# Acelogic/LTX-2-MLX

Measured on AMD Instinct MI355X. Metric: denoise_steps_per_sec, higher is better.
Workload: dtype bf16; 1 GPU; LTX-2 19B distilled DiT (48 layers, D=4096, 32x128 heads), 768x512x65 (N=3456 video tokens, S=1024 text tokens), 8-step distilled sigmas, bf16, random-init weights; parallelism=prompt-parallel x1 (independent prompt/seed per GPU, one RCCL weight broadcast)

## Files before the change

include/ltx2hip.h:

```cpp
#ifndef LTX2HIP_H
#define LTX2HIP_H

#include <stdint.h>

#ifdef __cplusplus
extern "C" {
#endif

#define LTX2_OK 0
#define LTX2_E_INVALID (-1)
#define LTX2_E_HIP (-2)
#define LTX2_E_STATE (-3)

#define LTX2_DTYPE_BF16 0
#define LTX2_DTYPE_F32 1
#define LTX2_DTYPE_FP8_E4M3FN 2

#define LTX2_ABI_VERSION 3

const char* ltx2_last_error(void);
void ltx2_clear_error(void);
int ltx2_abi_version(void);


#define LTX2_EPI_BF16 0
#define LTX2_EPI_GELU_BF16 1
#define LTX2_EPI_SILU_BF16 2
#define LTX2_EPI_F32 3
#define LTX2_EPI_RESID_GATE_F32 4
#define LTX2_EPI_ADD_BF16 5

int ltx2_gemm_bf16(const void* A, int64_t lda, const void* W, const float* bias, void* out, int64_t ldo, int M,
                   int N, int K, int epilogue, const float* gate, int64_t gate_stride, const float* gate_table,
                   const void* res, int64_t ldres, void* stream);

int ltx2_gemm_qkv_vt(const void* A, int64_t lda, const void* W, const float* bias, void* out, int64_t ldo, int M, int N, int K,
                     void* vt, int vt_col0, int Npad, int head_dim, int* fused, void* stream);

int ltx2_gemm_w8a16(const void* A, int64_t lda, const void* W8, const float* wscale, const float* bias, void* out, int64_t ldo, int M,
                    int N, int K, int epilogue, const float* gate, int64_t gate_stride, const float* gate_table, void* stream);

int ltx2_gemm_bf16_rowss(const void* A, int64_t lda, const void* W, const float* bias, void* out, int64_t ldo, int M, int N, int K, float* rowss,
                         int* written, void* stream);
int ltx2_flash_attn_rowscale(const void* Q, int64_t ldq, const void* K, int64_t ldk, const void* VT, int Npad, void* out, int64_t ldo, int Nq, int Nkv,
                             int H, int head_dim, float scale, const float* q_ss, int q_ss_ld, int q_norm_dim, float q_eps, void* stream);

int ltx2_gemm_bf16_fold(const void* A, int64_t lda, const void* W, const float* bias, void* out, int64_t ldo, int M, int N, int K, int epilogue,
                        const float* gate_table, void* shadow, int64_t ld_shadow, const float* shadow_scale, float* shadow_ss, int64_t ld_ss,
                        const float* rf_parts, int64_t rf_ld, int rf_nparts, int rf_dim, float rf_eps, int* supported, void* stream);

int ltx2_flash_attn_keymask(const void* Q, int64_t ldq, const void* K, int64_t ldk, const void* VT, int Npad, void* out, int64_t ldo,
                            int Nq, int Nkv, int H, int head_dim, float scale, const float* mask, void* words, void* stream);

#define LTX2_ROUTE_SKINNY 0
#define LTX2_ROUTE_V4_224 1
#define LTX2_ROUTE_V4_256 2
#define LTX2_ROUTE_V4_W8_224 3
#define LTX2_ROUTE_V4_W8_256 4
#define LTX2_ROUTE_V4_F8_224 5
#define LTX2_ROUTE_V4_F8_256 6
#define LTX2_ROUTE_PP 7
#define LTX2_ROUTE_SMALL 8
#define LTX2_ROUTE_NARROW 9
int ltx2_gemm_route(int M, int N, int K, int epilogue, int weights, int has_vt);

int ltx2_quantize_rows_fp8(const void* x_bf16, int64_t ldx, int rows, int K, void* codes, int64_t ldo, float* scale, void* stream);
int ltx2_gemm_fp8(const void* A8, int64_t lda, const float* ascale, const void* W8, const float* wscale, const float* bias, void* out,
                  int64_t ldo, int M, int N, int K, int epilogue, const float* gate, int64_t gate_stride, const float* gate_table,
                  void* stream);

int ltx2_gemm_fp8_qkv_vt(const void* A8, int64_t lda, const float* ascale, const void* W8, const float* wscale, const float* bias, void* out,
                         int64_t ldo, int M, int N, int K, void* vt, int vt_col0, int Npad, int head_dim, int* fused, void* stream);

int ltx2_gemv_f32(const float* a, int64_t lda, const void* W, const float* bias, float* out, int64_t ldo, int M,
                  int N, int K, int act_in, int act_out, void* stream);

int ltx2_conv3d_fused(const void* x, const void* w, const float* bias, void* out, int T, int H, int W, int Cin,
                      int Cout, int causal, int mode, const void* res, int ft, int fh, int fw, int residual,
                      int pad_zero, int kt, void* stream);

int ltx2_groupnorm_silu(const void* x, const void* res, void* y, int64_t P, int C, int groups, float eps,
                        const float* gamma, const float* beta, float* scratch, int act, void* stream);

int ltx2_s2d_downsample(const void* y, const void* x, void* out, int T, int H, int W, int Cc, int Cin, int st, int sh,
                        int sw, void* stream);

int ltx2_latent_normalize_nchw(const void* x, const float* mean, const float* std, float* out, int C, int64_t P,
                               void* stream);

int ltx2_adaln_rmsnorm(const float* x, int64_t ldx, void* out, int64_t ldo, int rows, int D, float eps,
                       int layer_norm, const float* scale_tab, const float* shift_tab, const float* scale_emb,
                       const float* shift_emb, int64_t emb_stride, void* stream);
int ltx2_adaln_rmsnorm2(const float* x, int64_t ldx, void* out0, void* out1, int64_t ldo, int rows, int D, float eps, const float* scale0,
                        const float* shift0, const float* scale1, const float* shift1, void* stream);

int ltx2_adaln_rmsnorm_fp8(const float* x, int64_t ldx, void* out_bf16, int64_t ldo, void* codes, int64_t ldq, float* scale, int rows, int D,
                           float eps, int layer_norm, const float* scale_tab, const float* shift_tab, const float* scale_emb,
                           const float* shift_emb, int64_t emb_stride, void* stream);

int ltx2_qknorm_rope(void* buf, int64_t ld, int rows, int D, int head_dim, int q_off, const float* q_weight,
                     int k_off, const float* k_weight, float eps, const float* cos, const float* sin, void* stream);

int ltx2_vt_transpose(const void* V, int64_t ld, void* VT, int Nkv, int Npad, int H, int head_dim, void* stream);

int ltx2_flash_attn(const void* Q, int64_t ldq, const void* K, int64_t ldk, const void* VT, int Npad, void* out,
                    int64_t ldo, int Nq, int Nkv, int H, int head_dim, float scale, void* stream);


int ltx2_attn_head_gate(void* att, int64_t ld, const void* x, int64_t ldx, const void* gate_w, const float* gate_b,
                        float* logits, int rows, int Dq, int H, int head_dim, void* stream);

int ltx2_flash_attn_gated(const void* Q, int64_t ldq, const void* K, int64_t ldk, const void* VT, int Npad, void* out, int64_t ldo, int Nq, int Nkv,
                          int H, int head_dim, float scale, const float* gate_logits, int gate_ld, void* stream);

int ltx2_flash_attn_gated_parts(const void* Q, int64_t ldq, const void* K, int64_t ldk, const void* VT, int Npad, void* out, int64_t ldo, int Nq, int Nkv,
                                int H, int head_dim, float scale, const void* x, int64_t ldx, const void* gate_w, const float* gate_b, int Dq, float* parts,
                                void* stream);

int ltx2_rope_tables(const float* positions, const float* freq_grid, const float* max_pos, int N, int n_dims, int n_freq,
                     int half_dim, float* cos_out, float* sin_out, void* stream);

int ltx2_timestep_sinusoid(const float* t, int64_t t_stride, float mult, int T, int dim, float* out_f32,
                           void* out_bf16, void* stream);

int ltx2_dequant_fp8_e4m3fn(const void* in, float scale, void* out_bf16, int64_t n, void* stream);
int ltx2_cast_f32_bf16(const float* in, void* out, int64_t n, void* stream);

int ltx2_x0_from_velocity(const float* latent, const float* velocity, const float* ts_ptr, int64_t ts_stride,
                          float ts_scalar, float* x0, int rows, int C, void* stream);

int ltx2_euler_step(const float* x, const float* x0, const float* mask, const float* clean, float sigma,
                    float sigma_next, float* out, int rows, int C, void* stream);

int ltx2_vae_prepare_latent(const float* latent, const float* std, const float* mean, const float* noise,
                            float noise_scale, void* out_bf16, int C, int64_t P, void* stream);
int ltx2_pixnorm_mod_silu(const void* x, void* y, int64_t P, int C, float eps, const float* table, const float* te,
                          int shift_row, int scale_row, void* stream);
int ltx2_vae_unpatchify(const void* x, float* video, int T, int H, int W, void* stream);
int ltx2_video_to_uint8(const float* video, uint8_t* frames, int T, int H, int W, void* stream);
int ltx2_video_chunk_to_uint8(const float* cur, const float* prev, const float* ramp, uint8_t* frames, int Tc, int prev_T, int ov, int H,
                              int W, int t_dst0, int T_out, void* stream);
int ltx2_tile_blend_accumulate(const float* tile, int dt, int dh, int dw, int nt, int nh, int nw, const float* mt, const float* mh,
                               const float* mw, float* out, float* wsum, int OT, int OH, int OW, int t0, int h0, int w0, void* stream);
int ltx2_tile_blend_finish(float* out, const float* wsum, int64_t plane, void* stream);

#define LTX2_MODEL_VIDEO_ONLY 0
#define LTX2_MODEL_AUDIO_VIDEO 1

typedef struct ltx2_dit ltx2_dit;

typedef struct ltx2_dit_config {
    int num_layers;
    int num_heads;
    int head_dim;
    int in_channels;
    int out_channels;
    int caption_channels;
    float norm_eps;
    float timestep_scale;
    int model_type;
    int audio_heads;
    int audio_head_dim;
    int audio_in_channels;
    int audio_out_channels;
    int cross_attention_adaln;
    int apply_gated_attention;
    float av_ca_timestep_scale;
} ltx2_dit_config;

int ltx2_dit_create(const ltx2_dit_config* cfg, ltx2_dit** out);
void ltx2_dit_destroy(ltx2_dit* ctx);

int ltx2_dit_set_weight(ltx2_dit* ctx, const char* name, const void* ptr, int dtype, int64_t numel);

int64_t ltx2_dit_workspace_bytes(const ltx2_dit* ctx, int N, int S, int per_token);
int ltx2_dit_bind_workspace(ltx2_dit* ctx, void* ptr, int64_t bytes, int N, int S, int per_token);
int64_t ltx2_dit_workspace_bytes_av(const ltx2_dit* ctx, int N, int S, int Na, int Sa, int per_token);
int ltx2_dit_bind_workspace_av(ltx2_dit* ctx, void* ptr, int64_t bytes, int N, int S, int Na, int Sa, int per_token);

int ltx2_dit_prepare(ltx2_dit* ctx, const float* context, int S, const float* rope_cos, const float* rope_sin,
                     void* stream);
int ltx2_dit_prepare_av(ltx2_dit* ctx, const float* v_context, int S, const float* v_cos, const float* v_sin,
                        const float* v_cross_cos, const float* v_cross_sin, const float* a_context, int Sa,
                        const float* a_cos, const float* a_sin, const float* a_cross_cos, const float* a_cross_sin,
                        void* stream);

int ltx2_dit_forward(ltx2_dit* ctx, const float* latent, const float* timesteps, int n_timesteps, const float* sigma,
                     float* velocity, void* stream);
int ltx2_dit_forward_av(ltx2_dit* ctx, const float* v_latent, const float* v_timesteps, int n_v_timesteps,
                        const float* v_sigma, const float* a_latent, const float* a_timesteps, int n_a_timesteps,
                        const float* a_sigma, float* v_velocity, float* a_velocity, void* stream);

int ltx2_dit_denoise_step(ltx2_dit* ctx, float* latent, const float* timesteps, int n_timesteps, const float* sigma_dev,
                          const float* mask, const float* clean, float sigma, float sigma_next, float* x0_out, void* stream);
int ltx2_dit_denoise_step_av(ltx2_dit* ctx, float* v_latent, float* a_latent, const float* v_timesteps,
                             int n_v_timesteps, const float* a_timesteps, int n_a_timesteps, const float* sigma_dev,
                             const float* v_mask, const float* v_clean, const float* a_mask, const float* a_clean,
                             float sigma, float sigma_next, float* v_x0_out, float* a_x0_out, void* stream);

int ltx2_dit_graph_capture(ltx2_dit* ctx, float* latent, const float* host_sigmas, int n_steps, void* stream);
int ltx2_dit_graph_capture_cond(ltx2_dit* ctx, float* latent, const float* host_sigmas, int n_steps, const float* mask, int64_t n_mask, const float* clean,
                                int64_t n_clean, void* stream);
int ltx2_dit_graph_capture_cond_av(ltx2_dit* ctx, float* v_latent, float* a_latent, const float* host_sigmas, int n_steps, const float* v_mask, int64_t n_v_mask,
                                   const float* v_clean, int64_t n_v_clean, const float* a_mask, int64_t n_a_mask, const float* a_clean, int64_t n_a_clean, void* stream);
int ltx2_dit_graph_capture_av(ltx2_dit* ctx, float* v_latent, float* a_latent, const float* host_sigmas, int n_steps,
                              void* stream);
int ltx2_dit_graph_launch(ltx2_dit* ctx, void* stream);

int ltx2_dit_set_context_mask(ltx2_dit* ctx, int modality, const float* mask, int S, void* stream);

int ltx2_dit_set_option(ltx2_dit* ctx, const char* name, int value);


int ltx2_dit_profile_begin(ltx2_dit* ctx, int epilogue);
int ltx2_dit_profile_end(ltx2_dit* ctx, double* total_ms, int64_t* launches, double* flops);

typedef struct ltx2_vae ltx2_vae;

#define LTX2_VAE_MAX_BLOCKS 16
#define LTX2_VAE_RES 0
#define LTX2_VAE_UPSAMPLE 1

typedef struct ltx2_vae_config {
    int n_blocks;
    int kind[LTX2_VAE_MAX_BLOCKS];
    int num_layers[LTX2_VAE_MAX_BLOCKS];
    int stride[LTX2_VAE_MAX_BLOCKS][3];
    int multiplier[LTX2_VAE_MAX_BLOCKS];
    int residual[LTX2_VAE_MAX_BLOCKS];
    int base_channels;
    int latent_channels;
    int timestep_conditioning;
    float decode_noise_scale;
} ltx2_vae_config;

int ltx2_vae_create(const ltx2_vae_config* cfg, ltx2_vae** out);
void ltx2_vae_destroy(ltx2_vae* ctx);
int ltx2_vae_set_weight(ltx2_vae* ctx, const char* name, const void* ptr, int dtype, int64_t numel);
int ltx2_vae_set_timestep_multiplier(ltx2_vae* ctx, float multiplier);
int64_t ltx2_vae_workspace_bytes(const ltx2_vae* ctx, int T, int H, int W);
int ltx2_vae_bind_workspace(ltx2_vae* ctx, void* ptr, int64_t bytes);
int ltx2_vae_decode(ltx2_vae* ctx, const float* latent, int T, int H, int W, float timestep, const float* noise,
                    int causal, float* video, void* stream);
int ltx2_vae_out_frames(const ltx2_vae* ctx, int T);

int ltx2_gemma_attn(const void* q, int64_t ldq, const void* k, int64_t ldk, const void* v, int64_t ldv, void* out, int64_t ldo, int Tq,
                    int Tkv, int heads, int kv_heads, int causal, int window, float scale, void* stream);
int ltx2_gemma_qknorm_rope(void* qkv, int64_t ld, int rows, int q_heads, int kv_heads, const float* q_w, const float* k_w, float eps,
                           const float* cos, const float* sin, void* stream);
int ltx2_gemma_resid_norm(const float* x_in, int64_t ldx, const void* y, int64_t ldy, const float* w_post, const float* w_next, float* x_out,
                          int64_t ld_xout, void* h_out, int64_t ldh, float* hf_out, int64_t ldhf, int rows, int D, float eps, void* stream);
#define LTX2_GEMMA_ACT_SILU 0
#define LTX2_GEMMA_ACT_GELU_TANH 1
int ltx2_gemma_gated_act(const void* gu, int64_t ldgu, void* out, int64_t ldo, int rows, int inter, int act, void* stream);
int ltx2_gemma_embed(const int32_t* ids, int rows, const void* table, int vocab, int D, float scale, float* x, int64_t ldx, void* stream);
int ltx2_gemma_features_rms(const float* hs, int64_t layer_stride, int64_t row_stride, const int32_t* valid, void* out, int64_t ldo, int T, int L,
                            int D, float eps, void* stream);

#define LTX2_AUDIO_PRO_NONE 0
#define LTX2_AUDIO_PRO_LEAKY_RELU 1
#define LTX2_AUDIO_PRO_MAGNITUDE 2
#define LTX2_AUDIO_ACT_NONE 0
#define LTX2_AUDIO_ACT_TANH 1
#define LTX2_AUDIO_ACT_CLIP 2
#define LTX2_AUDIO_ACT_LOG 3
int ltx2_audio_conv(const float* x, int64_t ldx, int h_in, int w_in, int c_in, const float* w, int64_t ldw, const float* bias, float* y,
                    int64_t ldy, int h_out, int w_out, int c_out, int kh, int kw, int stride, int dilation, int pad_h, int pad_w, int upsample,
                    int prologue, float slope, const float* res, int64_t ldres, float alpha, float beta, int act, void* stream);
int ltx2_audio_conv_transpose1d(const float* x, int64_t ldx, int t_in, int c_in, const float* w_phase, const float* bias, float* y, int64_t ldy,
                                int t_out, int c_out, int k, int rate, int padding, int prologue, float slope, void* stream);
int ltx2_audio_pixnorm_silu(const float* x, int64_t ldx, float* y, int64_t ldy, int64_t rows, int c, float eps, void* stream);
int ltx2_audio_snake_aa(const float* x, int64_t ldx, int t, int c, const float* alpha, const float* beta, const float* up_filter, int up_k,
                        const float* down_filter, int down_k, float* y, int64_t ldy, void* stream);
int ltx2_audio_upsample(const float* x, int64_t ldx, int t_in, int c, const float* filter, int k, int ratio, int pad, int pad_left, float* y,
                        int64_t ldy, int t_out, void* stream);

#ifdef __cplusplus
}
#endif
#endif
```

ltx-2-mlx_amd/csrc/attention.h:

```cpp
#pragma once
#include "common.h"

struct AttnParams {
    const bf16* Q;
    const bf16* K;
    const bf16* VT;
    bf16* O;
    long ldq, ldk, ldo, vt_head_stride;
    int Nq, Nkv, Npad, H;
    int head_dim;
    float scale_log2e;
    const float* q_ss;
    int q_ss_ld, q_norm_dim;
    float q_eps;
    const unsigned long long* kmask;
    const float* gate;
    int gate_ld;
    int gate_parts;
    const float* gate_bias;
};

int attn_launch(const AttnParams& p, hipStream_t stream);
int vt_transpose_launch(const bf16* V, long ld, bf16* VT, int Nkv, int Npad, int H, hipStream_t stream, int head_dim = 128);
```

ltx-2-mlx_amd/csrc/attention.hip:

```cpp
#include "attention.h"
#include <type_traits>

namespace {

constexpr int KVB = 64;
template <int HD>
struct Geo {
    static constexpr int K_TILE = KVB * HD * 2;
    static constexpr int V_TILE = HD * KVB * 2;
    static constexpr int STAGE = K_TILE + V_TILE;
    static constexpr int LDS_BYTES = 2 * STAGE;
    static constexpr int NJ = HD / 32;
};

#ifndef AT_DK
#define AT_DK 6
#endif
#ifndef AT_DV
#define AT_DV 6
#endif
#ifndef AT_XCD
#define AT_XCD 1
#endif
#ifndef AT_DMA
#define AT_DMA 0
#endif
#ifndef AT_PQK
#define AT_PQK 2
#endif
#ifndef AT_PPV
#define AT_PPV 1
#endif
#ifndef AT_PGAP
#define AT_PGAP 0
#endif
#ifndef AT_PRIO
#define AT_PRIO 1
#endif

__device__ __forceinline__ float max3(float a, float b, float c) {
    float d;
    asm("v_max3_f32 %0, %1, %2, %3" : "=v"(d) : "v"(a), "v"(b), "v"(c));
    return d;
}

#define AT_KEY_MASKED (-1.0e30f)

__device__ __forceinline__ void quad_fold_max(float& a, float& b) {
    asm volatile("s_nop 1\n\tv_permlane32_swap_b32 %0, %1\n\ts_nop 1" : "+v"(a), "+v"(b));
    float c = fmaxf(a, b), d = c;
    asm volatile("s_nop 1\n\tv_permlane16_swap_b32 %0, %1\n\ts_nop 1" : "+v"(c), "+v"(d));
    float e = fmaxf(c, d);
    a = e;
    b = e;
    asm volatile("s_nop 1\n\tv_permlane32_swap_b32 %0, %1\n\ts_nop 1" : "+v"(a), "+v"(b));
}
__device__ __forceinline__ void quad_fold_sum(float& a, float& b) {
    asm volatile("s_nop 1\n\tv_permlane32_swap_b32 %0, %1\n\ts_nop 1" : "+v"(a), "+v"(b));
    float c = a + b, d = c;
    asm volatile("s_nop 1\n\tv_permlane16_swap_b32 %0, %1\n\ts_nop 1" : "+v"(c), "+v"(d));
    float e = c + d;
    a = e;
    b = e;
    asm volatile("s_nop 1\n\tv_permlane32_swap_b32 %0, %1\n\ts_nop 1" : "+v"(a), "+v"(b));
}
__device__ __forceinline__ void mfma16_result_guard(f32x4 (&s)[4][2], float& t0, float& t1) {
    asm volatile("s_nop 7\n\ts_nop 7\n\ts_nop 3" : "+v"(s[0][0]), "+v"(s[0][1]), "+v"(s[1][0]), "+v"(s[1][1]), "+v"(s[2][0]), "+v"(s[2][1]), "+v"(s[3][0]), "+v"(s[3][1]),
                 "+v"(t0), "+v"(t1));
}

#ifndef AT_P_BIG
#ifdef LTX2_F16
#define AT_P_BIG 32768.0f
#else
#define AT_P_BIG 1073741824.0f
#endif
#endif

#ifdef AT_COUNT_FALLBACK
__device__ unsigned long long ltx2_at_counts[2];
#endif

template <int HD, bool QS = false, bool KM = false, int NW = 4>
__global__ __launch_bounds__(NW * 64, NW == 4 ? 2 : 1) void attn_fwd_kernel(const AttnParams p) {
    using G = Geo<HD>;
    constexpr int K_TILE = G::K_TILE, STAGE = G::STAGE, NJ = G::NJ * 4 / NW, QB = NW * 32;
    static_assert(NW == 4 || (NW == 8 && HD == 128), "waves per workgroup");
    constexpr int NKS = HD / 32, NDB = HD / 16;
    constexpr int NK = 4 * NKS, NV = 2 * NDB;
    constexpr int DK = AT_DK < NK ? AT_DK : NK, DV = AT_DV < NV ? AT_DV : NV;
    extern __shared__ __attribute__((aligned(16))) char smem[];
    const unsigned lds0 = (unsigned)(uintptr_t)(lds_ptr_t)smem;
    const int tid = threadIdx.x, lane = tid & 63;
    const int wv = __builtin_amdgcn_readfirstlane(tid >> 6);
    const int l15 = lane & 15, g = lane >> 4;
    const int nt = (p.Nkv + KVB - 1) / KVB, nfull = p.Nkv / KVB;

    unsigned k_vo[NJ], v_vo[NJ];
#pragma unroll
    for (int j = 0; j < NJ; ++j) {
        const int kr = HD == 128 ? (wv * NJ + j) * 4 + (lane >> 4) : (wv * NJ + j) * 8 + (lane >> 3);
        const int kchunk = HD == 128 ? ((lane & 15) ^ (kr & 15)) : ((lane & 7) ^ ((kr >> 1) & 7));
        k_vo[j] = ((unsigned)kr * (unsigned)p.ldk + kchunk * 8) * 2;
        const int vr = (wv * NJ + j) * 8 + (lane >> 3);
        const int vchunk = (lane & 7) ^ ((vr >> 1) & 7);
        v_vo[j] = ((unsigned)vr * (unsigned)p.Npad + vchunk * 8) * 2;
    }
    const unsigned k_tile_bytes = (unsigned)KVB * (unsigned)p.ldk * 2;
    const unsigned k_bytes = ((unsigned)(p.Nkv - 1) * (unsigned)p.ldk + HD) * 2, v_bytes = (unsigned)HD * (unsigned)p.Npad * 2;
    const int k_xor = HD == 128 ? l15 : ((l15 >> 1) & 7);
    const int v_xor = (l15 >> 1) & 7;
    unsigned k_lane[NKS], v_lane[2];
#pragma unroll
    for (int ks = 0; ks < NKS; ++ks) k_lane[ks] = lds0 + l15 * (2 * HD) + (((4 * ks + g) ^ k_xor) << 4);
#pragma unroll
    for (int kk = 0; kk < 2; ++kk) v_lane[kk] = lds0 + K_TILE + l15 * 128 + (((4 * kk + g) ^ v_xor) << 4);

    int head = blockIdx.y, qt = blockIdx.x;
#if AT_XCD
    if ((gridDim.y & 7) == 0) {
        const int b = blockIdx.y * gridDim.x + blockIdx.x, xcd = b & 7, idx = b >> 3;
        head = xcd + 8 * (idx / (int)gridDim.x);
        qt = idx % (int)gridDim.x;
    }
#endif
    const int tb = nt;
    const int q0 = qt * QB + wv * 32;

    const __amdgpu_buffer_rsrc_t rk = __builtin_amdgcn_make_buffer_rsrc((void*)(p.K + head * HD), 0, (int)k_bytes, 0x00020000);
    const __amdgpu_buffer_rsrc_t rv = __builtin_amdgcn_make_buffer_rsrc((void*)(p.VT + (long)head * p.vt_head_stride), 0, (int)v_bytes, 0x00020000);
    auto stage_piece = [&](int t, int buf, int i) {
        char* dst = smem + buf * STAGE + wv * (NJ * 1024);
#if defined(__HIP_DEVICE_COMPILE__)
        if (i < NJ)
            __builtin_amdgcn_raw_ptr_buffer_load_lds(rk, (lds_ptr_t)(dst + i * 1024), 16, k_vo[i], t * k_tile_bytes, 0, 0);
        else
            __builtin_amdgcn_raw_ptr_buffer_load_lds(rv, (lds_ptr_t)(dst + K_TILE + (i - NJ) * 1024), 16, v_vo[i - NJ], t * (KVB * 2), 0, 0);
#else
        (void)dst; (void)t; (void)i;
#endif
    };
#pragma unroll
    for (int i = 0; i < 2 * NJ; ++i) stage_piece(0, 0, i);

    float c[2] = {p.scale_log2e, p.scale_log2e};
    if constexpr (QS) {
        const int quarter = p.q_ss_ld >> 2;
        float ss[2] = {0.f, 0.f};
#pragma unroll
        for (int qb = 0; qb < 2; ++qb) {
            const float* sp = p.q_ss + (long)min(q0 + 16 * qb + l15, p.Nq - 1) * p.q_ss_ld + g * quarter;
#pragma unroll 4
            for (int jj = 0; jj < quarter; jj += 4) {
                const f32x4 t = *(const f32x4*)(sp + jj);
                ss[qb] += (t[0] + t[1]) + (t[2] + t[3]);
            }
        }
        quad_fold_sum(ss[0], ss[1]);
        c[0] *= rsqrtf(ss[0] / (float)p.q_norm_dim + p.q_eps);
        c[1] *= rsqrtf(ss[1] / (float)p.q_norm_dim + p.q_eps);
    }
    bf16x8 qf[2][NKS];
#pragma unroll
    for (int qb = 0; qb < 2; ++qb) {
        const int qrow = min(q0 + 16 * qb + l15, p.Nq - 1);
        const bf16* qp = p.Q + (long)qrow * p.ldq + head * HD + 8 * g;
#pragma unroll
        for (int ks = 0; ks < NKS; ++ks) {
            const bf16x8 raw = *(const bf16x8*)(qp + 32 * ks);
#pragma unroll
            for (int e = 0; e < 8; ++e) qf[qb][ks][e] = f2bf(bf2f(raw[e]) * c[qb]);
        }
    }

    f32x4 o[NDB][2];
#pragma unroll
    for (int d = 0; d < NDB; ++d)
#pragma unroll
        for (int qb = 0; qb < 2; ++qb) o[d][qb] = f32x4{0.f, 0.f, 0.f, 0.f};
    float M[2] = {0.f, 0.f}, l_run[2] = {0.f, 0.f};
    auto tile = [&](const int t, auto fast, auto masked, auto par, const bool first) __attribute__((always_inline)) {
        constexpr bool FAST = decltype(fast)::value, MASKED = decltype(masked)::value;
        constexpr int PAR = decltype(par)::value;
        static_assert(!(FAST && (MASKED || KM)), "the stale-maximum path takes whole, unmasked tiles");
        asm volatile("s_waitcnt vmcnt(0)" ::: "memory");
        __syncthreads();
        const int tn = min(t + 1, tb - 1);
        constexpr int nbuf = 1 - PAR;
#if AT_PRIO
        __builtin_amdgcn_s_setprio(AT_PQK);
#endif
        f32x4 s[4][2];
#pragma unroll
        for (int kb = 0; kb < 4; ++kb)
#pragma unroll
            for (int qb = 0; qb < 2; ++qb) {
                const float init = KM ? 0.f : -M[qb];
                s[kb][qb] = f32x4{init, init, init, init};
            }
        bf16x8 pf[2][2];
        float ps[2] = {0.f, 0.f};
        auto exp_pair = [&](auto KB, auto Q4) __attribute__((always_inline)) {
            constexpr int kb = decltype(KB)::value, q4 = decltype(Q4)::value, qb = q4 / 2, r = 2 * (q4 % 2), kk = kb / 2, e = 4 * (kb % 2) + r;
            asm volatile("" : "+v"(s[kb][qb]));
            float p0 = __builtin_amdgcn_exp2f(s[kb][qb][r]), p1 = __builtin_amdgcn_exp2f(s[kb][qb][r + 1]);
            asm volatile("" : "+v"(p0), "+v"(p1));
            ps[qb] += p0 + p1;
            pf[qb][kk][e] = f2bf(p0);
            pf[qb][kk][e + 1] = f2bf(p1);
        };
        u32x4 kf[NK];
        auto read_k = [&](auto N) {
            constexpr int n = decltype(N)::value, kb = n / NKS, ks = n % NKS;
            kf[n] = lds_read16<PAR * STAGE + kb * 16 * 2 * HD>(k_lane[ks]);
        };
        static_for<0, DK>(read_k);
        static_for<0, NK>([&](auto N) __attribute__((always_inline)) {
            constexpr int n = decltype(N)::value, kb = n / NKS, ks = n % NKS;
            if constexpr (n + DK < NK) read_k(std::integral_constant<int, n + DK>{});
            lds_wait<(n + DK < NK ? DK : NK - 1 - n)>(kf[n]);
            s[kb][0] = LTX2_MFMA_16x16x32(as_bf16x8(kf[n]), qf[0][ks], s[kb][0], 0, 0, 0);
            if constexpr (FAST && kb > 0) static_for<(4 * ks) / NKS, (4 * ks + 2) / NKS>([&](auto Q4) { exp_pair(std::integral_constant<int, kb - 1>{}, Q4); });
            s[kb][1] = LTX2_MFMA_16x16x32(as_bf16x8(kf[n]), qf[1][ks], s[kb][1], 0, 0, 0);
            if constexpr (FAST && kb > 0) static_for<(4 * ks + 2) / NKS, (4 * (ks + 1)) / NKS>([&](auto Q4) { exp_pair(std::integral_constant<int, kb - 1>{}, Q4); });
#if AT_DMA == 0
            if constexpr ((n & 1) && n / 2 < 2 * NJ) stage_piece(tn, nbuf, n / 2);
#elif AT_DMA == 2
            if constexpr ((n & 1) && n / 2 < NJ) stage_piece(tn, nbuf, n / 2);
#endif
        });
#if AT_DMA == 0
        static_for<NK / 2, 2 * NJ>([&](auto I) { stage_piece(tn, nbuf, decltype(I)::value); });
#elif AT_DMA == 1
        static_for<0, 2 * NJ>([&](auto I) { stage_piece(tn, nbuf, decltype(I)::value); });
#else
        static_for<(NK / 2 < NJ ? NK / 2 : NJ), 2 * NJ>([&](auto I) { stage_piece(tn, nbuf, decltype(I)::value); });
#endif
        u32x4 vf[NV];
        auto read_v = [&](auto N) {
            constexpr int n = decltype(N)::value, kk = n / NDB, db = n % NDB;
            vf[n] = lds_read16<PAR * STAGE + db * 16 * 128>(v_lane[kk]);
        };
        static_for<0, DV>(read_v);
#if AT_PRIO
        __builtin_amdgcn_s_setprio(AT_PGAP);
#endif
        auto pv = [&](auto N0, auto N1) __attribute__((always_inline)) {
            constexpr int n0 = decltype(N0)::value, n1 = decltype(N1)::value;
#if AT_PRIO
            __builtin_amdgcn_s_setprio(AT_PPV);
#endif
            static_for<n0, n1>([&](auto N) __attribute__((always_inline)) {
                constexpr int n = decltype(N)::value, kk = n / NDB, db = n % NDB;
                if constexpr (n + DV < NV) read_v(std::integral_constant<int, n + DV>{});
                lds_wait<(n + DV < NV ? DV : NV - 1 - n)>(vf[n]);
                o[db][0] = LTX2_MFMA_16x16x32(as_bf16x8(vf[n]), pf[0][kk], o[db][0], 0, 0, 0);
                o[db][1] = LTX2_MFMA_16x16x32(as_bf16x8(vf[n]), pf[1][kk], o[db][1], 0, 0, 0);
            });
#if AT_PRIO
            __builtin_amdgcn_s_setprio(AT_PGAP);
#endif
        };
        using I0 = std::integral_constant<int, 0>;
        using IN = std::integral_constant<int, NV>;
        bool classic = !FAST;
        if constexpr (FAST) {
            static_for<0, 4>([&](auto Q4) { exp_pair(std::integral_constant<int, 3>{}, Q4); });
            classic = __any(!(ps[0] <= AT_P_BIG && ps[1] <= AT_P_BIG));
#ifdef AT_COUNT_FALLBACK
            if (lane == 0) {
                atomicAdd(&ltx2_at_counts[0], 1ull);
                if (classic) atomicAdd(&ltx2_at_counts[1], 1ull);
            }
#endif
        }
        if (classic) {
            if constexpr (MASKED) {
                const int kv0 = t * KVB;
                unsigned long long km = ~0ull;
                if constexpr (KM) km = p.kmask[t];
#pragma unroll
                for (int kb = 0; kb < 4; ++kb)
#pragma unroll
                    for (int r = 0; r < 4; ++r) {
                        const int kl = 16 * kb + 4 * g + r;
                        const bool oob = kv0 + kl >= p.Nkv, off = KM && !((km >> kl) & 1ull);
#pragma unroll
                        for (int qb = 0; qb < 2; ++qb) {
                            if (oob) s[kb][qb][r] = -INFINITY;
                            else if (off) s[kb][qb][r] = AT_KEY_MASKED;
                        }
                    }
            }
            float tmax[2] = {-INFINITY, -INFINITY};
            mfma16_result_guard(s, tmax[0], tmax[1]);
#pragma unroll
            for (int qb = 0; qb < 2; ++qb)
#pragma unroll
                for (int r = 0; r < 4; ++r) {
                    tmax[qb] = max3(tmax[qb], s[0][qb][r], s[1][qb][r]);
                    tmax[qb] = max3(tmax[qb], s[2][qb][r], s[3][qb][r]);
                }
            quad_fold_max(tmax[0], tmax[1]);
            float sub[2];
#pragma unroll
            for (int qb = 0; qb < 2; ++qb) {
                if constexpr (KM) {
                    const float m_new = first ? tmax[qb] : fmaxf(M[qb], tmax[qb]);
                    if (!first) {
                        const float alpha = __builtin_amdgcn_exp2f(M[qb] - m_new);
                        l_run[qb] *= alpha;
#pragma unroll
                        for (int d = 0; d < NDB; ++d) o[d][qb] *= alpha;
                    }
                    M[qb] = m_new;
                    sub[qb] = m_new;
                } else {
                    const float up = first ? tmax[qb] : fmaxf(tmax[qb], 0.f);
                    if (!first) {
                        const float alpha = __builtin_amdgcn_exp2f(-up);
                        l_run[qb] *= alpha;
#pragma unroll
                        for (int d = 0; d < NDB; ++d) o[d][qb] *= alpha;
                    }
                    M[qb] += up;
                    sub[qb] = up;
                }
            }
            ps[0] = 0.f;
            ps[1] = 0.f;
#pragma unroll
            for (int kb = 0; kb < 4; ++kb)
#pragma unroll
                for (int qb = 0; qb < 2; ++qb)
#pragma unroll
                    for (int r = 0; r < 4; r += 2) {
                        const float p0 = __builtin_amdgcn_exp2f(s[kb][qb][r] - sub[qb]), p1 = __builtin_amdgcn_exp2f(s[kb][qb][r + 1] - sub[qb]);
                        ps[qb] += p0 + p1;
                        pf[qb][kb / 2][4 * (kb % 2) + r] = f2bf(p0);
                        pf[qb][kb / 2][4 * (kb % 2) + r + 1] = f2bf(p1);
                    }
        }
        l_run[0] += ps[0];
        l_run[1] += ps[1];
        pv(I0{}, IN{});
    };

    using T_ = std::true_type;
    using F_ = std::false_type;
    using P0 = std::integral_constant<int, 0>;
    using P1 = std::integral_constant<int, 1>;
    if constexpr (KM) {
        for (int t = 0; t < tb; ++t) {
            if (t & 1) tile(t, F_{}, T_{}, P1{}, false);
            else tile(t, F_{}, T_{}, P0{}, t == 0);
        }
    } else {
        const int t_fast_end = min(tb, nfull);
        int t = 0;
        if (nfull > 0) {
            tile(0, F_{}, F_{}, P0{}, true);
            t = 1;
            for (; t + 1 < t_fast_end; t += 2) {
                tile(t, T_{}, F_{}, P1{}, false);
                tile(t + 1, T_{}, F_{}, P0{}, false);
            }
            if (t < t_fast_end) {
                tile(t, T_{}, F_{}, P1{}, false);
                ++t;
            }
        }
        if (nfull < tb) {
            if (nfull & 1) tile(nfull, F_{}, T_{}, P1{}, false);
            else tile(nfull, F_{}, T_{}, P0{}, nfull == 0);
        }
    }
    asm volatile("s_waitcnt vmcnt(0)" ::: "memory");

    float lt[2] = {l_run[0], l_run[1]};
    quad_fold_sum(lt[0], lt[1]);
#pragma unroll
    for (int qb = 0; qb < 2; ++qb) {
        const int qrow = q0 + 16 * qb + l15;
        float inv = 1.0f / lt[qb];
        if (p.gate && qrow < p.Nq) {
            float gl = p.gate[(long)qrow * p.gate_ld + head];
            if (p.gate_parts > 1) {
                for (int pt = 1; pt < p.gate_parts; ++pt) gl += p.gate[((long)pt * p.Nq + qrow) * p.gate_ld + head];
                gl += p.gate_bias[head];
            }
            inv *= 2.f / (1.f + __expf(-gl));
        }
        bf16* op = p.O + (long)min(qrow, p.Nq - 1) * p.ldo + head * HD + 16 * (g & 1) + 8 * (g >> 1);
#pragma unroll
        for (int i = 0; i < NDB / 2; ++i) {
            bf16x4 a, b;
#pragma unroll
            for (int e = 0; e < 4; ++e) {
                a[e] = f2bf(o[2 * i][qb][e] * inv);
                b[e] = f2bf(o[2 * i + 1][qb][e] * inv);
            }
            u32x2 ua = __builtin_bit_cast(u32x2, a), ub = __builtin_bit_cast(u32x2, b);
            asm volatile("s_nop 1\n\tv_permlane16_swap_b32 %0, %2\n\tv_permlane16_swap_b32 %1, %3\n\ts_nop 1" : "+v"(ua[0]), "+v"(ua[1]), "+v"(ub[0]), "+v"(ub[1]));
            const u32x4 w = {ua[0], ua[1], ub[0], ub[1]};
            if (qrow < p.Nq) *(u32x4*)(op + 32 * i) = w;
        }
    }
}

template <int HD>
__global__ __launch_bounds__(256) void vt_transpose_kernel(const bf16* __restrict__ V, long ld, bf16* __restrict__ VT,
                                                           int Nkv, int Npad, long head_stride) {
    __shared__ bf16 tile[64][HD + 2];
    const int head = blockIdx.y, kv0 = blockIdx.x * 64, tid = threadIdx.x;
    {
        constexpr int W = HD / 4;
        const int r = tid >> 2, c0 = (tid & 3) * W;
        const int kv = kv0 + r;
        if (kv < Nkv) {
            const bf16* src = V + (long)kv * ld + head * HD + c0;
#pragma unroll
            for (int i = 0; i < W / 8; ++i) {
                const bf16x8 v = *(const bf16x8*)(src + i * 8);
#pragma unroll
                for (int e = 0; e < 8; ++e) tile[r][c0 + i * 8 + e] = v[e];
            }
        } else {
#pragma unroll
            for (int i = 0; i < W; ++i) tile[r][c0 + i] = f2bf(0.f);
        }
    }
    __syncthreads();
    if (tid < 2 * HD) {
        const int d = tid >> 1, p0 = (tid & 1) * 32;
        bf16* dst = VT + (long)head * head_stride + (long)d * Npad + kv0 + p0;
#pragma unroll
        for (int i = 0; i < 4; ++i) {
            bf16x8 v;
#pragma unroll
            for (int e = 0; e < 8; ++e) {
                const int pos = i * 8 + e;
                const int kvl = 16 * ((pos >> 2) & 1) + 4 * (pos >> 3) + (pos & 3);
                v[e] = tile[p0 + kvl][d];
            }
            *(bf16x8*)(dst + i * 8) = v;
        }
    }
}

}

int attn_launch(const AttnParams& p, hipStream_t stream) {
    LTX2_CHECK_ARG(p.Nq > 0 && p.Nkv > 0 && p.H > 0, "attention: empty problem");
    LTX2_CHECK_ARG(p.head_dim == 0 || p.head_dim == 128 || p.head_dim == 64, "attention: head_dim=%d, only 128 and 64 are implemented", p.head_dim);
    LTX2_CHECK_ARG(p.Npad % 64 == 0 && p.Npad >= p.Nkv, "attention: Npad=%d must be a multiple of 64 >= Nkv", p.Npad);
    LTX2_CHECK_ARG(p.ldq % 8 == 0 && p.ldk % 8 == 0 && p.ldo % 8 == 0, "attention: row strides must keep 16-byte alignment");
    LTX2_CHECK_ARG(p.ldk > 0 && ((long)p.Nkv + 2 * KVB) * p.ldk * 2 < (1L << 31), "attention: Nkv * ldk exceeds the 31-bit K byte offset");
    LTX2_CHECK_ARG((long)p.Npad * (p.head_dim == 64 ? 64 : 128) * 2 < (1L << 31), "attention: Npad * head_dim exceeds the 31-bit V^T byte offset");
    if (p.q_ss)
        LTX2_CHECK_ARG(p.head_dim != 64 && p.q_ss_ld > 0 && p.q_ss_ld % 16 == 0 && p.q_norm_dim > 0, "attention: the per-row scale form needs head_dim 128 and q_ss_ld %% 16 == 0");
#ifndef AT_NW
#define AT_NW 4
#endif
    const int nw = (p.head_dim != 64 && !p.kmask) ? AT_NW : 4;
    dim3 grid((p.Nq + nw * 32 - 1) / (nw * 32), p.H);
#define AT_LAUNCH_NW(HDV, QSV, KMV, NWV)                                                                                                        \
    do {                                                                                                                                        \
        static PerDeviceOnce once_;                                                                                                             \
        if (once_.first())                                                                                                                      \
            (void)hipFuncSetAttribute((const void*)attn_fwd_kernel<HDV, QSV, KMV, NWV>, hipFuncAttributeMaxDynamicSharedMemorySize, Geo<HDV>::LDS_BYTES); \
        hipLaunchKernelGGL((attn_fwd_kernel<HDV, QSV, KMV, NWV>), grid, dim3(NWV * 64), Geo<HDV>::LDS_BYTES, stream, p);                         \
    } while (0)
#define AT_LAUNCH(HDV, QSV, KMV) AT_LAUNCH_NW(HDV, QSV, KMV, 4)
    if (p.head_dim == 64) {
        if (p.kmask) AT_LAUNCH(64, false, true);
        else AT_LAUNCH(64, false, false);
    } else if (p.kmask) {
        if (p.q_ss) AT_LAUNCH(128, true, true);
        else AT_LAUNCH(128, false, true);
    } else if (p.q_ss) {
        if (nw == 8) AT_LAUNCH_NW(128, true, false, 8);
        else AT_LAUNCH(128, true, false);
    } else if (nw == 8) AT_LAUNCH_NW(128, false, false, 8);
    else AT_LAUNCH(128, false, false);
#undef AT_LAUNCH
#undef AT_LAUNCH_NW
    LTX2_CHECK_LAUNCH("attn_fwd_kernel");
    return LTX2_OK;
}

#ifdef AT_COUNT_FALLBACK
extern "C" int ltx2_attn_fallback_counts(unsigned long long* out2, int reset) {
    if (hipMemcpyFromSymbol(out2, HIP_SYMBOL(ltx2_at_counts), 16) != hipSuccess) return LTX2_E_HIP;
    if (reset) {
        const unsigned long long z[2] = {0, 0};
        if (hipMemcpyToSymbol(HIP_SYMBOL(ltx2_at_counts), z, 16) != hipSuccess) return LTX2_E_HIP;
    }
    return LTX2_OK;
}
#endif

int vt_transpose_launch(const bf16* V, long ld, bf16* VT, int Nkv, int Npad, int H, hipStream_t stream, int head_dim) {
    LTX2_CHECK_ARG(Npad % 64 == 0 && Npad >= Nkv && ld % 8 == 0, "vt_transpose: bad strides");
    LTX2_CHECK_ARG(head_dim == 128 || head_dim == 64, "vt_transpose: head_dim=%d, only 128 and 64 are implemented", head_dim);
    dim3 grid(Npad / 64, H);
    if (head_dim == 64)
        hipLaunchKernelGGL(vt_transpose_kernel<64>, grid, dim3(256), 0, stream, V, ld, VT, Nkv, Npad, 64L * Npad);
    else
        hipLaunchKernelGGL(vt_transpose_kernel<128>, grid, dim3(256), 0, stream, V, ld, VT, Nkv, Npad, 128L * Npad);
    LTX2_CHECK_LAUNCH("vt_transpose_kernel");
    return LTX2_OK;
}
```

ltx-2-mlx_amd/csrc/capi.hip:

```cpp
#include <stdarg.h>
#include <stdio.h>

#include "../../include/ltx2hip.h"
#include "attention.h"
#include "gemm.h"
#include "gemma.h"
#include "rowops.h"

static thread_local char g_err[512] = "";

void ltx2_set_error(const char* fmt, ...) {
    va_list ap;
    va_start(ap, fmt);
    vsnprintf(g_err, sizeof(g_err), fmt, ap);
    va_end(ap);
}

extern "C" {

const char* ltx2_last_error(void) { return g_err; }
void ltx2_clear_error(void) { g_err[0] = 0; }
int ltx2_abi_version(void) { return LTX2_ABI_VERSION; }

int ltx2_gemm_bf16(const void* A, int64_t lda, const void* W, const float* bias, void* out, int64_t ldo, int M,
                   int N, int K, int epilogue, const float* gate, int64_t gate_stride, const float* gate_table,
                   const void* res, int64_t ldres, void* stream) {
    LTX2_CHECK_ARG(epilogue >= 0 && epilogue <= LTX2_EPI_ADD_BF16, "gemm: epilogue %d out of range", epilogue);
    LTX2_CHECK_ARG(epilogue != LTX2_EPI_ADD_BF16 || res, "gemm: epilogue ADD_BF16 needs res");
    GemmParams p{};
    p.A = (const bf16*)A;
    p.lda = lda;
    p.W = (const bf16*)W;
    p.bias = bias;
    p.out = out;
    p.ldo = ldo;
    p.M = M;
    p.N = N;
    p.K = K;
    p.gate = gate;
    p.gate_stride = gate_stride;
    p.gate_table = gate_table;
    p.res = (const bf16*)res;
    p.ldres = ldres;
    return gemm_launch(p, epilogue, false, (hipStream_t)stream);
}

int ltx2_adaln_rmsnorm2(const float* x, int64_t ldx, void* out0, void* out1, int64_t ldo, int rows, int D, float eps, const float* scale0,
                        const float* shift0, const float* scale1, const float* shift1, void* stream) {
    LTX2_CHECK_ARG(x && out0 && out1, "adaln_rmsnorm2: null operand");
    const float* sct[2] = {scale0, scale1};
    const float* sht[2] = {shift0, shift1};
    const float* none[2] = {nullptr, nullptr};
    return norm_mod2_launch(x, ldx, (bf16*)out0, (bf16*)out1, ldo, rows, D, eps, sct, sht, none, none, (hipStream_t)stream);
}

int ltx2_gemm_bf16_rowss(const void* A, int64_t lda, const void* W, const float* bias, void* out, int64_t ldo, int M, int N, int K, float* rowss,
                         int* written, void* stream) {
    LTX2_CHECK_ARG(A && W && out && rowss && written, "gemm_bf16_rowss: null argument");
    GemmParams p{};
    p.A = (const bf16*)A;
    p.lda = lda;
    p.W = (const bf16*)W;
    p.bias = bias;
    p.out = out;
    p.ldo = ldo;
    p.M = M;
    p.N = N;
    p.K = K;
    *written = gemm_rowss_supported(p, EPI_BF16) ? 1 : 0;
    if (*written) p.rowss = rowss;
    return gemm_launch(p, EPI_BF16, false, (hipStream_t)stream);
}

int ltx2_gemm_bf16_fold(const void* A, int64_t lda, const void* W, const float* bias, void* out, int64_t ldo, int M, int N, int K, int epilogue,
                        const float* gate_table, void* shadow, int64_t ld_shadow, const float* shadow_scale, float* shadow_ss, int64_t ld_ss,
                        const float* rf_parts, int64_t rf_ld, int rf_nparts, int rf_dim, float rf_eps, int* supported, void* stream) {
    LTX2_CHECK_ARG(A && W && out && supported, "gemm_bf16_fold: null argument");
    LTX2_CHECK_ARG(epilogue == LTX2_EPI_BF16 || epilogue == LTX2_EPI_GELU_BF16 || epilogue == LTX2_EPI_RESID_GATE_F32, "gemm_bf16_fold: epilogue %d (BF16, GELU_BF16 or RESID_GATE_F32)", epilogue);
    GemmParams p{};
    p.A = (const bf16*)A;
    p.lda = lda;
    p.W = (const bf16*)W;
    p.bias = bias;
    p.out = out;
    p.ldo = ldo;
    p.M = M;
    p.N = N;
    p.K = K;
    p.gate_table = gate_table;
    p.shadow = (bf16*)shadow;
    p.ld_shadow = ld_shadow;
    p.shadow_scale = shadow_scale;
    p.shadow_ss = shadow_ss;
    p.ld_ss = ld_ss;
    p.rf_parts = rf_parts;
    p.rf_ld = rf_ld;
    p.rf_nparts = rf_nparts;
    p.rf_dim = rf_dim;
    p.rf_eps = rf_eps;
    *supported = ((p.shadow || p.rf_parts) && gemm_fold_supported(p, epilogue)) ? 1 : 0;
    if (!*supported) return LTX2_OK;
    return gemm_launch(p, epilogue, false, (hipStream_t)stream);
}

int ltx2_flash_attn_rowscale(const void* Q, int64_t ldq, const void* K, int64_t ldk, const void* VT, int Npad, void* out, int64_t ldo, int Nq, int Nkv,
                             int H, int head_dim, float scale, const float* q_ss, int q_ss_ld, int q_norm_dim, float q_eps, void* stream) {
    LTX2_CHECK_ARG(Q && K && VT && out && q_ss, "flash_attn_rowscale: null operand");
    LTX2_CHECK_ARG(head_dim == 128, "flash_attn_rowscale: head_dim=%d, only 128 is implemented", head_dim);
    AttnParams a{};
    a.Q = (const bf16*)Q;
    a.ldq = ldq;
    a.K = (const bf16*)K;
    a.ldk = ldk;
    a.VT = (const bf16*)VT;
    a.vt_head_stride = (long)head_dim * Npad;
    a.head_dim = head_dim;
    a.O = (bf16*)out;
    a.ldo = ldo;
    a.Nq = Nq;
    a.Nkv = Nkv;
    a.Npad = Npad;
    a.H = H;
    a.scale_log2e = scale * 1.4426950408889634f;
    a.q_ss = q_ss;
    a.q_ss_ld = q_ss_ld;
    a.q_norm_dim = q_norm_dim;
    a.q_eps = q_eps;
    return attn_launch(a, (hipStream_t)stream);
}

int ltx2_flash_attn_keymask(const void* Q, int64_t ldq, const void* K, int64_t ldk, const void* VT, int Npad, void* out, int64_t ldo, int Nq, int Nkv,
                            int H, int head_dim, float scale, const float* mask, void* words, void* stream) {
    LTX2_CHECK_ARG(Q && K && VT && out && mask && words, "flash_attn_keymask: null operand");
    if (const int rc = keymask_words_launch(mask, Nkv, (unsigned long long*)words, Npad / 64, (hipStream_t)stream)) return rc;
    AttnParams a{};
    a.Q = (const bf16*)Q;
    a.ldq = ldq;
    a.K = (const bf16*)K;
    a.ldk = ldk;
    a.VT = (const bf16*)VT;
    a.vt_head_stride = (long)head_dim * Npad;
    a.head_dim = head_dim;
    a.O = (bf16*)out;
    a.ldo = ldo;
    a.Nq = Nq;
    a.Nkv = Nkv;
    a.Npad = Npad;
    a.H = H;
    a.scale_log2e = scale * 1.4426950408889634f;
    a.kmask = (const unsigned long long*)words;
    return attn_launch(a, (hipStream_t)stream);
}

int ltx2_gemm_route(int M, int N, int K, int epilogue, int weights, int has_vt) {
    static const long dummy[2] = {0, 0};
    GemmParams p{};
    p.M = M;
    p.N = N;
    p.K = K;
    p.lda = K;
    p.ldo = N;
    p.out = (void*)dummy;
    if (weights == 2) {
        p.A8 = (const unsigned char*)dummy;
        p.ascale = (const float*)dummy;
    } else {
        p.A = (const bf16*)dummy;
    }
    if (weights >= 1) {
        p.W8 = (const unsigned char*)dummy;
        p.wscale = (const float*)dummy;
    } else {
        p.W = (const bf16*)dummy;
    }
    const int r = gemm_route(p, epilogue, false);
    if (!has_vt || r < 0) return r;
    p.vt = (bf16*)dummy;
    p.vt_col0 = 2 * (N / 3);
    p.vt_hd = (N / 3) % 128 == 0 ? 128 : 64;
    p.vt_npad = (M + 63) / 64 * 64;
    return r | (gemm_vt_fused(p, epilogue) ? 0x100 : 0);
}

int ltx2_quantize_rows_fp8(const void* x, int64_t ldx, int rows, int K, void* codes, int64_t ldo, float* scale, void* stream) {
    LTX2_CHECK_ARG(x && codes && scale, "quantize_rows_fp8: null argument");
    return quant_rows_fp8_launch((const bf16*)x, ldx, rows, K, (unsigned char*)codes, ldo, scale, (hipStream_t)stream);
}

int ltx2_gemm_fp8(const void* A8, int64_t lda, const float* ascale, const void* W8, const float* wscale, const float* bias, void* out,
                  int64_t ldo, int M, int N, int K, int epilogue, const float* gate, int64_t gate_stride, const float* gate_table,
                  void* stream) {
    LTX2_CHECK_ARG(A8 && ascale && W8 && wscale && out, "gemm_fp8: null operand");
    GemmParams p{};
    p.A8 = (const unsigned char*)A8;
    p.ascale = ascale;
    p.lda = lda;
    p.W8 = (const unsigned char*)W8;
    p.wscale = wscale;
    p.bias = bias;
    p.out = out;
    p.ldo = ldo;
    p.M = M;
    p.N = N;
    p.K = K;
    p.gate = gate;
    p.gate_stride = gate_stride;
    p.gate_table = gate_table;
    return gemm_launch(p, epilogue, false, (hipStream_t)stream);
}

int ltx2_gemm_qkv_vt(const void* A, int64_t lda, const void* W, const float* bias, void* out, int64_t ldo, int M, int N, int K,
                     void* vt, int vt_col0, int Npad, int head_dim, int* fused, void* stream) {
    LTX2_CHECK_ARG(A && W && out && vt, "gemm_qkv_vt: null operand");
    LTX2_CHECK_ARG(head_dim == 64 || head_dim == 128, "gemm_qkv_vt: head_dim=%d, only 128 and 64 are implemented", head_dim);
    LTX2_CHECK_ARG(vt_col0 > 0 && vt_col0 < N && (N - vt_col0) % head_dim == 0 && Npad % 64 == 0 && Npad >= M, "gemm_qkv_vt: bad V column range / Npad");
    GemmParams p{};
    p.A = (const bf16*)A;
    p.lda = lda;
    p.W = (const bf16*)W;
    p.bias = bias;
    p.out = out;
    p.ldo = ldo;
    p.M = M;
    p.N = N;
    p.K = K;
    p.vt = (bf16*)vt;
    p.vt_col0 = vt_col0;
    p.vt_npad = Npad;
    p.vt_hd = head_dim;
    p.vt_head_stride = (long)head_dim * Npad;
    const bool f = gemm_vt_fused(p, EPI_BF16);
    if (fused) *fused = f ? 1 : 0;
    if (!f) p.vt = nullptr;
    int rc = gemm_launch(p, EPI_BF16, false, (hipStream_t)stream);
    if (rc != LTX2_OK || f) return rc;
    return vt_transpose_launch((const bf16*)out + vt_col0, ldo, (bf16*)vt, M, Npad, (N - vt_col0) / head_dim, (hipStream_t)stream, head_dim);
}

int ltx2_gemm_fp8_qkv_vt(const void* A8, int64_t lda, const float* ascale, const void* W8, const float* wscale, const float* bias, void* out,
                         int64_t ldo, int M, int N, int K, void* vt, int vt_col0, int Npad, int head_dim, int* fused, void* stream) {
    LTX2_CHECK_ARG(A8 && ascale && W8 && wscale && out && vt, "gemm_fp8_qkv_vt: null operand");
    LTX2_CHECK_ARG(head_dim == 64 || head_dim == 128, "gemm_fp8_qkv_vt: head_dim=%d, only 128 and 64 are implemented", head_dim);
    LTX2_CHECK_ARG(vt_col0 > 0 && vt_col0 < N && (N - vt_col0) % head_dim == 0 && Npad % 64 == 0 && Npad >= M, "gemm_fp8_qkv_vt: bad V column range / Npad");
    GemmParams p{};
    p.A8 = (const unsigned char*)A8;
    p.ascale = ascale;
    p.lda = lda;
    p.W8 = (const unsigned char*)W8;
    p.wscale = wscale;
    p.bias = bias;
    p.out = out;
    p.ldo = ldo;
    p.M = M;
    p.N = N;
    p.K = K;
    p.vt = (bf16*)vt;
    p.vt_col0 = vt_col0;
    p.vt_npad = Npad;
    p.vt_hd = head_dim;
    p.vt_head_stride = (long)head_dim * Npad;
    const bool f = gemm_vt_fused(p, EPI_BF16);
    if (fused) *fused = f ? 1 : 0;
    if (!f) p.vt = nullptr;
    int rc = gemm_launch(p, EPI_BF16, false, (hipStream_t)stream);
    if (rc != LTX2_OK || f) return rc;
    return vt_transpose_launch((const bf16*)out + vt_col0, ldo, (bf16*)vt, M, Npad, (N - vt_col0) / head_dim, (hipStream_t)stream, head_dim);
}

int ltx2_gemm_w8a16(const void* A, int64_t lda, const void* W8, const float* wscale, const float* bias, void* out, int64_t ldo, int M,
                    int N, int K, int epilogue, const float* gate, int64_t gate_stride, const float* gate_table, void* stream) {
    LTX2_CHECK_ARG(A && W8 && wscale && out, "gemm_w8a16: null operand");
    GemmParams p{};
    p.A = (const bf16*)A;
    p.lda = lda;
    p.W8 = (const unsigned char*)W8;
    p.wscale = wscale;
    p.bias = bias;
    p.out = out;
    p.ldo = ldo;
    p.M = M;
    p.N = N;
    p.K = K;
    p.gate = gate;
    p.gate_stride = gate_stride;
    p.gate_table = gate_table;
    return gemm_launch(p, epilogue, false, (hipStream_t)stream);
}

int ltx2_gemv_f32(const float* a, int64_t lda, const void* W, const float* bias, float* out, int64_t ldo, int M,
                  int N, int K, int act_in, int act_out, void* stream) {
    LTX2_CHECK_ARG(a && W && out, "gemv: null operand");
    return gemv_launch(a, lda, (const bf16*)W, bias, out, ldo, M, N, K, act_in, act_out, (hipStream_t)stream);
}

int ltx2_adaln_rmsnorm(const float* x, int64_t ldx, void* out, int64_t ldo, int rows, int D, float eps,
                       int layer_norm, const float* scale_tab, const float* shift_tab, const float* scale_emb,
                       const float* shift_emb, int64_t emb_stride, void* stream) {
    LTX2_CHECK_ARG(x && out, "adaln_rmsnorm: null operand");
    return norm_mod_launch(x, ldx, (bf16*)out, ldo, rows, D, eps, layer_norm, scale_tab, shift_tab, scale_emb, shift_emb,
                           emb_stride, (hipStream_t)stream);
}

int ltx2_adaln_rmsnorm_fp8(const float* x, int64_t ldx, void* out_bf16, int64_t ldo, void* codes, int64_t ldq, float* scale, int rows, int D,
                           float eps, int layer_norm, const float* scale_tab, const float* shift_tab, const float* scale_emb,
                           const float* shift_emb, int64_t emb_stride, void* stream) {
    LTX2_CHECK_ARG(x && codes && scale, "adaln_rmsnorm_fp8: null operand");
    return norm_mod_launch(x, ldx, (bf16*)out_bf16, ldo, rows, D, eps, layer_norm, scale_tab, shift_tab, scale_emb, shift_emb, emb_stride,
                           (hipStream_t)stream, (unsigned char*)codes, ldq, scale);
}

int ltx2_qknorm_rope(void* buf, int64_t ld, int rows, int D, int head_dim, int q_off, const float* q_weight,
                     int k_off, const float* k_weight, float eps, const float* cos, const float* sin, void* stream) {
    LTX2_CHECK_ARG(buf && q_weight, "qknorm_rope: null operand");
    const int offs[2] = {q_off, k_off};
    const float* wts[2] = {q_weight, k_weight};
    return qknorm_rope_launch((bf16*)buf, ld, rows, D, head_dim, k_weight ? 2 : 1, offs, wts, eps, cos, sin,
                              (hipStream_t)stream);
}

int ltx2_vt_transpose(const void* V, int64_t ld, void* VT, int Nkv, int Npad, int H, int head_dim, void* stream) {
    LTX2_CHECK_ARG(V && VT, "vt_transpose: null operand");
    return vt_transpose_launch((const bf16*)V, ld, (bf16*)VT, Nkv, Npad, H, (hipStream_t)stream, head_dim);
}

int ltx2_attn_head_gate(void* att, int64_t ld, const void* x, int64_t ldx, const void* gate_w, const float* gate_b,
                        float* logits, int rows, int Dq, int H, int head_dim, void* stream) {
    LTX2_CHECK_ARG(att && x && gate_w && gate_b && logits, "attn_head_gate: null operand");
    int rc = gate_logits_launch((const bf16*)x, ldx, (const bf16*)gate_w, gate_b, logits, H, rows, Dq, H, (hipStream_t)stream);
    if (rc != LTX2_OK) return rc;
    return head_gate_launch((bf16*)att, ld, logits, H, rows, H, head_dim, (hipStream_t)stream);
}

int ltx2_flash_attn_gated(const void* Q, int64_t ldq, const void* K, int64_t ldk, const void* VT, int Npad, void* out, int64_t ldo, int Nq, int Nkv,
                          int H, int head_dim, float scale, const float* gate_logits, int gate_ld, void* stream) {
    LTX2_CHECK_ARG(Q && K && VT && out && gate_logits && gate_ld >= H, "flash_attn_gated: null operand / gate_ld < H");
    LTX2_CHECK_ARG(head_dim == 128 || head_dim == 64, "flash_attn_gated: head_dim=%d, only 128 and 64 are implemented", head_dim);
    AttnParams a{};
    a.Q = (const bf16*)Q;
    a.ldq = ldq;
    a.K = (const bf16*)K;
    a.ldk = ldk;
    a.VT = (const bf16*)VT;
    a.vt_head_stride = (long)head_dim * Npad;
    a.head_dim = head_dim;
    a.O = (bf16*)out;
    a.ldo = ldo;
    a.Nq = Nq;
    a.Nkv = Nkv;
    a.Npad = Npad;
    a.H = H;
    a.scale_log2e = scale * 1.4426950408889634f;
    a.gate = gate_logits;
    a.gate_ld = gate_ld;
    return attn_launch(a, (hipStream_t)stream);
}

int ltx2_flash_attn_gated_parts(const void* Q, int64_t ldq, const void* K, int64_t ldk, const void* VT, int Npad, void* out, int64_t ldo, int Nq, int Nkv,
                                int H, int head_dim, float scale, const void* x, int64_t ldx, const void* gate_w, const float* gate_b, int Dq, float* parts,
                                void* stream) {
    LTX2_CHECK_ARG(Q && K && VT && out && x && gate_w && gate_b && parts, "flash_attn_gated_parts: null operand");
    LTX2_CHECK_ARG(head_dim == 128 || head_dim == 64, "flash_attn_gated_parts: head_dim=%d, only 128 and 64 are implemented", head_dim);
    if (const int rc = gate_logits_parts_launch((const bf16*)x, ldx, (const bf16*)gate_w, parts, Nq, Dq, H, (hipStream_t)stream)) return rc;
    AttnParams a{};
    a.Q = (const bf16*)Q;
    a.ldq = ldq;
    a.K = (const bf16*)K;
    a.ldk = ldk;
    a.VT = (const bf16*)VT;
    a.vt_head_stride = (long)head_dim * Npad;
    a.head_dim = head_dim;
    a.O = (bf16*)out;
    a.ldo = ldo;
    a.Nq = Nq;
    a.Nkv = Nkv;
    a.Npad = Npad;
    a.H = H;
    a.scale_log2e = scale * 1.4426950408889634f;
    a.gate = parts;
    a.gate_ld = H;
    a.gate_parts = GATE_LOGIT_PARTS;
    a.gate_bias = gate_b;
    return attn_launch(a, (hipStream_t)stream);
}

int ltx2_flash_attn(const void* Q, int64_t ldq, const void* K, int64_t ldk, const void* VT, int Npad, void* out,
                    int64_t ldo, int Nq, int Nkv, int H, int head_dim, float scale, void* stream) {
    LTX2_CHECK_ARG(Q && K && VT && out, "flash_attn: null operand");
    LTX2_CHECK_ARG(head_dim == 128 || head_dim == 64, "flash_attn: head_dim=%d, only 128 and 64 are implemented", head_dim);
    AttnParams a{};
    a.Q = (const bf16*)Q;
    a.ldq = ldq;
    a.K = (const bf16*)K;
    a.ldk = ldk;
    a.VT = (const bf16*)VT;
    a.vt_head_stride = (long)head_dim * Npad;
    a.head_dim = head_dim;
    a.O = (bf16*)out;
    a.ldo = ldo;
    a.Nq = Nq;
    a.Nkv = Nkv;
    a.Npad = Npad;
    a.H = H;
    a.scale_log2e = scale * 1.4426950408889634f;
    return attn_launch(a, (hipStream_t)stream);
}

int ltx2_timestep_sinusoid(const float* t, int64_t t_stride, float mult, int T, int dim, float* out_f32,
                           void* out_bf16, void* stream) {
    LTX2_CHECK_ARG(t && (out_f32 || out_bf16), "timestep_sinusoid: null operand");
    return timestep_sinusoid_launch(t, t_stride, 0.f, mult, T, dim, out_f32, (bf16*)out_bf16, (hipStream_t)stream);
}

int ltx2_dequant_fp8_e4m3fn(const void* in, float scale, void* out_bf16, int64_t n, void* stream) {
    return dequant_fp8_launch((const unsigned char*)in, scale, (bf16*)out_bf16, n, (hipStream_t)stream);
}

int ltx2_groupnorm_silu(const void* x, const void* res, void* y, int64_t P, int C, int groups, float eps,
                        const float* gamma, const float* beta, float* scratch, int act, void* stream) {
    return groupnorm_silu_launch((const bf16*)x, (const bf16*)res, (bf16*)y, P, C, groups, eps, gamma, beta, scratch, act, (hipStream_t)stream);
}

int ltx2_s2d_downsample(const void* y, const void* x, void* out, int T, int H, int W, int Cc, int Cin, int st, int sh,
                        int sw, void* stream) {
    return s2d_downsample_launch((const bf16*)y, (const bf16*)x, (bf16*)out, T, H, W, Cc, Cin, st, sh, sw, (hipStream_t)stream);
}

int ltx2_latent_normalize_nchw(const void* x, const float* mean, const float* std, float* out, int C, int64_t P, void* stream) {
    return latent_normalize_nchw_launch((const bf16*)x, mean, std, out, C, P, (hipStream_t)stream);
}

int ltx2_rope_tables(const float* positions, const float* freq_grid, const float* max_pos, int N, int n_dims, int n_freq,
                     int half_dim, float* cos_out, float* sin_out, void* stream) {
    return rope_tables_launch(positions, freq_grid, max_pos, N, n_dims, n_freq, half_dim, cos_out, sin_out, (hipStream_t)stream);
}

int ltx2_cast_f32_bf16(const float* in, void* out, int64_t n, void* stream) {
    LTX2_CHECK_ARG(in && out, "cast: null operand");
    return cast_f32_bf16_launch(in, (bf16*)out, n, (hipStream_t)stream);
}

int ltx2_x0_from_velocity(const float* latent, const float* velocity, const float* ts_ptr, int64_t ts_stride,
                          float ts_scalar, float* x0, int rows, int C, void* stream) {
    LTX2_CHECK_ARG(latent && velocity && x0, "x0_from_velocity: null operand");
    return x0_from_velocity_launch(latent, velocity, ts_ptr, ts_stride, ts_scalar, x0, rows, C, (hipStream_t)stream);
}

int ltx2_euler_step(const float* x, const float* x0, const float* mask, const float* clean, float sigma,
                    float sigma_next, float* out, int rows, int C, void* stream) {
    LTX2_CHECK_ARG(x && x0 && out, "euler_step: null operand");
    return euler_step_launch(x, x0, mask, clean, sigma, sigma_next, out, rows, C, (hipStream_t)stream);
}

int ltx2_vae_prepare_latent(const float* latent, const float* std, const float* mean, const float* noise,
                            float noise_scale, void* out_bf16, int C, int64_t P, void* stream) {
    LTX2_CHECK_ARG(latent && std && mean && out_bf16, "vae_prepare_latent: null operand");
    return vae_prepare_latent_launch(latent, std, mean, noise, noise_scale, (bf16*)out_bf16, C, P, (hipStream_t)stream);
}

int ltx2_pixnorm_mod_silu(const void* x, void* y, int64_t P, int C, float eps, const float* table, const float* te,
                          int shift_row, int scale_row, void* stream) {
    LTX2_CHECK_ARG(x && y && table, "pixnorm_mod_silu: null operand");
    return pixnorm_mod_silu_launch((const bf16*)x, (bf16*)y, P, C, eps, table, te, shift_row, scale_row,
                                   (hipStream_t)stream);
}

int ltx2_vae_unpatchify(const void* x, float* video, int T, int H, int W, void* stream) {
    LTX2_CHECK_ARG(x && video, "vae_unpatchify: null operand");
    return vae_unpatchify_launch((const bf16*)x, video, T, H, W, (hipStream_t)stream);
}

int ltx2_video_chunk_to_uint8(const float* cur, const float* prev, const float* ramp, uint8_t* frames, int Tc, int prev_T, int ov, int H,
                              int W, int t_dst0, int T_out, void* stream) {
    LTX2_CHECK_ARG(cur && frames, "video_chunk_to_uint8: null operand");
    return video_chunk_to_uint8_launch(cur, prev, ramp, frames, Tc, prev_T, ov, H, W, t_dst0, T_out, (hipStream_t)stream);
}

int ltx2_tile_blend_accumulate(const float* tile, int dt, int dh, int dw, int nt, int nh, int nw, const float* mt, const float* mh,
                               const float* mw, float* out, float* wsum, int OT, int OH, int OW, int t0, int h0, int w0, void* stream) {
    LTX2_CHECK_ARG(tile && mt && mh && mw && out && wsum, "tile_blend_accumulate: null operand");
    return tile_blend_accumulate_launch(tile, dt, dh, dw, nt, nh, nw, mt, mh, mw, out, wsum, OT, OH, OW, t0, h0, w0, (hipStream_t)stream);
}

int ltx2_tile_blend_finish(float* out, const float* wsum, int64_t plane, void* stream) {
    LTX2_CHECK_ARG(out && wsum && plane > 0, "tile_blend_finish: bad argument");
    return tile_blend_finish_launch(out, wsum, (long)plane, (hipStream_t)stream);
}

int ltx2_video_to_uint8(const float* video, uint8_t* frames, int T, int H, int W, void* stream) {
    LTX2_CHECK_ARG(video && frames, "video_to_uint8: null operand");
    return video_to_uint8_launch(video, frames, T, H, W, (hipStream_t)stream);
}

int ltx2_gemma_attn(const void* q, int64_t ldq, const void* k, int64_t ldk, const void* v, int64_t ldv, void* out, int64_t ldo, int Tq,
                    int Tkv, int heads, int kv_heads, int causal, int window, float scale, void* stream) {
    return gemma_attn_launch((const bf16*)q, (long)ldq, (const bf16*)k, (long)ldk, (const bf16*)v, (long)ldv, (bf16*)out, (long)ldo, Tq, Tkv,
                             heads, kv_heads, causal, window, scale, (hipStream_t)stream);
}

int ltx2_gemma_qknorm_rope(void* qkv, int64_t ld, int rows, int q_heads, int kv_heads, const float* q_w, const float* k_w, float eps,
                           const float* cos, const float* sin, void* stream) {
    return gemma_qknorm_rope_launch((bf16*)qkv, (long)ld, rows, q_heads, kv_heads, q_w, k_w, eps, cos, sin, (hipStream_t)stream);
}

int ltx2_gemma_resid_norm(const float* x_in, int64_t ldx, const void* y, int64_t ldy, const float* w_post, const float* w_next, float* x_out,
                          int64_t ld_xout, void* h_out, int64_t ldh, float* hf_out, int64_t ldhf, int rows, int D, float eps, void* stream) {
    return gemma_resid_norm_launch(x_in, (long)ldx, (const bf16*)y, (long)ldy, w_post, w_next, x_out, (long)ld_xout, (bf16*)h_out, (long)ldh,
                                   hf_out, (long)ldhf, rows, D, eps, (hipStream_t)stream);
}

int ltx2_gemma_gated_act(const void* gu, int64_t ldgu, void* out, int64_t ldo, int rows, int inter, int act, void* stream) {
    return gemma_gated_act_launch((const bf16*)gu, (long)ldgu, (bf16*)out, (long)ldo, rows, inter, act, (hipStream_t)stream);
}

int ltx2_gemma_embed(const int32_t* ids, int rows, const void* table, int vocab, int D, float scale, float* x, int64_t ldx, void* stream) {
    return gemma_embed_launch((const int*)ids, rows, (const bf16*)table, vocab, D, scale, x, (long)ldx, (hipStream_t)stream);
}

int ltx2_gemma_features_rms(const float* hs, int64_t layer_stride, int64_t row_stride, const int32_t* valid, void* out, int64_t ldo, int T, int L,
                            int D, float eps, void* stream) {
    return gemma_features_rms_launch(hs, (long)layer_stride, (long)row_stride, (const int*)valid, (bf16*)out, (long)ldo, T, L, D, eps,
                                     (hipStream_t)stream);
}

}
```

ltx-2-mlx_amd/csrc/dit_engine.hip:

```cpp
#include <math.h>
#include <string.h>

#include <string>
#include <unordered_map>
#include <vector>

#include "../../include/ltx2hip.h"
#include "attention.h"
#include "gemm.h"
#include "rowops.h"

#define TRY(expr)                       \
    do {                                \
        int rc_ = (expr);               \
        if (rc_ != LTX2_OK) return rc_; \
    } while (0)

namespace {
struct Wt {
    const void* p;
    int dtype;
    long n;
};

struct AdaW {
    const bf16 *t1_w = nullptr, *t2_w = nullptr, *lin_w = nullptr;
    const float *t1_b = nullptr, *t2_b = nullptr, *lin_b = nullptr;
    int rows = 0;
};

struct AttnW {
    const bf16 *qkv_w = nullptr, *q_w = nullptr, *kv_w = nullptr, *o_w = nullptr, *g_w = nullptr;
    const float *qkv_b = nullptr, *q_b = nullptr, *kv_b = nullptr, *o_b = nullptr, *g_b = nullptr, *qn = nullptr,
                *kn = nullptr;
};

struct BlockW {
    AttnW self, text;
    const bf16 *ff1_w = nullptr, *ff2_w = nullptr;
    const float *ff1_b = nullptr, *ff2_b = nullptr, *sst = nullptr, *prompt_sst = nullptr;
};

struct LayerW {
    BlockW m[2];
    AttnW a2v, v2a;
    const float* ca[2] = {nullptr, nullptr};
};

struct ModW {
    const bf16 *patch_w = nullptr, *cap1_w = nullptr, *cap2_w = nullptr, *proj_w = nullptr;
    const float *patch_b = nullptr, *cap1_b = nullptr, *cap2_b = nullptr, *proj_b = nullptr, *sst_out = nullptr;
    AdaW ada, prompt, cross_ss, cross_gate;
};

struct Mod {
    int D = 0, H = 0, hd = 0, Cin = 0, Cout = 0;
    int N = 0, Npad = 0, S = 0, Spad = 0;
    float *x = nullptr, *sin_f = nullptr, *e1_f = nullptr, *e_f = nullptr, *emb = nullptr, *vel = nullptr, *x0 = nullptr,
          *cosb = nullptr, *sinb = nullptr, *ccos = nullptr, *csin = nullptr, *aux_e = nullptr, *prompt_emb = nullptr, *sst_all = nullptr, *comb = nullptr, *ca_all = nullptr, *ca_comb = nullptr,
          *cross_ss = nullptr, *cross_gate = nullptr, *glog = nullptr;
    int glog_parts = 1;
    const float* glog_bias = nullptr;
    bf16 *lat = nullptr, *h = nullptr, *h2 = nullptr, *qkv = nullptr, *vt = nullptr, *att = nullptr, *ff = nullptr,
         *sin_b = nullptr, *e1_b = nullptr, *es_b = nullptr, *ctx_in = nullptr, *c1 = nullptr, *ctxp = nullptr,
         *ctxm = nullptr, *kv2 = nullptr, *vt2 = nullptr;
    const bf16* ctx = nullptr;
    unsigned long long* kmask = nullptr;
    bool use_comb = false;
    bool has_kmask = false;
    float* ts_tok = nullptr;
    float* qss = nullptr;
    float* knq = nullptr;
    bool qfold = false;
    float* rss = nullptr;
    long rss_ld = 0;
    int fold_max = 0;
    unsigned char* a8 = nullptr;
    float* a8s = nullptr;
};

inline long align_up(long v, long a = 256) { return (v + a - 1) / a * a; }
}

struct ltx2_dit {
    ltx2_dit_config cfg{};
    bool av = false, v2 = false, gated = false;
    std::unordered_map<std::string, Wt> weights;
    std::vector<LayerW> layers;
    ModW mw[2];
    Mod m[2];
    bool resolved = false;
    char* ws = nullptr;
    long ws_bytes = 0;
    int per_token = 0;
    float* sigmas_dev = nullptr;
    std::unordered_map<const void*, const float*> fp8_scale;
    bool adaln_combine = true;
    bool text_kv_ahead = true;
    hipEvent_t text_kv_ev = nullptr;
    int fold_norms = 1;
    bool fp8_compute = false;
    bool prepared = false;
    hipGraph_t graph = nullptr;
    hipGraphExec_t exec = nullptr;
    hipStream_t side = nullptr;
    std::vector<hipEvent_t> sync_ev;
    size_t sync_next = 0;
    int prof_epi = -2;
    std::vector<hipEvent_t> prof_ev;
    size_t prof_used = 0;
    double prof_flops = 0;
};

namespace {

long carve(ltx2_dit* c, char* base, int N, int S, int Na, int Sa, int per_token) {
    const long L = c->cfg.num_layers;
    long off = 0;
    auto take = [&](long bytes) {
        char* p = base ? base + off : nullptr;
        off += align_up(bytes);
        return p;
    };
    c->sigmas_dev = (float*)take(4L * 64);
    for (int k = 0; k < (c->av ? 2 : 1); ++k) {
        Mod& m = c->m[k];
        const long n = k ? Na : N, s = k ? Sa : S;
        const long D = m.D, npad = align_up(n, 64), spad = align_up(s, 64);
        const long Cctx = c->cfg.caption_channels > 0 ? c->cfg.caption_channels : D;
        const long T = per_token ? n : 1, rows = c->v2 ? 9 : 6;
        m.x = (float*)take(4L * n * D);
        m.lat = (bf16*)take(2L * n * m.Cin);
        m.h = (bf16*)take(2L * n * D);
        m.h2 = (bf16*)take(c->av ? 2L * n * D : 0);
        m.qkv = (bf16*)take(2L * n * 3 * D);
        m.vt = (bf16*)take(2L * D * npad);
        m.att = (bf16*)take(2L * n * D);
        m.ff = (bf16*)take(2L * n * 4 * D);
        m.glog = (float*)take(c->gated ? 4L * n * m.H * GATE_LOGIT_PARTS : 0);
        m.kmask = (unsigned long long*)take(8L * (spad / 64));
        m.qss = (float*)take(4L * n * (D / 64));
        m.knq = (float*)take(4L * L * D);
        const bool fold_bufs = k == 0 && !c->av;
        m.rss_ld = align_up(n, 256) + 256;
        m.rss = (float*)take(fold_bufs ? 4L * (D / 256 + 1) * m.rss_ld : 0);
        m.a8 = (unsigned char*)take((c->fp8_compute && k == 0) ? n * 4 * D : 0);
        m.a8s = (float*)take((c->fp8_compute && k == 0) ? 4L * n : 0);
        m.sin_f = (float*)take(4L * 256);
        m.e1_f = (float*)take(4L * D);
        m.aux_e = (float*)take(4L * D);
        m.e_f = (float*)take(4L * T * D);
        m.emb = (float*)take(4L * T * rows * D);
        m.prompt_emb = (float*)take(c->v2 ? 4L * 2 * D : 0);
        m.sst_all = (float*)take(4L * L * rows * D);
        m.comb = (float*)take(4L * L * rows * D);
        m.cross_ss = (float*)take(c->av ? 4L * 4 * D : 0);
        m.cross_gate = (float*)take(c->av ? 4L * D : 0);
        m.ca_all = (float*)take(c->av ? 4L * L * 5 * D : 0);
        m.ca_comb = (float*)take(c->av ? 4L * L * 5 * D : 0);
        m.ts_tok = (float*)take(per_token ? 4L * n : 0);
        m.sin_b = (bf16*)take(per_token ? 2L * n * 256 : 0);
        m.e1_b = (bf16*)take(per_token ? 2L * n * D : 0);
        m.es_b = (bf16*)take(per_token ? 2L * n * D : 0);
        m.vel = (float*)take(4L * n * m.Cout);
        m.x0 = (float*)take(4L * n * m.Cout);
        m.cosb = (float*)take(4L * n * (D / 2));
        m.sinb = (float*)take(4L * n * (D / 2));
        const long Dc = c->m[c->av ? 1 : 0].D;
        m.ccos = (float*)take(c->av ? 4L * n * (Dc / 2) : 0);
        m.csin = (float*)take(c->av ? 4L * n * (Dc / 2) : 0);
        m.ctx_in = (bf16*)take(2L * s * Cctx);
        m.c1 = (bf16*)take(c->cfg.caption_channels > 0 ? 2L * s * D : 0);
        m.ctxp = (bf16*)take(c->cfg.caption_channels > 0 ? 2L * s * D : 0);
        m.ctxm = (bf16*)take(c->v2 ? 2L * s * D : 0);
        const long kv_layers = c->v2 ? 1 : L;
        m.kv2 = (bf16*)take(2L * kv_layers * s * 2 * D);
        m.vt2 = (bf16*)take(2L * kv_layers * D * spad);
    }
    return off;
}

const void* find(ltx2_dit* c, const std::string& name, int dtype, long numel) {
    auto it = c->weights.find(name);
    if (it == c->weights.end()) {
        ltx2_set_error("dit: missing weight '%s'", name.c_str());
        return nullptr;
    }
    if (dtype == LTX2_DTYPE_BF16 && it->second.dtype == LTX2_DTYPE_FP8_E4M3FN && it->second.n == numel) {
        auto sc = c->weights.find(name + "_scale");
        if (sc == c->weights.end() || sc->second.dtype != LTX2_DTYPE_F32) {
            ltx2_set_error("dit: fp8-resident weight '%s' has no fp32 '%s_scale' vector", name.c_str(), name.c_str());
            return nullptr;
        }
        c->fp8_scale[it->second.p] = (const float*)sc->second.p;
        return it->second.p;
    }
    if (it->second.dtype != dtype || it->second.n != numel) {
        ltx2_set_error("dit: weight '%s' has dtype %d / numel %ld, expected dtype %d / numel %ld", name.c_str(),
                       it->second.dtype, it->second.n, dtype, numel);
        return nullptr;
    }
    return it->second.p;
}

#define GETW(dst, name, rows, cols)                                                                          \
    do {                                                                                                     \
        dst = (const bf16*)find(c, std::string(name) + ".weight", LTX2_DTYPE_BF16, (long)(rows) * (cols));   \
        if (!dst) return LTX2_E_STATE;                                                                       \
    } while (0)
#define GETB(dst, name, n)                                                                    \
    do {                                                                                      \
        dst = (const float*)find(c, std::string(name) + ".bias", LTX2_DTYPE_F32, (long)(n));  \
        if (!dst) return LTX2_E_STATE;                                                        \
    } while (0)
#define GETF(dst, name, n)                                                          \
    do {                                                                            \
        dst = (const float*)find(c, std::string(name), LTX2_DTYPE_F32, (long)(n));  \
        if (!dst) return LTX2_E_STATE;                                              \
    } while (0)

int resolve_ada(ltx2_dit* c, AdaW& a, const std::string& name, long D, int rows) {
    GETW(a.t1_w, name + ".emb.timestep_embedder.linear_1", D, 256);
    GETB(a.t1_b, name + ".emb.timestep_embedder.linear_1", D);
    GETW(a.t2_w, name + ".emb.timestep_embedder.linear_2", D, D);
    GETB(a.t2_b, name + ".emb.timestep_embedder.linear_2", D);
    GETW(a.lin_w, name + ".linear", rows * D, D);
    GETB(a.lin_b, name + ".linear", rows * D);
    a.rows = rows;
    return LTX2_OK;
}

int resolve_attn(ltx2_dit* c, AttnW& a, const std::string& name, long Dq, long Dc, long Di, int heads, bool self) {
    if (self) {
        GETW(a.qkv_w, name + ".to_qkv", 3 * Di, Dq);
        GETB(a.qkv_b, name + ".to_qkv", 3 * Di);
    } else {
        GETW(a.q_w, name + ".to_q", Di, Dq);
        GETB(a.q_b, name + ".to_q", Di);
        GETW(a.kv_w, name + ".to_kv", 2 * Di, Dc);
        GETB(a.kv_b, name + ".to_kv", 2 * Di);
    }
    GETW(a.o_w, name + ".to_out.0", Dq, Di);
    GETB(a.o_b, name + ".to_out.0", Dq);
    GETF(a.qn, name + ".q_norm.weight", Di);
    GETF(a.kn, name + ".k_norm.weight", Di);
    if (c->gated) {
        GETW(a.g_w, name + ".to_gate_logits", heads, Dq);
        GETB(a.g_b, name + ".to_gate_logits", heads);
    }
    return LTX2_OK;
}

int resolve(ltx2_dit* c) {
    if (c->resolved) return LTX2_OK;
    c->fp8_scale.clear();
    const int nm = c->av ? 2 : 1;
    const int rows = c->v2 ? 9 : 6;
    for (int k = 0; k < nm; ++k) {
        const std::string pre = k ? "audio_" : "";
        const long D = c->m[k].D;
        ModW& w = c->mw[k];
        GETW(w.patch_w, pre + "patchify_proj", D, c->m[k].Cin);
        GETB(w.patch_b, pre + "patchify_proj", D);
        TRY(resolve_ada(c, w.ada, pre + "adaln_single", D, rows));
        if (c->v2) TRY(resolve_ada(c, w.prompt, pre + "prompt_adaln_single", D, 2));
        if (c->cfg.caption_channels > 0) {
            GETW(w.cap1_w, pre + "caption_projection.linear_1", D, c->cfg.caption_channels);
            GETB(w.cap1_b, pre + "caption_projection.linear_1", D);
            GETW(w.cap2_w, pre + "caption_projection.linear_2", D, D);
            GETB(w.cap2_b, pre + "caption_projection.linear_2", D);
        }
        GETF(w.sst_out, pre + "scale_shift_table", 2 * D);
        GETW(w.proj_w, pre + "proj_out", c->m[k].Cout, D);
        GETB(w.proj_b, pre + "proj_out", c->m[k].Cout);
    }
    if (c->av) {
        TRY(resolve_ada(c, c->mw[0].cross_ss, "av_ca_video_scale_shift_adaln_single", c->m[0].D, 4));
        TRY(resolve_ada(c, c->mw[0].cross_gate, "av_ca_a2v_gate_adaln_single", c->m[0].D, 1));
        TRY(resolve_ada(c, c->mw[1].cross_ss, "av_ca_audio_scale_shift_adaln_single", c->m[1].D, 4));
        TRY(resolve_ada(c, c->mw[1].cross_gate, "av_ca_v2a_gate_adaln_single", c->m[1].D, 1));
    }
    c->layers.assign(c->cfg.num_layers, LayerW());
    for (int i = 0; i < c->cfg.num_layers; ++i) {
        LayerW& w = c->layers[i];
        const std::string p = "transformer_blocks." + std::to_string(i) + ".";
        for (int k = 0; k < nm; ++k) {
            const std::string pre = k ? "audio_" : "";
            const long D = c->m[k].D;
            BlockW& b = w.m[k];
            TRY(resolve_attn(c, b.self, p + pre + "attn1", D, D, D, c->m[k].H, true));
            TRY(resolve_attn(c, b.text, p + pre + "attn2", D, D, D, c->m[k].H, false));
            GETW(b.ff1_w, p + pre + "ff.net.0.proj", 4 * D, D);
            GETB(b.ff1_b, p + pre + "ff.net.0.proj", 4 * D);
            GETW(b.ff2_w, p + pre + "ff.net.2", D, 4 * D);
            GETB(b.ff2_b, p + pre + "ff.net.2", D);
            GETF(b.sst, p + pre + "scale_shift_table", rows * D);
            if (c->v2) GETF(b.prompt_sst, p + pre + "prompt_scale_shift_table", 2 * D);
        }
        if (c->av) {
            const long Dv = c->m[0].D, Da = c->m[1].D;
            TRY(resolve_attn(c, w.a2v, p + "audio_to_video_attn", Dv, Da, Da, c->m[1].H, false));
            TRY(resolve_attn(c, w.v2a, p + "video_to_audio_attn", Da, Dv, Da, c->m[1].H, false));
            GETF(w.ca[0], p + "scale_shift_table_a2v_ca_video", 5 * Dv);
            GETF(w.ca[1], p + "scale_shift_table_a2v_ca_audio", 5 * Da);
        }
    }
    c->resolved = true;
    return LTX2_OK;
}
#undef GETW
#undef GETB
#undef GETF

thread_local ltx2_dit* g_prof_ctx = nullptr;

struct VtOut {
    bf16* vt;
    int col0, npad, hd;
};

bool f8_route(ltx2_dit* c, const bf16* W, int M, int N, int K, int epi) {
    if (!c->fp8_compute || !c->m[0].a8 || M < 1024 || M > c->m[0].N || K > 4 * c->m[0].D) return false;
    auto f8 = c->fp8_scale.find((const void*)W);
    if (f8 == c->fp8_scale.end()) return false;
    GemmParams q{};
    q.A8 = c->m[0].a8;
    q.ascale = c->m[0].a8s;
    q.lda = K;
    q.W8 = (const unsigned char*)W;
    q.wscale = f8->second;
    q.out = c->m[0].x;
    q.ldo = 8;
    q.M = M;
    q.N = N;
    q.K = K;
    return gemm_v4_f8_supported(q, epi);
}

bool text_qfold_ok(ltx2_dit* c, int k) {
    const Mod& m = c->m[k];
    if (m.D % 1024 != 0 || m.hd != 128) return false;
    const bf16* W = c->layers[0].m[k].text.q_w;
    GemmParams q{};
    q.M = m.N;
    q.N = m.D;
    q.K = m.D;
    q.lda = m.D;
    q.ldo = m.D;
    q.out = m.x;
    if (k == 0 && f8_route(c, W, m.N, m.D, m.D, EPI_BF16)) {
        q.A8 = m.a8;
        q.ascale = m.a8s;
    } else {
        q.A = m.h;
    }
    auto f8 = c->fp8_scale.find((const void*)W);
    if (f8 != c->fp8_scale.end()) {
        q.W8 = (const unsigned char*)W;
        q.wscale = f8->second;
    } else {
        q.W = W;
    }
    return gemm_rowss_supported(q, EPI_BF16);
}

int fold_supported(ltx2_dit* c, int k) {
#ifdef LTX2_F16
    (void)c; (void)k;
    return 0;
#else
    if (c->av || c->v2 || c->gated || c->fp8_compute || !c->fp8_scale.empty() || k != 0) return 0;
    const Mod& m = c->m[k];
    if (!m.rss || m.D % 256 != 0 || m.D / 256 > GEMM_RF_MAX_PARTS) return 0;
    const BlockW& w = c->layers[0].m[k];
    GemmParams q{};
    q.A = m.h;
    q.lda = m.D;
    q.M = m.N;
    q.K = m.D;
    q.out = m.x;
    q.W = w.self.o_w;
    q.N = m.D;
    q.ldo = m.D;
    q.shadow = m.h;
    q.ld_shadow = m.D;
    q.shadow_ss = m.rss;
    q.ld_ss = m.rss_ld;
    if (!gemm_fold_supported(q, EPI_RESID_GATE_F32)) return 0;
    GemmParams r{};
    r.A = m.h;
    r.lda = m.D;
    r.M = m.N;
    r.K = m.D;
    r.N = m.D;
    r.ldo = m.D;
    r.out = m.qkv;
    r.W = w.text.q_w;
    r.rf_parts = m.rss;
    r.rf_ld = m.rss_ld;
    r.rf_nparts = m.D / 256;
    r.rf_dim = m.D;
    if (!gemm_fold_supported(r, EPI_BF16)) return 0;
    return 1;
#endif
}

__global__ void vec_mul_kernel(const float* __restrict__ a, const float* __restrict__ b, float* __restrict__ out, int n) {
    const int i = blockIdx.x * blockDim.x + threadIdx.x;
    if (i < n) out[i] = a[i] * b[i];
}

struct Fold {
    bf16* shadow = nullptr;
    const float* shadow_scale = nullptr;
    float* shadow_ss = nullptr;
    long ld_shadow = 0;
    const float* rf_parts = nullptr;
    long ld_ss = 0;
    int rf_nparts = 0, rf_dim = 0;
    float rf_eps = 0.f;
};

int dense(ltx2_dit* c, const bf16* A, long lda, const bf16* W, const float* bias, void* out, long ldo, int M, int N, int K, int epi,
          hipStream_t st, const float* gate = nullptr, long gate_stride = 0, const float* gate_table = nullptr,
          const VtOut* vt = nullptr, bool* vt_done = nullptr, bool preq = false, float* rowss = nullptr, const Fold* fold = nullptr) {
    GemmParams p{};
    if (fold) {
        p.shadow = fold->shadow;
        p.shadow_scale = fold->shadow_scale;
        p.shadow_ss = fold->shadow_ss;
        p.ld_shadow = fold->ld_shadow;
        p.ld_ss = fold->ld_ss;
        p.rf_parts = fold->rf_parts;
        p.rf_ld = fold->ld_ss;
        p.rf_nparts = fold->rf_nparts;
        p.rf_dim = fold->rf_dim;
        p.rf_eps = fold->rf_eps;
    }
    p.A = A;
    p.lda = lda;
    p.W = W;
    if (!c->fp8_scale.empty()) {
        auto f8 = c->fp8_scale.find((const void*)W);
        if (f8 != c->fp8_scale.end()) {
            p.W = nullptr;
            p.W8 = (const unsigned char*)W;
            p.wscale = f8->second;
        }
    }
    p.bias = bias;
    p.out = out;
    p.ldo = ldo;
    p.M = M;
    p.N = N;
    p.K = K;
    p.gate = gate;
    p.gate_stride = gate_stride;
    p.gate_table = gate_table;
    p.rowss = rowss;
    if (p.W8 && f8_route(c, W, M, N, K, epi)) {
        if (!preq) TRY(quant_rows_fp8_launch(A, lda, M, K, c->m[0].a8, K, c->m[0].a8s, st));
        p.A8 = c->m[0].a8;
        p.ascale = c->m[0].a8s;
        p.lda = K;
        p.A = nullptr;
    } else if (preq) {
        ltx2_set_error("dit: a pre-quantised activation reached a GEMM that does not take the fp8 path");
        return LTX2_E_STATE;
    }
    if (vt) {
        p.vt = vt->vt;
        p.vt_col0 = vt->col0;
        p.vt_npad = vt->npad;
        p.vt_hd = vt->hd;
        p.vt_head_stride = (long)vt->hd * vt->npad;
        *vt_done = gemm_vt_fused(p, epi);
        if (!*vt_done) p.vt = nullptr;
    }
    ltx2_dit* pc = g_prof_ctx;
    const bool prof = pc && (pc->prof_epi == -1 || pc->prof_epi == epi);
    if (prof) {
        while (pc->prof_ev.size() < pc->prof_used + 2) {
            hipEvent_t e;
            if (hipEventCreate(&e) != hipSuccess) return LTX2_E_HIP;
            pc->prof_ev.push_back(e);
        }
        (void)hipEventRecord(pc->prof_ev[pc->prof_used], st);
    }
    const int rc = gemm_launch(p, epi, false, st);
    if (prof) {
        (void)hipEventRecord(pc->prof_ev[pc->prof_used + 1], st);
        pc->prof_used += 2;
        pc->prof_flops += 2.0 * M * N * K;
    }
    return rc;
}

__global__ void mask_sigma_kernel(const float* __restrict__ mask, const float* __restrict__ sigma, float* __restrict__ ts, int n) {
    const int i = blockIdx.x * blockDim.x + threadIdx.x;
    if (i < n) ts[i] = mask[i] * sigma[0];
}

__global__ void silu_cast_kernel(const float* __restrict__ in, bf16* __restrict__ out, long n) {
    for (long i = (long)blockIdx.x * blockDim.x + threadIdx.x; i < n; i += (long)gridDim.x * blockDim.x)
        out[i] = f2bf(silu_f(in[i]));
}

int adaln_chain(ltx2_dit* c, Mod& m, const AdaW& a, const float* ts, long t_stride, int T, float mult, float* emb, float* e_out,
                hipStream_t st) {
    const int D = m.D;
    if (T == 1) {
        float* e = e_out ? e_out : m.aux_e;
        TRY(timestep_sinusoid_launch(ts, 0, 0.f, mult, 1, 256, m.sin_f, nullptr, st));
        TRY(gemv_launch(m.sin_f, 256, a.t1_w, a.t1_b, m.e1_f, D, 1, D, 256, 0, 1, st));
        TRY(gemv_launch(m.e1_f, D, a.t2_w, a.t2_b, e, D, 1, D, D, 0, 0, st));
        TRY(gemv_launch(e, D, a.lin_w, a.lin_b, emb, (long)a.rows * D, 1, a.rows * D, D, 1, 0, st));
    } else {
        TRY(timestep_sinusoid_launch(ts, t_stride, 0.f, mult, T, 256, nullptr, m.sin_b, st));
        TRY(dense(c, m.sin_b, 256, a.t1_w, a.t1_b, m.e1_b, D, T, D, 256, EPI_SILU_BF16, st));
        TRY(dense(c, m.e1_b, D, a.t2_w, a.t2_b, e_out, D, T, D, D, EPI_F32, st));
        hipLaunchKernelGGL(silu_cast_kernel, dim3(2048), dim3(256), 0, st, e_out, m.es_b, (long)T * D);
        LTX2_CHECK_LAUNCH("silu_cast_kernel");
        TRY(dense(c, m.es_b, D, a.lin_w, a.lin_b, emb, (long)a.rows * D, T, a.rows * D, D, EPI_F32, st));
    }
    return LTX2_OK;
}

struct GateRef {
    const float* p = nullptr;
    int parts = 1;
    const float* bias = nullptr;
};
int attend(const bf16* q, long ldq, const bf16* k, long ldk, const bf16* vt, int npad, bf16* out, long ldo, int nq,
           int nkv, int H, int hd, hipStream_t st, const float* q_ss = nullptr, float q_eps = 0.f,
           const unsigned long long* kmask = nullptr, GateRef gate = GateRef{}) {
    AttnParams a{};
    a.kmask = kmask;
    a.gate = gate.p;
    a.gate_ld = H;
    a.gate_parts = gate.parts;
    a.gate_bias = gate.bias;
    if (q_ss) {
        a.q_ss = q_ss;
        a.q_ss_ld = H * hd / 64;
        a.q_norm_dim = H * hd;
        a.q_eps = q_eps;
    }
    a.Q = q;
    a.ldq = ldq;
    a.K = k;
    a.ldk = ldk;
    a.VT = vt;
    a.vt_head_stride = (long)hd * npad;
    a.O = out;
    a.ldo = ldo;
    a.Nq = nq;
    a.Nkv = nkv;
    a.Npad = npad;
    a.H = H;
    a.head_dim = hd;
    a.scale_log2e = 1.4426950408889634f / sqrtf((float)hd);
    return attn_launch(a, st);
}

hipEvent_t next_event(ltx2_dit* c) {
    if (c->sync_next == c->sync_ev.size()) {
        hipEvent_t e = nullptr;
        if (hipEventCreateWithFlags(&e, hipEventDisableTiming) != hipSuccess) return nullptr;
        c->sync_ev.push_back(e);
    }
    return c->sync_ev[c->sync_next++];
}

int stream_after(ltx2_dit* c, hipStream_t from, hipStream_t to) {
    if (from == to) return LTX2_OK;
    hipEvent_t e = next_event(c);
    if (!e || hipEventRecord(e, from) != hipSuccess || hipStreamWaitEvent(to, e, 0) != hipSuccess) {
        ltx2_set_error("dit: stream fork/join failed: %s", hipGetErrorString(hipGetLastError()));
        return LTX2_E_HIP;
    }
    return LTX2_OK;
}

hipEvent_t event_record(ltx2_dit* c, hipStream_t from) {
    hipEvent_t e = next_event(c);
    if (!e || hipEventRecord(e, from) != hipSuccess) {
        ltx2_set_error("dit: event record failed: %s", hipGetErrorString(hipGetLastError()));
        return nullptr;
    }
    return e;
}

int event_wait(hipEvent_t e, hipStream_t to) {
    if (!e || hipStreamWaitEvent(to, e, 0) != hipSuccess) {
        ltx2_set_error("dit: stream wait failed: %s", hipGetErrorString(hipGetLastError()));
        return LTX2_E_HIP;
    }
    return LTX2_OK;
}

inline bool gate_in_parts(int rows, int Dq) { return rows >= 1024 && Dq % (GATE_LOGIT_PARTS * 32) == 0 && Dq <= 8192; }
int gate_logits(ltx2_dit* c, Mod& m, const AttnW& w, const bf16* xin, int Dq, int rows, int H, hipStream_t st) {
    if (!c->gated) return LTX2_OK;
    m.glog_parts = gate_in_parts(rows, Dq) ? GATE_LOGIT_PARTS : 1;
    m.glog_bias = w.g_b;
    if (m.glog_parts > 1) return gate_logits_parts_launch(xin, Dq, w.g_w, m.glog, rows, Dq, H, st);
    return gate_logits_launch(xin, Dq, w.g_w, w.g_b, m.glog, H, rows, Dq, H, st);
}

GateRef glog(ltx2_dit* c, const Mod& m) { return c->gated ? GateRef{m.glog, m.glog_parts, m.glog_bias} : GateRef{}; }

int project_kv(ltx2_dit* c, const bf16* ctx, int rows, int Dc, const AttnW& w, int Di, int H, int hd, float eps, const float* cosb,
               const float* sinb, bf16* kv, bf16* vt, int npad, hipStream_t st, const float* k_weight = nullptr) {
    const VtOut vo{vt, Di, npad, hd};
    bool vt_done = false;
    TRY(dense(c, ctx, Dc, w.kv_w, w.kv_b, kv, 2 * Di, rows, 2 * Di, Dc, EPI_BF16, st, nullptr, 0, nullptr, &vo, &vt_done));
    const int offs[1] = {0};
    const float* wts[1] = {k_weight ? k_weight : w.kn};
    TRY(qknorm_rope_launch(kv, 2 * Di, rows, Di, hd, 1, offs, wts, eps, cosb, sinb, st));
    if (vt_done) return LTX2_OK;
    return vt_transpose_launch(kv + Di, 2 * Di, vt, rows, npad, H, st, hd);
}

int text_kv(ltx2_dit* c, int k, int l, hipStream_t st) {
    Mod& m = c->m[k];
    const BlockW& w = c->layers[l].m[k];
    const int D = m.D;
    TRY(ctx_mod_launch(m.ctx, m.ctxm, m.S, D, w.prompt_sst + D, w.prompt_sst, m.prompt_emb + D, m.prompt_emb, st));
    return project_kv(c, m.ctxm, m.S, D, w.text, D, m.H, m.hd, c->cfg.norm_eps, nullptr, nullptr, m.kv2, m.vt2, m.Spad, st, m.qfold ? m.knq + (long)l * D : nullptr);
}

inline void fold_produce(Fold& f, Mod& m, const float* scale) {
    f.shadow = m.h;
    f.ld_shadow = m.D;
    f.shadow_ss = m.rss;
    f.ld_ss = m.rss_ld;
    f.shadow_scale = scale;
}
inline void fold_consume(Fold& f, const Mod& m, float eps) {
    f.rf_parts = m.rss;
    f.ld_ss = m.rss_ld;
    f.rf_nparts = m.D / 256;
    f.rf_dim = m.D;
    f.rf_eps = eps;
}

int block_attention(ltx2_dit* c, int k, int l, long es, hipStream_t st, int fold = 0) {
    Mod& m = c->m[k];
    const BlockW& w = c->layers[l].m[k];
    const int N = m.N, D = m.D, H = m.H, hd = m.hd;
    const float eps = c->cfg.norm_eps;
    const float* const tab = m.use_comb ? m.comb + (long)l * (c->v2 ? 9 : 6) * D : w.sst;
    const float* const emb0 = m.use_comb ? nullptr : m.emb;
    auto E = [&](int r) { return emb0 ? emb0 + (long)r * D : nullptr; };
    const bool q1 = k == 0 && f8_route(c, w.self.qkv_w, N, 3 * D, D, EPI_BF16);
    const int fl = k == 0 ? fold : 0;
    TRY(norm_mod_launch(m.x, D, (q1 && !c->gated) ? nullptr : m.h, D, N, D, eps, 0, tab + D, tab, E(1), E(0), es, st, q1 ? m.a8 : nullptr, D,
                        q1 ? m.a8s : nullptr));
    TRY(gate_logits(c, m, w.self, m.h, D, N, H, st));
    const VtOut vo{m.vt, 2 * D, m.Npad, hd};
    bool vt_done = false;
    TRY(dense(c, m.h, D, w.self.qkv_w, w.self.qkv_b, m.qkv, 3 * D, N, 3 * D, D, EPI_BF16, st, nullptr, 0, nullptr, &vo, &vt_done, q1));
    {
        const int offs[2] = {0, D};
        const float* wts[2] = {w.self.qn, w.self.kn};
        TRY(qknorm_rope_launch(m.qkv, 3 * D, N, D, hd, 2, offs, wts, eps, m.cosb, m.sinb, st));
    }
    if (!vt_done) TRY(vt_transpose_launch(m.qkv + 2 * D, 3 * D, m.vt, N, m.Npad, H, st, hd));
    TRY(attend(m.qkv, 3 * D, m.qkv + D, 3 * D, m.vt, m.Npad, m.att, D, N, N, H, hd, st, nullptr, 0.f, nullptr, glog(c, m)));
    Fold fo{};
    if (fl >= 1) fold_produce(fo, m, nullptr);
    TRY(dense(c, m.att, D, w.self.o_w, w.self.o_b, m.x, D, N, D, D, EPI_RESID_GATE_F32, st, E(2), es, tab + 2 * D, nullptr, nullptr, false, nullptr, fl >= 1 ? &fo : nullptr));

    const bf16* kk;
    const bf16* vt;
    const bool q2 = k == 0 && f8_route(c, w.text.q_w, N, D, D, EPI_BF16);
    bf16* h2 = (q2 && !c->gated) ? nullptr : m.h;
    unsigned char* a8q = q2 ? m.a8 : nullptr;
    float* a8sq = q2 ? m.a8s : nullptr;
    if (c->v2) {
        TRY(norm_mod_launch(m.x, D, h2, D, N, D, eps, 0, tab + 7 * D, tab + 6 * D, E(7), E(6), es, st, a8q, D, a8sq));
        if (k == 0 && c->text_kv_ev) {
            TRY(event_wait(c->text_kv_ev, st));
            c->text_kv_ev = nullptr;
        } else {
            TRY(text_kv(c, k, l, st));
        }
        kk = m.kv2;
        vt = m.vt2;
    } else {
        if (fl < 1) TRY(norm_mod_launch(m.x, D, h2, D, N, D, eps, 0, nullptr, nullptr, nullptr, nullptr, 0, st, a8q, D, a8sq));
        kk = m.kv2 + (long)l * m.S * 2 * D;
        vt = m.vt2 + (long)l * D * m.Spad;
    }
    TRY(gate_logits(c, m, w.text, m.h, D, N, H, st));
    Fold fc{};
    fold_consume(fc, m, eps);
    TRY(dense(c, m.h, D, w.text.q_w, w.text.q_b, m.qkv, D, N, D, D, EPI_BF16, st, nullptr, 0, nullptr, nullptr, nullptr, q2, m.qfold ? m.qss : nullptr, fl >= 1 ? &fc : nullptr));
    if (!m.qfold) {
        const int offs[1] = {0};
        const float* wts[1] = {w.text.qn};
        TRY(qknorm_rope_launch(m.qkv, D, N, D, hd, 1, offs, wts, eps, nullptr, nullptr, st));
    }
    TRY(attend(m.qkv, D, kk, 2 * D, vt, m.Spad, m.att, D, N, m.S, H, hd, st, m.qfold ? m.qss : nullptr, eps,
               m.has_kmask ? m.kmask : nullptr, glog(c, m)));
    if (c->v2)
        TRY(dense(c, m.att, D, w.text.o_w, w.text.o_b, m.x, D, N, D, D, EPI_RESID_GATE_F32, st, E(8), es, tab + 8 * D));
    else
        TRY(dense(c, m.att, D, w.text.o_w, w.text.o_b, m.x, D, N, D, D, EPI_RESID_GATE_F32, st));
    return LTX2_OK;
}

int block_ffn(ltx2_dit* c, int k, int l, long es, hipStream_t st) {
    Mod& m = c->m[k];
    const BlockW& w = c->layers[l].m[k];
    const int N = m.N, D = m.D;
    const float* const tab = m.use_comb ? m.comb + (long)l * (c->v2 ? 9 : 6) * D : w.sst;
    const float* const emb0 = m.use_comb ? nullptr : m.emb;
    auto E = [&](int r) { return emb0 ? emb0 + (long)r * D : nullptr; };
    const bool q3 = k == 0 && f8_route(c, w.ff1_w, N, 4 * D, D, EPI_GELU_BF16);
    TRY(norm_mod_launch(m.x, D, q3 ? nullptr : m.h, D, N, D, c->cfg.norm_eps, 0, tab + 4 * D, tab + 3 * D, E(4), E(3), es, st,
                        q3 ? m.a8 : nullptr, D, q3 ? m.a8s : nullptr));
    TRY(dense(c, m.h, D, w.ff1_w, w.ff1_b, m.ff, 4 * D, N, 4 * D, D, EPI_GELU_BF16, st, nullptr, 0, nullptr, nullptr, nullptr, q3));
    TRY(dense(c, m.ff, 4 * D, w.ff2_w, w.ff2_b, m.x, D, N, D, 4 * D, EPI_RESID_GATE_F32, st, E(5), es, tab + 5 * D));
    return LTX2_OK;
}

int block_cross_modal(ltx2_dit* c, int l, hipStream_t st, hipStream_t sa) {
    Mod &v = c->m[0], &a = c->m[1];
    const LayerW& w = c->layers[l];
    const int Dv = v.D, Da = a.D, H = a.H, hd = a.hd;
    const float eps = c->cfg.norm_eps;
    const bool comb = c->adaln_combine;
    const float *tv = comb ? v.ca_comb + (long)l * 5 * Dv : w.ca[0], *ta = comb ? a.ca_comb + (long)l * 5 * Da : w.ca[1];
    const int offs[1] = {0};
    bf16* v_q = v.qkv;
    bf16* v_kv = v.qkv + (long)v.N * Da;
    bf16* a_kv = a.qkv;
    bf16* a_q = a.qkv + (long)a.N * 2 * Da;
    {
        const float* sct[2] = {tv, tv + 2 * Dv};
        const float* sht[2] = {tv + Dv, tv + 3 * Dv};
        const float* sce[2] = {comb ? nullptr : v.cross_ss, comb ? nullptr : v.cross_ss + 2 * Dv};
        const float* she[2] = {comb ? nullptr : v.cross_ss + Dv, comb ? nullptr : v.cross_ss + 3 * Dv};
        TRY(norm_mod2_launch(v.x, Dv, v.h, v.h2, Dv, v.N, Dv, eps, sct, sht, sce, she, st));
    }
    bool vt_done = false;
    const VtOut vo{v.vt, Da, v.Npad, hd};
    hipEvent_t video_norm = event_record(c, st);
    if (!video_norm) return LTX2_E_HIP;
    TRY(gate_logits(c, v, w.a2v, v.h, Dv, v.N, H, st));
    TRY(dense(c, v.h, Dv, w.a2v.q_w, w.a2v.q_b, v_q, Da, v.N, Da, Dv, EPI_BF16, st));
    {
        const float* wts[1] = {w.a2v.qn};
        TRY(qknorm_rope_launch(v_q, Da, v.N, Da, hd, 1, offs, wts, eps, v.ccos, v.csin, st));
    }
    {
        const float* sct[2] = {ta, ta + 2 * Da};
        const float* sht[2] = {ta + Da, ta + 3 * Da};
        const float* sce[2] = {comb ? nullptr : a.cross_ss, comb ? nullptr : a.cross_ss + 2 * Da};
        const float* she[2] = {comb ? nullptr : a.cross_ss + Da, comb ? nullptr : a.cross_ss + 3 * Da};
        TRY(norm_mod2_launch(a.x, Da, a.h, a.h2, Da, a.N, Da, eps, sct, sht, sce, she, sa));
    }
    TRY(project_kv(c, a.h, a.N, Da, w.a2v, Da, H, hd, eps, a.ccos, a.csin, a_kv, a.vt, a.Npad, sa));
    hipEvent_t audio_kv = event_record(c, sa);
    if (!audio_kv) return LTX2_E_HIP;
    TRY(gate_logits(c, a, w.v2a, a.h2, Da, a.N, H, sa));
    TRY(dense(c, a.h2, Da, w.v2a.q_w, w.v2a.q_b, a_q, Da, a.N, Da, Da, EPI_BF16, sa));
    {
        const float* wts[1] = {w.v2a.qn};
        TRY(qknorm_rope_launch(a_q, Da, a.N, Da, hd, 1, offs, wts, eps, a.ccos, a.csin, sa));
    }
    TRY(event_wait(audio_kv, st));
    TRY(attend(v_q, Da, a_kv, 2 * Da, a.vt, a.Npad, v.att, Da, v.N, a.N, H, hd, st, nullptr, 0.f, nullptr, glog(c, v)));
    TRY(dense(c, v.att, Da, w.a2v.o_w, w.a2v.o_b, v.x, Dv, v.N, Dv, Da, EPI_RESID_GATE_F32, st, comb ? nullptr : v.cross_gate, 0, tv + 4 * Dv));
    TRY(event_wait(video_norm, sa));
    TRY(dense(c, v.h2, Dv, w.v2a.kv_w, w.v2a.kv_b, v_kv, 2 * Da, v.N, 2 * Da, Dv, EPI_BF16, sa, nullptr, 0, nullptr, &vo, &vt_done));
    {
        const float* wts[1] = {w.v2a.kn};
        TRY(qknorm_rope_launch(v_kv, 2 * Da, v.N, Da, hd, 1, offs, wts, eps, v.ccos, v.csin, sa));
    }
    if (!vt_done) TRY(vt_transpose_launch(v_kv + Da, 2 * Da, v.vt, v.N, v.Npad, H, sa, hd));
    TRY(attend(a_q, Da, v_kv, 2 * Da, v.vt, v.Npad, a.att, Da, a.N, v.N, H, hd, sa, nullptr, 0.f, nullptr, glog(c, a)));
    TRY(dense(c, a.att, Da, w.v2a.o_w, w.v2a.o_b, a.x, Da, a.N, Da, Da, EPI_RESID_GATE_F32, sa, comb ? nullptr : a.cross_gate, 0, ta + 4 * Da));
    return LTX2_OK;
}

struct ModIn {
    const float* latent;
    const float* ts;
    int n_ts;
    const float* sigma;
    float* velocity;
};

int forward(ltx2_dit* c, const ModIn* in, hipStream_t st, bool rewind_events = true) {
    const int nm = c->av ? 2 : 1;
    if (rewind_events) c->sync_next = 0;
    long es[2] = {0, 0}, ee[2] = {0, 0};
    for (int k = 0; k < nm; ++k) {
        Mod& m = c->m[k];
        const ModW& w = c->mw[k];
        LTX2_CHECK_ARG(in[k].n_ts == 1 || in[k].n_ts == m.N, "dit_forward: n_timesteps=%d must be 1 or N=%d", in[k].n_ts, m.N);
        LTX2_CHECK_ARG(in[k].n_ts == 1 || c->per_token, "dit_forward: workspace was not sized for per-token timesteps");
        TRY(cast_f32_bf16_launch(in[k].latent, m.lat, (long)m.N * m.Cin, st));
        TRY(dense(c, m.lat, m.Cin, w.patch_w, w.patch_b, m.x, m.D, m.N, m.D, m.Cin, EPI_F32, st));
        TRY(adaln_chain(c, m, w.ada, in[k].ts, 1, in[k].n_ts, c->cfg.timestep_scale, m.emb, m.e_f, st));
        if (in[k].n_ts > 1) {
            es[k] = (long)w.ada.rows * m.D;
            ee[k] = m.D;
        } else if (c->adaln_combine) {
            TRY(adaln_combine_launch(m.sst_all, m.emb, m.comb, c->cfg.num_layers, (long)w.ada.rows * m.D, st));
        }
        m.use_comb = in[k].n_ts == 1 && c->adaln_combine;
        if (c->v2)
            TRY(adaln_chain(c, m, w.prompt, in[k].sigma, 0, 1, c->cfg.timestep_scale, m.prompt_emb, nullptr, st));
        if (c->av) {
            const float* cs = in[1 - k].sigma;
            TRY(adaln_chain(c, m, w.cross_ss, cs, 0, 1, c->cfg.timestep_scale, m.cross_ss, nullptr, st));
            TRY(adaln_chain(c, m, w.cross_gate, cs, 0, 1, c->cfg.av_ca_timestep_scale, m.cross_gate, nullptr, st));
            if (c->adaln_combine) {
                LTX2_CHECK_ARG(m.cross_gate == m.cross_ss + 4L * m.D, "dit_forward: cross-modal embedding rows are not contiguous");
                TRY(adaln_combine_launch(m.ca_all, m.cross_ss, m.ca_comb, c->cfg.num_layers, 5L * m.D, st));
            }
        }
    }
    const int fold = (!c->av && c->m[0].use_comb && c->fold_norms >= 1 && c->m[0].fold_max >= 1) ? 1 : 0;
    hipStream_t sa = (c->av && c->side) ? c->side : st;
    c->text_kv_ev = nullptr;
    for (int l = 0; l < c->cfg.num_layers; ++l) {
        if (c->av) {
            TRY(stream_after(c, st, sa));
            if (c->v2 && c->text_kv_ahead && sa != st && !c->fp8_compute) {
                TRY(text_kv(c, 0, l, sa));
                c->text_kv_ev = event_record(c, sa);
                if (!c->text_kv_ev) return LTX2_E_HIP;
            }
            TRY(block_attention(c, 1, l, es[1], sa));
        }
        TRY(block_attention(c, 0, l, es[0], st, fold));
        if (c->av) {
            TRY(block_cross_modal(c, l, st, sa));
            TRY(block_ffn(c, 1, l, es[1], sa));
        }
        TRY(block_ffn(c, 0, l, es[0], st));
        if (c->av) TRY(stream_after(c, sa, st));
    }
    for (int k = 0; k < nm; ++k) {
        Mod& m = c->m[k];
        const ModW& w = c->mw[k];
        TRY(norm_mod_launch(m.x, m.D, m.h, m.D, m.N, m.D, c->cfg.norm_eps, 1, w.sst_out + m.D, w.sst_out, m.e_f, m.e_f, ee[k], st));
        TRY(dense(c, m.h, m.D, w.proj_w, w.proj_b, in[k].velocity, m.Cout, m.N, m.Cout, m.D, EPI_F32, st));
    }
    return LTX2_OK;
}

struct StepIo {
    float* latent;
    const float* mask;
    const float* clean;
    float* x0_out;
};

int denoise_step(ltx2_dit* c, ModIn* in, const StepIo* io, float sigma, float sigma_next, hipStream_t st,
                 bool rewind_events = true) {
    const int nm = c->av ? 2 : 1;
    for (int k = 0; k < nm; ++k) {
        in[k].latent = io[k].latent;
        in[k].velocity = c->m[k].vel;
    }
    TRY(forward(c, in, st, rewind_events));
    for (int k = 0; k < nm; ++k) {
        Mod& m = c->m[k];
        float* x0 = io[k].x0_out ? io[k].x0_out : m.x0;
        TRY(x0_from_velocity_launch(io[k].latent, m.vel, in[k].ts, in[k].n_ts == 1 ? 0 : 1, 0.f, x0, m.N, m.Cout, st));
        TRY(euler_step_launch(io[k].latent, x0, io[k].mask, io[k].clean, sigma, sigma_next, io[k].latent, m.N, m.Cout, st));
    }
    return LTX2_OK;
}

int prepare_modality(ltx2_dit* c, int k, const float* context, int S, const float* cosb, const float* sinb,
                     const float* ccos, const float* csin, hipStream_t st) {
    Mod& m = c->m[k];
    const ModW& w = c->mw[k];
    LTX2_CHECK_ARG(context && cosb && sinb, "dit_prepare: null argument");
    LTX2_CHECK_ARG(S == m.S, "dit_prepare: S=%d differs from the bound workspace S=%d", S, m.S);
    const int D = m.D;
    const int Cctx = c->cfg.caption_channels > 0 ? c->cfg.caption_channels : D;
    bool ok = hipMemcpyAsync(m.cosb, cosb, 4L * m.N * (D / 2), hipMemcpyDeviceToDevice, st) == hipSuccess &&
              hipMemcpyAsync(m.sinb, sinb, 4L * m.N * (D / 2), hipMemcpyDeviceToDevice, st) == hipSuccess;
    if (c->av) {
        LTX2_CHECK_ARG(ccos && csin, "dit_prepare: cross-modal RoPE tables are required for AudioVideo models");
        const long Dc = c->m[1].D;
        ok = ok && hipMemcpyAsync(m.ccos, ccos, 4L * m.N * (Dc / 2), hipMemcpyDeviceToDevice, st) == hipSuccess &&
             hipMemcpyAsync(m.csin, csin, 4L * m.N * (Dc / 2), hipMemcpyDeviceToDevice, st) == hipSuccess;
    }
    if (!ok) {
        ltx2_set_error("dit_prepare: RoPE table copy failed");
        return LTX2_E_HIP;
    }
    TRY(cast_f32_bf16_launch(context, m.ctx_in, (long)S * Cctx, st));
    m.ctx = m.ctx_in;
    if (c->cfg.caption_channels > 0) {
        TRY(dense(c, m.ctx_in, Cctx, w.cap1_w, w.cap1_b, m.c1, D, S, D, Cctx, EPI_GELU_BF16, st));
        TRY(dense(c, m.c1, D, w.cap2_w, w.cap2_b, m.ctxp, D, S, D, D, EPI_BF16, st));
        m.ctx = m.ctxp;
    }
    {
        const long n = (long)(c->v2 ? 9 : 6) * D;
        for (int l = 0; l < c->cfg.num_layers; ++l)
            if (hipMemcpyAsync(m.sst_all + l * n, c->layers[l].m[k].sst, 4L * n, hipMemcpyDeviceToDevice, st) != hipSuccess) {
                ltx2_set_error("dit_prepare: scale_shift_table copy failed");
                return LTX2_E_HIP;
            }
    }
    if (c->av)
        for (int l = 0; l < c->cfg.num_layers; ++l)
            if (hipMemcpyAsync(m.ca_all + (long)l * 5 * D, c->layers[l].ca[k], 4L * 5 * D, hipMemcpyDeviceToDevice, st) != hipSuccess) {
                ltx2_set_error("dit_prepare: cross-modal scale_shift_table copy failed");
                return LTX2_E_HIP;
            }
    m.fold_max = fold_supported(c, k);
    m.qfold = text_qfold_ok(c, k);
    if (m.qfold)
        for (int l = 0; l < c->cfg.num_layers; ++l) {
            const AttnW& tw = c->layers[l].m[k].text;
            hipLaunchKernelGGL(vec_mul_kernel, dim3((D + 255) / 256), dim3(256), 0, st, tw.kn, tw.qn, m.knq + (long)l * D, D);
        }
    if (!c->v2)
        for (int l = 0; l < c->cfg.num_layers; ++l)
            TRY(project_kv(c, m.ctx, S, D, c->layers[l].m[k].text, D, m.H, m.hd, c->cfg.norm_eps, nullptr, nullptr,
                           m.kv2 + (long)l * S * 2 * D, m.vt2 + (long)l * D * m.Spad, m.Spad, st, m.qfold ? m.knq + (long)l * D : nullptr));
    return LTX2_OK;
}

int begin_capture(ltx2_dit* c, const float* host_sigmas, int n_steps, hipStream_t st) {
    LTX2_CHECK_ARG(st != nullptr, "dit_graph_capture: needs a non-default stream");
    for (int i = 0; i < n_steps; ++i) LTX2_CHECK_ARG(host_sigmas[i] != 0.f, "Sigma can't be 0.0");
    if (hipMemcpyAsync(c->sigmas_dev, host_sigmas, 4L * (n_steps + 1), hipMemcpyHostToDevice, st) != hipSuccess ||
        hipStreamSynchronize(st) != hipSuccess) {
        ltx2_set_error("dit_graph_capture: sigma upload failed");
        return LTX2_E_HIP;
    }
    if (c->exec) {
        (void)hipGraphExecDestroy(c->exec);
        c->exec = nullptr;
    }
    if (c->graph) {
        (void)hipGraphDestroy(c->graph);
        c->graph = nullptr;
    }
    if (hipStreamBeginCapture(st, hipStreamCaptureModeThreadLocal) != hipSuccess) {
        ltx2_set_error("dit_graph_capture: hipStreamBeginCapture failed");
        return LTX2_E_HIP;
    }
    return LTX2_OK;
}

int end_capture(ltx2_dit* c, int rc, hipStream_t st) {
    hipGraph_t g = nullptr;
    const hipError_t e = hipStreamEndCapture(st, &g);
    if (rc != LTX2_OK) {
        if (g) (void)hipGraphDestroy(g);
        return rc;
    }
    if (e != hipSuccess || !g) {
        ltx2_set_error("dit_graph_capture: hipStreamEndCapture failed: %s", hipGetErrorString(e));
        return LTX2_E_HIP;
    }
    c->graph = g;
    if (hipGraphInstantiate(&c->exec, g, nullptr, nullptr, 0) != hipSuccess) {
        ltx2_set_error("dit_graph_capture: hipGraphInstantiate failed");
        return LTX2_E_HIP;
    }
    return LTX2_OK;
}

int check_ready(ltx2_dit* c, const char* who, bool want_av) {
    LTX2_CHECK_ARG(c, "%s: null context", who);
    LTX2_CHECK_ARG(c->av == want_av, "%s: model is %s", who, c->av ? "AudioVideo (use the *_av entry points)" : "VideoOnly");
    if (!c->prepared) {
        ltx2_set_error("%s: ltx2_dit_prepare has not been called", who);
        return LTX2_E_STATE;
    }
    return LTX2_OK;
}

int bind(ltx2_dit* c, void* ptr, int64_t bytes, int N, int S, int Na, int Sa, int per_token) {
    LTX2_CHECK_ARG(((uintptr_t)ptr & 255) == 0, "dit_bind_workspace: pointer must be 256-byte aligned");
    const long need = carve(c, (char*)ptr, N, S, Na, Sa, per_token);
    if (bytes < need) {
        ltx2_set_error("dit_bind_workspace: %ld bytes given, %ld needed", (long)bytes, need);
        return LTX2_E_STATE;
    }
    c->ws = (char*)ptr;
    c->ws_bytes = bytes;
    const int n[2] = {N, Na}, s[2] = {S, Sa};
    for (int k = 0; k < 2; ++k) {
        c->m[k].N = n[k];
        c->m[k].S = s[k];
        c->m[k].Npad = (int)align_up(n[k], 64);
        c->m[k].Spad = (int)align_up(s[k], 64);
    }
    c->per_token = per_token;
    c->prepared = false;
    c->m[0].has_kmask = c->m[1].has_kmask = false;
    return LTX2_OK;
}

}

extern "C" {

int ltx2_dit_create(const ltx2_dit_config* cfg, ltx2_dit** out) {
    LTX2_CHECK_ARG(cfg && out, "dit_create: null argument");
    LTX2_CHECK_ARG(cfg->head_dim == 128 || cfg->head_dim == 64, "dit_create: head_dim=%d, only 128 and 64 are implemented", cfg->head_dim);
    LTX2_CHECK_ARG(cfg->num_layers > 0 && cfg->num_heads > 0, "dit_create: bad layer/head count");
    LTX2_CHECK_ARG(cfg->in_channels % 64 == 0, "dit_create: in_channels must be a multiple of 64");
    LTX2_CHECK_ARG(cfg->caption_channels % 64 == 0, "dit_create: caption_channels must be a multiple of 64");
    LTX2_CHECK_ARG(cfg->model_type == LTX2_MODEL_VIDEO_ONLY || cfg->model_type == LTX2_MODEL_AUDIO_VIDEO, "dit_create: bad model_type %d", cfg->model_type);
    ltx2_dit* c = new ltx2_dit();
    c->cfg = *cfg;
    c->av = cfg->model_type == LTX2_MODEL_AUDIO_VIDEO;
    c->v2 = cfg->cross_attention_adaln != 0;
    c->gated = cfg->apply_gated_attention != 0;
    Mod& v = c->m[0];
    v.H = cfg->num_heads;
    v.hd = cfg->head_dim;
    v.D = v.H * v.hd;
    v.Cin = cfg->in_channels;
    v.Cout = cfg->out_channels;
    if (c->av) {
        if (!(cfg->audio_head_dim == 64 && cfg->audio_heads == cfg->num_heads && cfg->audio_in_channels % 64 == 0)) {
            delete c;
            ltx2_set_error("dit_create: AudioVideo needs audio_head_dim = 64, audio_heads = num_heads (shared cross-modal RoPE heads) and audio_in_channels %% 64 == 0");
            return LTX2_E_INVALID;
        }
        Mod& a = c->m[1];
        a.H = cfg->audio_heads;
        a.hd = cfg->audio_head_dim;
        a.D = a.H * a.hd;
        a.Cin = cfg->audio_in_channels;
        a.Cout = cfg->audio_out_channels;
    }
    if (c->av) {
        const bool ok = hipStreamCreateWithFlags(&c->side, hipStreamNonBlocking) == hipSuccess;
        if (!ok) {
            ltx2_set_error("dit_create: side stream / event creation failed");
            return LTX2_E_HIP;
        }
    }
    *out = c;
    return LTX2_OK;
}

void ltx2_dit_destroy(ltx2_dit* c) {
    if (!c) return;
    for (hipEvent_t e : c->sync_ev) (void)hipEventDestroy(e);
    if (c->side) (void)hipStreamDestroy(c->side);
    if (c->exec) (void)hipGraphExecDestroy(c->exec);
    if (c->graph) (void)hipGraphDestroy(c->graph);
    for (hipEvent_t e : c->prof_ev) (void)hipEventDestroy(e);
    delete c;
}

int ltx2_dit_set_weight(ltx2_dit* c, const char* name, const void* ptr, int dtype, int64_t numel) {
    LTX2_CHECK_ARG(c && name && ptr, "dit_set_weight: null argument");
    LTX2_CHECK_ARG(dtype == LTX2_DTYPE_BF16 || dtype == LTX2_DTYPE_F32 || dtype == LTX2_DTYPE_FP8_E4M3FN, "dit_set_weight: bad dtype %d", dtype);
    c->weights[name] = Wt{ptr, dtype, (long)numel};
    c->resolved = false;
    c->prepared = false;
    return LTX2_OK;
}

int64_t ltx2_dit_workspace_bytes_av(const ltx2_dit* c, int N, int S, int Na, int Sa, int per_token) {
    if (!c || N <= 0 || S <= 0 || (c->av && (Na <= 0 || Sa <= 0))) return -1;
    ltx2_dit tmp;
    tmp.cfg = c->cfg;
    tmp.av = c->av;
    tmp.v2 = c->v2;
    tmp.gated = c->gated;
    tmp.fp8_compute = c->fp8_compute;
    tmp.m[0] = c->m[0];
    tmp.m[1] = c->m[1];
    return carve(&tmp, nullptr, N, S, Na, Sa, per_token);
}

int64_t ltx2_dit_workspace_bytes(const ltx2_dit* c, int N, int S, int per_token) {
    if (!c || c->av) return -1;
    return ltx2_dit_workspace_bytes_av(c, N, S, 0, 0, per_token);
}

int ltx2_dit_bind_workspace(ltx2_dit* c, void* ptr, int64_t bytes, int N, int S, int per_token) {
    LTX2_CHECK_ARG(c && ptr && N > 0 && S > 0, "dit_bind_workspace: bad argument");
    LTX2_CHECK_ARG(!c->av, "dit_bind_workspace: AudioVideo model, use ltx2_dit_bind_workspace_av");
    return bind(c, ptr, bytes, N, S, 0, 0, per_token);
}

int ltx2_dit_bind_workspace_av(ltx2_dit* c, void* ptr, int64_t bytes, int N, int S, int Na, int Sa, int per_token) {
    LTX2_CHECK_ARG(c && ptr && N > 0 && S > 0 && Na > 0 && Sa > 0, "dit_bind_workspace_av: bad argument");
    LTX2_CHECK_ARG(c->av, "dit_bind_workspace_av: VideoOnly model, use ltx2_dit_bind_workspace");
    return bind(c, ptr, bytes, N, S, Na, Sa, per_token);
}

int ltx2_dit_prepare(ltx2_dit* c, const float* context, int S, const float* rope_cos, const float* rope_sin,
                     void* stream) {
    LTX2_CHECK_ARG(c, "dit_prepare: null context");
    LTX2_CHECK_ARG(!c->av, "dit_prepare: AudioVideo model, use ltx2_dit_prepare_av");
    if (!c->ws) {
        ltx2_set_error("dit_prepare: no workspace bound");
        return LTX2_E_STATE;
    }
    TRY(resolve(c));
    TRY(prepare_modality(c, 0, context, S, rope_cos, rope_sin, nullptr, nullptr, (hipStream_t)stream));
    c->prepared = true;
    return LTX2_OK;
}

int ltx2_dit_prepare_av(ltx2_dit* c, const float* v_context, int S, const float* v_cos, const float* v_sin,
                        const float* v_cross_cos, const float* v_cross_sin, const float* a_context, int Sa,
                        const float* a_cos, const float* a_sin, const float* a_cross_cos, const float* a_cross_sin,
                        void* stream) {
    LTX2_CHECK_ARG(c, "dit_prepare_av: null context");
    LTX2_CHECK_ARG(c->av, "dit_prepare_av: VideoOnly model, use ltx2_dit_prepare");
    if (!c->ws) {
        ltx2_set_error("dit_prepare_av: no workspace bound");
        return LTX2_E_STATE;
    }
    TRY(resolve(c));
    TRY(prepare_modality(c, 0, v_context, S, v_cos, v_sin, v_cross_cos, v_cross_sin, (hipStream_t)stream));
    TRY(prepare_modality(c, 1, a_context, Sa, a_cos, a_sin, a_cross_cos, a_cross_sin, (hipStream_t)stream));
    c->prepared = true;
    return LTX2_OK;
}

int ltx2_dit_forward(ltx2_dit* c, const float* latent, const float* timesteps, int n_timesteps, const float* sigma,
                     float* velocity, void* stream) {
    LTX2_CHECK_ARG(latent && timesteps && velocity, "dit_forward: null argument");
    TRY(check_ready(c, "dit_forward", false));
    ModIn in[1] = {{latent, timesteps, n_timesteps, sigma ? sigma : timesteps, velocity}};
    return forward(c, in, (hipStream_t)stream);
}

int ltx2_dit_forward_av(ltx2_dit* c, const float* v_latent, const float* v_timesteps, int n_v_timesteps,
                        const float* v_sigma, const float* a_latent, const float* a_timesteps, int n_a_timesteps,
                        const float* a_sigma, float* v_velocity, float* a_velocity, void* stream) {
    LTX2_CHECK_ARG(v_latent && v_timesteps && v_sigma && a_latent && a_timesteps && a_sigma && v_velocity && a_velocity,
                   "dit_forward_av: null argument");
    TRY(check_ready(c, "dit_forward_av", true));
    ModIn in[2] = {{v_latent, v_timesteps, n_v_timesteps, v_sigma, v_velocity},
                   {a_latent, a_timesteps, n_a_timesteps, a_sigma, a_velocity}};
    return forward(c, in, (hipStream_t)stream);
}

int ltx2_dit_denoise_step(ltx2_dit* c, float* latent, const float* timesteps, int n_timesteps, const float* sigma_dev,
                          const float* mask, const float* clean, float sigma, float sigma_next, float* x0_out, void* stream) {
    LTX2_CHECK_ARG(latent && timesteps, "dit_denoise_step: null argument");
    TRY(check_ready(c, "dit_denoise_step", false));
    ModIn in[1] = {{latent, timesteps, n_timesteps, sigma_dev ? sigma_dev : timesteps, nullptr}};
    const StepIo io[1] = {{latent, mask, clean, x0_out}};
    return denoise_step(c, in, io, sigma, sigma_next, (hipStream_t)stream);
}

int ltx2_dit_denoise_step_av(ltx2_dit* c, float* v_latent, float* a_latent, const float* v_timesteps, int n_v_timesteps,
                             const float* a_timesteps, int n_a_timesteps, const float* sigma_dev, const float* v_mask,
                             const float* v_clean, const float* a_mask, const float* a_clean, float sigma,
                             float sigma_next, float* v_x0_out, float* a_x0_out, void* stream) {
    LTX2_CHECK_ARG(v_latent && a_latent && v_timesteps && a_timesteps && sigma_dev, "dit_denoise_step_av: null argument");
    TRY(check_ready(c, "dit_denoise_step_av", true));
    ModIn in[2] = {{v_latent, v_timesteps, n_v_timesteps, sigma_dev, nullptr},
                   {a_latent, a_timesteps, n_a_timesteps, sigma_dev, nullptr}};
    const StepIo io[2] = {{v_latent, v_mask, v_clean, v_x0_out}, {a_latent, a_mask, a_clean, a_x0_out}};
    return denoise_step(c, in, io, sigma, sigma_next, (hipStream_t)stream);
}

int ltx2_dit_graph_capture(ltx2_dit* c, float* latent, const float* host_sigmas, int n_steps, void* stream) {
    LTX2_CHECK_ARG(latent && host_sigmas && n_steps > 0 && n_steps < 64, "dit_graph_capture: bad argument");
    TRY(check_ready(c, "dit_graph_capture", false));
    hipStream_t st = (hipStream_t)stream;
    TRY(begin_capture(c, host_sigmas, n_steps, st));
    int rc = LTX2_OK;
    for (int i = 0; i < n_steps && rc == LTX2_OK; ++i) {
        ModIn in[1] = {{latent, c->sigmas_dev + i, 1, c->sigmas_dev + i, nullptr}};
        const StepIo io[1] = {{latent, nullptr, nullptr, nullptr}};
        rc = denoise_step(c, in, io, host_sigmas[i], host_sigmas[i + 1], st, i == 0);
    }
    return end_capture(c, rc, st);
}

namespace {
int cond_modality(ltx2_dit* c, int k, const float* mask, long n_mask, const float* clean, long n_clean, const float* sigma_i, ModIn& in, StepIo& io, hipStream_t st) {
    Mod& m = c->m[k];
    if (!mask) return LTX2_OK;
    LTX2_CHECK_ARG(clean, "dit_graph_capture_cond: a denoise mask needs the clean latent");
    LTX2_CHECK_ARG(n_mask == m.N && n_clean == (long)m.N * m.Cout, "dit_graph_capture_cond: modality %d has %d tokens x %d channels, got a mask of %ld and a clean latent of %ld elements", k, m.N, m.Cout, n_mask, n_clean);
    if (!c->per_token || !m.ts_tok) {
        ltx2_set_error("dit_graph_capture_cond: the workspace was not bound for per-token timesteps");
        return LTX2_E_STATE;
    }
    hipLaunchKernelGGL(mask_sigma_kernel, dim3((m.N + 255) / 256), dim3(256), 0, st, mask, sigma_i, m.ts_tok, m.N);
    LTX2_CHECK_LAUNCH("mask_sigma_kernel");
    in.ts = m.ts_tok;
    in.n_ts = m.N;
    io.mask = mask;
    io.clean = clean;
    return LTX2_OK;
}
}

int ltx2_dit_graph_capture_cond(ltx2_dit* c, float* latent, const float* host_sigmas, int n_steps, const float* mask, int64_t n_mask, const float* clean,
                                int64_t n_clean, void* stream) {
    LTX2_CHECK_ARG(latent && host_sigmas && n_steps > 0 && n_steps < 64, "dit_graph_capture_cond: bad argument");
    TRY(check_ready(c, "dit_graph_capture_cond", false));
    hipStream_t st = (hipStream_t)stream;
    TRY(begin_capture(c, host_sigmas, n_steps, st));
    int rc = LTX2_OK;
    for (int i = 0; i < n_steps && rc == LTX2_OK; ++i) {
        ModIn in[1] = {{latent, c->sigmas_dev + i, 1, c->sigmas_dev + i, nullptr}};
        StepIo io[1] = {{latent, nullptr, nullptr, nullptr}};
        rc = cond_modality(c, 0, mask, n_mask, clean, n_clean, c->sigmas_dev + i, in[0], io[0], st);
        if (rc == LTX2_OK) rc = denoise_step(c, in, io, host_sigmas[i], host_sigmas[i + 1], st, i == 0);
    }
    return end_capture(c, rc, st);
}

int ltx2_dit_graph_capture_cond_av(ltx2_dit* c, float* v_latent, float* a_latent, const float* host_sigmas, int n_steps, const float* v_mask, int64_t n_v_mask,
                                   const float* v_clean, int64_t n_v_clean, const float* a_mask, int64_t n_a_mask, const float* a_clean, int64_t n_a_clean, void* stream) {
    LTX2_CHECK_ARG(v_latent && a_latent && host_sigmas && n_steps > 0 && n_steps < 64, "dit_graph_capture_cond_av: bad argument");
    TRY(check_ready(c, "dit_graph_capture_cond_av", true));
    hipStream_t st = (hipStream_t)stream;
    TRY(begin_capture(c, host_sigmas, n_steps, st));
    int rc = LTX2_OK;
    for (int i = 0; i < n_steps && rc == LTX2_OK; ++i) {
        const float* s = c->sigmas_dev + i;
        ModIn in[2] = {{v_latent, s, 1, s, nullptr}, {a_latent, s, 1, s, nullptr}};
        StepIo io[2] = {{v_latent, nullptr, nullptr, nullptr}, {a_latent, nullptr, nullptr, nullptr}};
        rc = cond_modality(c, 0, v_mask, n_v_mask, v_clean, n_v_clean, s, in[0], io[0], st);
        if (rc == LTX2_OK) rc = cond_modality(c, 1, a_mask, n_a_mask, a_clean, n_a_clean, s, in[1], io[1], st);
        if (rc == LTX2_OK) rc = denoise_step(c, in, io, host_sigmas[i], host_sigmas[i + 1], st, i == 0);
    }
    return end_capture(c, rc, st);
}

int ltx2_dit_graph_capture_av(ltx2_dit* c, float* v_latent, float* a_latent, const float* host_sigmas, int n_steps,
                              void* stream) {
    LTX2_CHECK_ARG(v_latent && a_latent && host_sigmas && n_steps > 0 && n_steps < 64, "dit_graph_capture_av: bad argument");
    TRY(check_ready(c, "dit_graph_capture_av", true));
    hipStream_t st = (hipStream_t)stream;
    TRY(begin_capture(c, host_sigmas, n_steps, st));
    int rc = LTX2_OK;
    for (int i = 0; i < n_steps && rc == LTX2_OK; ++i) {
        const float* s = c->sigmas_dev + i;
        ModIn in[2] = {{v_latent, s, 1, s, nullptr}, {a_latent, s, 1, s, nullptr}};
        const StepIo io[2] = {{v_latent, nullptr, nullptr, nullptr}, {a_latent, nullptr, nullptr, nullptr}};
        rc = denoise_step(c, in, io, host_sigmas[i], host_sigmas[i + 1], st, i == 0);
    }
    return end_capture(c, rc, st);
}

int ltx2_dit_profile_begin(ltx2_dit* c, int epilogue) {
    LTX2_CHECK_ARG(c && epilogue >= -1 && epilogue < EPI_COUNT, "dit_profile_begin: bad argument");
    c->prof_epi = epilogue;
    c->prof_used = 0;
    c->prof_flops = 0;
    g_prof_ctx = c;
    return LTX2_OK;
}

int ltx2_dit_profile_end(ltx2_dit* c, double* total_ms, int64_t* launches, double* flops) {
    LTX2_CHECK_ARG(c && total_ms && launches && flops, "dit_profile_end: null argument");
    g_prof_ctx = nullptr;
    c->prof_epi = -2;
    double tot = 0;
    for (size_t i = 0; i + 1 < c->prof_used; i += 2) {
        if (hipEventSynchronize(c->prof_ev[i + 1]) != hipSuccess) {
            ltx2_set_error("dit_profile_end: event synchronize failed");
            return LTX2_E_HIP;
        }
        float ms = 0;
        (void)hipEventElapsedTime(&ms, c->prof_ev[i], c->prof_ev[i + 1]);
        tot += ms;
    }
    *total_ms = tot;
    *launches = (int64_t)(c->prof_used / 2);
    *flops = c->prof_flops;
    return LTX2_OK;
}

int ltx2_dit_set_context_mask(ltx2_dit* c, int modality, const float* mask, int S, void* stream) {
    LTX2_CHECK_ARG(c && (modality == 0 || (modality == 1 && c->av)), "dit_set_context_mask: bad context / modality");
    Mod& m = c->m[modality];
    if (!c->ws) {
        ltx2_set_error("dit_set_context_mask: no workspace bound");
        return LTX2_E_STATE;
    }
    if (!mask) {
        m.has_kmask = false;
        return LTX2_OK;
    }
    LTX2_CHECK_ARG(S == m.S, "dit_set_context_mask: S=%d differs from the bound workspace S=%d", S, m.S);
    TRY(keymask_words_launch(mask, S, m.kmask, m.Spad / 64, (hipStream_t)stream));
    m.has_kmask = true;
    return LTX2_OK;
}

int ltx2_dit_set_option(ltx2_dit* c, const char* name, int value) {
    LTX2_CHECK_ARG(c && name, "dit_set_option: null argument");
    if (!strcmp(name, "fp8_compute")) {
        if (c->ws && (value != 0) != c->fp8_compute) {
            ltx2_set_error("dit_set_option: fp8_compute must be set before the workspace is bound");
            return LTX2_E_STATE;
        }
        c->fp8_compute = value != 0;
        return LTX2_OK;
    }
    if (!strcmp(name, "text_kv_ahead")) {
        c->text_kv_ahead = value != 0;
        return LTX2_OK;
    }
    if (!strcmp(name, "fold_norms")) {
        LTX2_CHECK_ARG(value == 0 || value == 1, "dit_set_option: fold_norms is 0 or 1");
        c->fold_norms = value;
        return LTX2_OK;
    }
    if (!strcmp(name, "adaln_combine")) {
        c->adaln_combine = value != 0;
        return LTX2_OK;
    }
    ltx2_set_error("dit_set_option: unknown option '%s'", name);
    return LTX2_E_INVALID;
}


int ltx2_dit_graph_launch(ltx2_dit* c, void* stream) {
    LTX2_CHECK_ARG(c, "dit_graph_launch: null context");
    if (!c->exec) {
        ltx2_set_error("dit_graph_launch: no captured graph");
        return LTX2_E_STATE;
    }
    if (hipGraphLaunch(c->exec, (hipStream_t)stream) != hipSuccess) {
        ltx2_set_error("dit_graph_launch: hipGraphLaunch failed");
        return LTX2_E_HIP;
    }
    return LTX2_OK;
}

}
```

ltx-2-mlx_amd/kernels.py:

```python
from __future__ import annotations

import math
from typing import Optional, Tuple

import torch

from . import _native as nv

BF16 = torch.bfloat16
F16 = torch.float16
ACT16 = (BF16, F16)


def _L(*tensors, dtype=None):
    for t in tensors:
        if t is not None and t.dtype in ACT16:
            return nv.lib(t.dtype)
    return nv.lib(dtype)


def _c(t: torch.Tensor) -> torch.Tensor:
    return t if t.is_contiguous() else t.contiguous()


def gemm(a: torch.Tensor, w: torch.Tensor, bias: Optional[torch.Tensor] = None, epilogue: int = nv.EPI_BF16,
         out: Optional[torch.Tensor] = None, gate: Optional[torch.Tensor] = None,
         gate_table: Optional[torch.Tensor] = None, res: Optional[torch.Tensor] = None) -> torch.Tensor:
    assert a.dtype in ACT16 and w.dtype == a.dtype and a.dim() == 2 and w.dim() == 2
    a, w = _c(a), _c(w)
    M, K = a.shape
    N = w.shape[0]
    if out is None:
        odt = torch.float32 if epilogue in (nv.EPI_F32, nv.EPI_RESID_GATE_F32) else a.dtype
        assert epilogue != nv.EPI_RESID_GATE_F32, "RESID_GATE accumulates into `out`; pass it"
        out = torch.empty(M, N, device=a.device, dtype=odt)
    gs = 0
    if gate is not None:
        gate = _c(gate)
        gs = 0 if gate.shape[0] == 1 else gate.stride(0)
    nv.check(_L(a).ltx2_gemm_bf16(nv.ptr(a), a.stride(0), nv.ptr(w), nv.ptr(bias), nv.ptr(out), out.stride(0), M, N, K,
                                     epilogue, nv.ptr(gate), gs, nv.ptr(gate_table), nv.ptr(res),
                                     res.stride(0) if res is not None else 0, nv.stream()))
    return out


def gemm_qkv_vt(a: torch.Tensor, w: torch.Tensor, bias: Optional[torch.Tensor], heads: int, head_dim: int = 128):
    assert a.dtype in ACT16 and w.dtype == a.dtype
    a, w = _c(a), _c(w)
    M, K = a.shape
    N = w.shape[0]
    D = heads * head_dim
    assert N == 3 * D
    npad = (M + 63) // 64 * 64
    out = torch.empty(M, N, device=a.device, dtype=a.dtype)
    vt = torch.empty(heads, head_dim, npad, device=a.device, dtype=a.dtype)
    import ctypes
    fused = ctypes.c_int(0)
    nv.check(_L(a).ltx2_gemm_qkv_vt(nv.ptr(a), a.stride(0), nv.ptr(w), nv.ptr(bias), nv.ptr(out), out.stride(0), M, N, K,
                                       nv.ptr(vt), 2 * D, npad, head_dim, ctypes.byref(fused), nv.stream()))
    return out, vt, bool(fused.value)


def adaln_rmsnorm2(x: torch.Tensor, scale0, shift0, scale1, shift1, eps: float = 1e-6, dtype: torch.dtype = BF16):
    x = _c(x.float())
    o0 = torch.empty(x.shape, device=x.device, dtype=dtype)
    o1 = torch.empty_like(o0)
    nv.check(nv.lib(dtype).ltx2_adaln_rmsnorm2(nv.ptr(x), x.stride(0), nv.ptr(o0), nv.ptr(o1), o0.stride(0), x.shape[0], x.shape[1], eps,
                                               nv.ptr(scale0), nv.ptr(shift0), nv.ptr(scale1), nv.ptr(shift1), nv.stream()))
    return o0, o1


def gemm_rowss(a: torch.Tensor, w: torch.Tensor, bias: Optional[torch.Tensor] = None):
    assert a.dtype in ACT16 and w.dtype == a.dtype
    a, w = _c(a), _c(w)
    M, K = a.shape
    N = w.shape[0]
    out = torch.empty(M, N, device=a.device, dtype=a.dtype)
    rowss = torch.zeros(M, max(N // 64, 1), device=a.device, dtype=torch.float32)
    import ctypes
    written = ctypes.c_int(0)
    nv.check(_L(a).ltx2_gemm_bf16_rowss(nv.ptr(a), a.stride(0), nv.ptr(w), nv.ptr(bias), nv.ptr(out), out.stride(0), M, N, K, nv.ptr(rowss),
                                        ctypes.byref(written), nv.stream()))
    return out, (rowss if written.value else None)


def gemm_fold(a: torch.Tensor, w: torch.Tensor, bias: Optional[torch.Tensor], epilogue: int, out: Optional[torch.Tensor] = None,
              gate_table: Optional[torch.Tensor] = None, shadow: Optional[torch.Tensor] = None, shadow_scale: Optional[torch.Tensor] = None,
              rf_parts: Optional[torch.Tensor] = None, rf_dim: int = 0, eps: float = 1e-6):
    import ctypes
    assert a.dtype in ACT16 and w.dtype == a.dtype
    a, w = _c(a), _c(w)
    M, K = a.shape
    N = w.shape[0]
    prod = epilogue == nv.EPI_RESID_GATE_F32
    if out is None:
        out = torch.empty(M, N, device=a.device, dtype=a.dtype)
    ss = torch.zeros(max(N // 256, 1), (M + 255) // 256 * 256 + 256, device=a.device, dtype=torch.float32) if (prod and shadow is not None) else None
    sup = ctypes.c_int(0)
    nv.check(_L(a).ltx2_gemm_bf16_fold(nv.ptr(a), a.stride(0), nv.ptr(w), nv.ptr(bias), nv.ptr(out), out.stride(0), M, N, K, epilogue, nv.ptr(gate_table),
                                       nv.ptr(shadow), shadow.stride(0) if shadow is not None else 0, nv.ptr(shadow_scale), nv.ptr(ss),
                                       ss.stride(0) if ss is not None else 0,
                                       nv.ptr(rf_parts), rf_parts.stride(0) if rf_parts is not None else 0, rf_parts.shape[0] if rf_parts is not None else 0,
                                       rf_dim, eps, ctypes.byref(sup), nv.stream()))
    if not sup.value:
        return None
    return (out, ss) if prod else out


def flash_attn_rowscale(q: torch.Tensor, k: torch.Tensor, vt: torch.Tensor, heads: int, nkv: int, q_ss: torch.Tensor, eps: float = 1e-6,
                        scale: Optional[float] = None) -> torch.Tensor:
    assert q.dtype in ACT16 and q_ss.dtype == torch.float32 and q_ss.is_contiguous()
    nq, hd = q.shape[0], vt.shape[1]
    out = torch.empty(nq, heads * hd, device=q.device, dtype=q.dtype)
    if scale is None:
        scale = 1.0 / math.sqrt(float(hd))
    nv.check(_L(q).ltx2_flash_attn_rowscale(nv.ptr(q), q.stride(0), nv.ptr(k), k.stride(0), nv.ptr(vt), vt.shape[2], nv.ptr(out), out.stride(0), nq, nkv,
                                            heads, hd, scale, nv.ptr(q_ss), q_ss.shape[1], heads * hd, eps, nv.stream()))
    return out


def flash_attn_gated(q: torch.Tensor, k: torch.Tensor, vt: torch.Tensor, heads: int, nkv: int, gate_logits: torch.Tensor,
                     scale: Optional[float] = None) -> torch.Tensor:
    assert q.dtype in ACT16 and gate_logits.dtype == torch.float32 and gate_logits.stride(1) == 1
    nq, hd = q.shape[0], vt.shape[1]
    out = torch.empty(nq, heads * hd, device=q.device, dtype=q.dtype)
    if scale is None:
        scale = 1.0 / math.sqrt(float(hd))
    nv.check(_L(q).ltx2_flash_attn_gated(nv.ptr(q), q.stride(0), nv.ptr(k), k.stride(0), nv.ptr(vt), vt.shape[2], nv.ptr(out), out.stride(0), nq, nkv,
                                         heads, hd, scale, nv.ptr(gate_logits), gate_logits.stride(0), nv.stream()))
    return out


def flash_attn_gated_parts(q: torch.Tensor, k: torch.Tensor, vt: torch.Tensor, heads: int, nkv: int, x: torch.Tensor, gate_w: torch.Tensor,
                           gate_b: torch.Tensor, scale: Optional[float] = None) -> torch.Tensor:
    assert q.dtype in ACT16 and x.dtype == q.dtype and gate_w.dtype == q.dtype and x.stride(1) == 1
    nq, hd = q.shape[0], vt.shape[1]
    out = torch.empty(nq, heads * hd, device=q.device, dtype=q.dtype)
    parts = torch.empty(8, nq, heads, device=q.device, dtype=torch.float32)
    if scale is None:
        scale = 1.0 / math.sqrt(float(hd))
    nv.check(_L(q).ltx2_flash_attn_gated_parts(nv.ptr(q), q.stride(0), nv.ptr(k), k.stride(0), nv.ptr(vt), vt.shape[2], nv.ptr(out), out.stride(0), nq, nkv,
                                               heads, hd, scale, nv.ptr(x), x.stride(0), nv.ptr(_c(gate_w)), nv.ptr(_c(gate_b.float())), x.shape[1], nv.ptr(parts),
                                               nv.stream()))
    return out


def flash_attn_keymask(q: torch.Tensor, k: torch.Tensor, vt: torch.Tensor, heads: int, nkv: int, mask: torch.Tensor,
                       scale: Optional[float] = None) -> torch.Tensor:
    assert q.dtype in ACT16 and mask.numel() == nkv
    nq, hd = q.shape[0], vt.shape[1]
    out = torch.empty(nq, heads * hd, device=q.device, dtype=q.dtype)
    f = (mask.reshape(-1).to(q.device) != 0).to(torch.float32).contiguous()
    words = torch.empty(vt.shape[2] // 64, device=q.device, dtype=torch.int64)
    if scale is None:
        scale = 1.0 / math.sqrt(float(hd))
    nv.check(_L(q).ltx2_flash_attn_keymask(nv.ptr(q), q.stride(0), nv.ptr(k), k.stride(0), nv.ptr(vt), vt.shape[2], nv.ptr(out), out.stride(0), nq, nkv,
                                           heads, hd, scale, nv.ptr(f), nv.ptr(words), nv.stream()))
    return out


def gemm_w8a16(a: torch.Tensor, w8: torch.Tensor, wscale: torch.Tensor, bias: Optional[torch.Tensor] = None, epilogue: int = nv.EPI_BF16,
               out: Optional[torch.Tensor] = None, gate_table: Optional[torch.Tensor] = None) -> torch.Tensor:
    assert a.dtype in ACT16 and w8.element_size() == 1 and wscale.dtype == torch.float32 and a.dim() == 2 and w8.dim() == 2
    a, w8, wscale = _c(a), _c(w8), _c(wscale)
    M, K = a.shape
    N = w8.shape[0]
    assert wscale.numel() == N
    if out is None:
        assert epilogue != nv.EPI_RESID_GATE_F32, "RESID_GATE accumulates into `out`; pass it"
        out = torch.empty(M, N, device=a.device, dtype=torch.float32 if epilogue == nv.EPI_F32 else a.dtype)
    nv.check(_L(a).ltx2_gemm_w8a16(nv.ptr(a), a.stride(0), nv.ptr(w8), nv.ptr(wscale), nv.ptr(bias), nv.ptr(out), out.stride(0), M, N, K,
                                      epilogue, None, 0, nv.ptr(gate_table), nv.stream()))
    return out


def quantize_rows_fp8(x: torch.Tensor) -> Tuple[torch.Tensor, torch.Tensor]:
    assert x.dtype in ACT16 and x.dim() == 2
    x = _c(x)
    R, K = x.shape
    codes = torch.empty(R, K, device=x.device, dtype=torch.uint8)
    scale = torch.empty(R, device=x.device, dtype=torch.float32)
    nv.check(_L(x).ltx2_quantize_rows_fp8(nv.ptr(x), x.stride(0), R, K, nv.ptr(codes), K, nv.ptr(scale), nv.stream()))
    return codes, scale


def gemm_fp8(a8: torch.Tensor, ascale: torch.Tensor, w8: torch.Tensor, wscale: torch.Tensor, bias: Optional[torch.Tensor] = None,
             epilogue: int = nv.EPI_BF16, out: Optional[torch.Tensor] = None, gate: Optional[torch.Tensor] = None,
             gate_table: Optional[torch.Tensor] = None) -> torch.Tensor:
    assert a8.element_size() == 1 and w8.element_size() == 1 and a8.dim() == 2 and w8.dim() == 2
    assert ascale.dtype == torch.float32 and wscale.dtype == torch.float32
    a8, w8, ascale, wscale = _c(a8), _c(w8), _c(ascale), _c(wscale)
    M, K = a8.shape
    N = w8.shape[0]
    assert ascale.numel() == M and wscale.numel() == N and w8.shape[1] == K
    if out is None:
        assert epilogue != nv.EPI_RESID_GATE_F32, "RESID_GATE accumulates into `out`; pass it"
        out = torch.empty(M, N, device=a8.device, dtype=torch.float32 if epilogue == nv.EPI_F32 else BF16)
    gs = 0
    if gate is not None:
        gate = _c(gate)
        gs = 0 if gate.shape[0] == 1 else gate.stride(0)
    nv.check(nv.lib().ltx2_gemm_fp8(nv.ptr(a8), a8.stride(0), nv.ptr(ascale), nv.ptr(w8), nv.ptr(wscale), nv.ptr(bias), nv.ptr(out), out.stride(0),
                                    M, N, K, epilogue, nv.ptr(gate), gs, nv.ptr(gate_table), nv.stream()))
    return out


def gemm_fp8_qkv_vt(a8, ascale, w8, wscale, bias, heads: int, head_dim: int = 128):
    a8, w8, ascale, wscale = _c(a8), _c(w8), _c(ascale), _c(wscale)
    M, K = a8.shape
    N = w8.shape[0]
    D = heads * head_dim
    assert N == 3 * D
    npad = (M + 63) // 64 * 64
    out = torch.empty(M, N, device=a8.device, dtype=BF16)
    vt = torch.empty(heads, head_dim, npad, device=a8.device, dtype=BF16)
    import ctypes
    fused = ctypes.c_int(0)
    nv.check(nv.lib().ltx2_gemm_fp8_qkv_vt(nv.ptr(a8), a8.stride(0), nv.ptr(ascale), nv.ptr(w8), nv.ptr(wscale), nv.ptr(bias), nv.ptr(out),
                                           out.stride(0), M, N, K, nv.ptr(vt), 2 * D, npad, head_dim, ctypes.byref(fused), nv.stream()))
    return out, vt, bool(fused.value)


def gemv(a: torch.Tensor, w: torch.Tensor, bias: Optional[torch.Tensor], act_in: int = 0, act_out: int = 0) -> torch.Tensor:
    assert a.dtype == torch.float32 and w.dtype in ACT16
    a, w = _c(a), _c(w)
    M, K = a.shape
    N = w.shape[0]
    out = torch.empty(M, N, device=a.device, dtype=torch.float32)
    nv.check(_L(w).ltx2_gemv_f32(nv.ptr(a), a.stride(0), nv.ptr(w), nv.ptr(bias), nv.ptr(out), N, M, N, K, act_in,
                                    act_out, nv.stream()))
    return out


def conv_weight_to_engine(w: torch.Tensor, d2s_stride: Optional[Tuple[int, int, int]] = None, dtype: torch.dtype = BF16) -> torch.Tensor:
    cout, cin = w.shape[0], w.shape[1]
    e = w.permute(0, 2, 3, 4, 1).reshape(cout, 27, cin)
    if d2s_stride is not None:
        sp = d2s_stride[0] * d2s_stride[1] * d2s_stride[2]
        cf = cout // sp
        e = e.reshape(cf, sp, 27, cin).permute(1, 0, 2, 3).reshape(cout, 27, cin)
    return e.to(dtype).contiguous()


def conv_bias_to_engine(b: torch.Tensor, d2s_stride: Optional[Tuple[int, int, int]] = None) -> torch.Tensor:
    if d2s_stride is not None:
        sp = d2s_stride[0] * d2s_stride[1] * d2s_stride[2]
        b = b.reshape(-1, sp).t().reshape(-1)
    return b.float().contiguous()


def conv3d(x: torch.Tensor, w_engine: torch.Tensor, bias: Optional[torch.Tensor], causal: bool = False, mode: int = 0,
           res: Optional[torch.Tensor] = None, stride: Tuple[int, int, int] = (1, 1, 1), residual: bool = False,
           pad_zero: int = 0) -> torch.Tensor:
    assert x.dtype in ACT16 and x.dim() == 4 and w_engine.dtype == x.dtype
    x = _c(x)
    T, H, W, Cin = x.shape
    Cout = w_engine.shape[0]
    kt = w_engine.shape[1] // 9
    ft, fh, fw = stride
    if mode == 2:
        sp = ft * fh * fw
        out = torch.empty(T * ft - (1 if ft > 1 else 0), H * fh, W * fw, Cout // sp, device=x.device, dtype=x.dtype)
    else:
        out = torch.empty(T, H, W, Cout, device=x.device, dtype=x.dtype)
    nv.check(_L(x).ltx2_conv3d_fused(nv.ptr(x), nv.ptr(w_engine), nv.ptr(bias), nv.ptr(out), T, H, W, Cin, Cout,
                                        int(causal), mode, nv.ptr(res), ft, fh, fw, int(residual), int(pad_zero), kt,
                                        nv.stream()))
    return out


def conv2d_weight_to_engine(w: torch.Tensor, pixel_shuffle: int = 0, dtype: torch.dtype = BF16) -> torch.Tensor:
    cout, cin = w.shape[0], w.shape[1]
    e = w.permute(0, 2, 3, 1).reshape(cout, 9, cin)
    if pixel_shuffle:
        sp = pixel_shuffle * pixel_shuffle
        e = e.reshape(cout // sp, sp, 9, cin).permute(1, 0, 2, 3).reshape(cout, 9, cin)
    return e.to(dtype).contiguous()


def groupnorm_silu(x: torch.Tensor, gamma: torch.Tensor, beta: torch.Tensor, groups: int = 32, eps: float = 1e-5,
                   res: Optional[torch.Tensor] = None, act: bool = True) -> torch.Tensor:
    assert x.dtype in ACT16 and x.is_contiguous()
    C = x.shape[-1]
    P = x.numel() // C
    y = torch.empty_like(x)
    sums = torch.empty(2 * groups * (1 + (P + 15) // 16), device=x.device, dtype=torch.float32)
    nv.check(_L(x).ltx2_groupnorm_silu(nv.ptr(x), nv.ptr(res), nv.ptr(y), P, C, groups, eps, nv.ptr(_c(gamma.float())),
                                          nv.ptr(_c(beta.float())), nv.ptr(sums), int(act), nv.stream()))
    return y


def s2d_downsample(y: torch.Tensor, x: torch.Tensor, stride: Tuple[int, int, int]) -> torch.Tensor:
    assert y.dtype in ACT16 and x.dtype == y.dtype and y.shape[:3] == x.shape[:3]
    y, x = _c(y), _c(x)
    T, H, W, Cc = y.shape
    st, sh, sw = stride
    out = torch.empty(T // st, H // sh, W // sw, Cc * st * sh * sw, device=y.device, dtype=y.dtype)
    nv.check(_L(y).ltx2_s2d_downsample(nv.ptr(y), nv.ptr(x), nv.ptr(out), T, H, W, Cc, x.shape[3], st, sh, sw, nv.stream()))
    return out


def latent_unnormalize_nhwc(latent: torch.Tensor, mean: torch.Tensor, std: torch.Tensor, dtype: torch.dtype = BF16) -> torch.Tensor:
    assert latent.dtype == torch.float32 and latent.dim() == 4
    latent = _c(latent)
    C, T, H, W = latent.shape
    out = torch.empty(T, H, W, C, device=latent.device, dtype=dtype)
    nv.check(nv.lib(dtype).ltx2_vae_prepare_latent(nv.ptr(latent), nv.ptr(_c(std.float())), nv.ptr(_c(mean.float())), None, 0.0,
                                              nv.ptr(out), C, T * H * W, nv.stream()))
    return out


def latent_normalize_nchw(x: torch.Tensor, mean: torch.Tensor, std: torch.Tensor) -> torch.Tensor:
    assert x.dtype in ACT16 and x.dim() == 4 and x.is_contiguous()
    T, H, W, C = x.shape
    out = torch.empty(C, T, H, W, device=x.device, dtype=torch.float32)
    nv.check(_L(x).ltx2_latent_normalize_nchw(nv.ptr(x), nv.ptr(_c(mean.float())), nv.ptr(_c(std.float())), nv.ptr(out), C,
                                                 T * H * W, nv.stream()))
    return out


def adaln_rmsnorm(x: torch.Tensor, eps: float = 1e-6, layer_norm: bool = False,
                  scale_tab: Optional[torch.Tensor] = None, shift_tab: Optional[torch.Tensor] = None,
                  scale_emb: Optional[torch.Tensor] = None, shift_emb: Optional[torch.Tensor] = None,
                  emb_stride: int = 0, dtype: torch.dtype = BF16) -> torch.Tensor:
    assert x.dtype == torch.float32 and x.dim() == 2
    x = _c(x)
    rows, D = x.shape
    out = torch.empty(rows, D, device=x.device, dtype=dtype)
    nv.check(nv.lib(dtype).ltx2_adaln_rmsnorm(nv.ptr(x), D, nv.ptr(out), D, rows, D, eps, int(layer_norm), nv.ptr(scale_tab),
                                         nv.ptr(shift_tab), nv.ptr(scale_emb), nv.ptr(shift_emb), emb_stride, nv.stream()))
    return out


def adaln_rmsnorm_fp8(x: torch.Tensor, eps: float = 1e-6, layer_norm: bool = False, scale_tab: Optional[torch.Tensor] = None,
                      shift_tab: Optional[torch.Tensor] = None, scale_emb: Optional[torch.Tensor] = None,
                      shift_emb: Optional[torch.Tensor] = None, emb_stride: int = 0, want_bf16: bool = True):
    assert x.dtype == torch.float32 and x.dim() == 2
    x = _c(x)
    rows, D = x.shape
    out = torch.empty(rows, D, device=x.device, dtype=BF16) if want_bf16 else None
    codes = torch.empty(rows, D, device=x.device, dtype=torch.uint8)
    scale = torch.empty(rows, device=x.device, dtype=torch.float32)
    nv.check(nv.lib().ltx2_adaln_rmsnorm_fp8(nv.ptr(x), D, nv.ptr(out), D, nv.ptr(codes), D, nv.ptr(scale), rows, D, eps, int(layer_norm),
                                             nv.ptr(scale_tab), nv.ptr(shift_tab), nv.ptr(scale_emb), nv.ptr(shift_emb), emb_stride, nv.stream()))
    return out, codes, scale


def qknorm_rope_(buf: torch.Tensor, D: int, head_dim: int, q_off: int, q_weight: torch.Tensor,
                 k_off: int = 0, k_weight: Optional[torch.Tensor] = None, eps: float = 1e-6,
                 cos: Optional[torch.Tensor] = None, sin: Optional[torch.Tensor] = None) -> torch.Tensor:
    assert buf.dtype in ACT16 and buf.dim() == 2 and buf.is_contiguous()
    nv.check(_L(buf).ltx2_qknorm_rope(nv.ptr(buf), buf.stride(0), buf.shape[0], D, head_dim, q_off, nv.ptr(q_weight),
                                       k_off, nv.ptr(k_weight), eps, nv.ptr(cos), nv.ptr(sin), nv.stream()))
    return buf


def vt_transpose(v: torch.Tensor, heads: int, head_dim: int = 128) -> torch.Tensor:
    assert v.dtype in ACT16 and v.dim() == 2 and v.stride(1) == 1
    nkv = v.shape[0]
    npad = (nkv + 63) // 64 * 64
    vt = torch.empty(heads, head_dim, npad, device=v.device, dtype=v.dtype)
    nv.check(_L(v).ltx2_vt_transpose(nv.ptr(v), v.stride(0), nv.ptr(vt), nkv, npad, heads, head_dim, nv.stream()))
    return vt


def flash_attn(q: torch.Tensor, k: torch.Tensor, vt: torch.Tensor, heads: int, nkv: int,
               scale: Optional[float] = None) -> torch.Tensor:
    assert q.dtype in ACT16 and k.dtype == q.dtype and vt.dtype == q.dtype and q.stride(1) == 1 and k.stride(1) == 1
    nq, hd = q.shape[0], vt.shape[1]
    out = torch.empty(nq, heads * hd, device=q.device, dtype=q.dtype)
    if scale is None:
        scale = 1.0 / math.sqrt(float(hd))
    nv.check(_L(q).ltx2_flash_attn(nv.ptr(q), q.stride(0), nv.ptr(k), k.stride(0), nv.ptr(vt), vt.shape[2], nv.ptr(out),
                                      out.stride(0), nq, nkv, heads, hd, scale, nv.stream()))
    return out


def attn_head_gate_(att: torch.Tensor, x: torch.Tensor, gate_w: torch.Tensor, gate_b: torch.Tensor, heads: int) -> torch.Tensor:
    assert att.dtype in ACT16 and x.dtype == att.dtype and gate_w.dtype == att.dtype and att.is_contiguous() and x.stride(1) == 1
    rows, hd = att.shape[0], att.shape[1] // heads
    logits = torch.empty(rows, heads, device=att.device, dtype=torch.float32)
    nv.check(_L(att).ltx2_attn_head_gate(nv.ptr(att), att.stride(0), nv.ptr(x), x.stride(0), nv.ptr(_c(gate_w)), nv.ptr(_c(gate_b.float())),
                                          nv.ptr(logits), rows, x.shape[1], heads, hd, nv.stream()))
    return logits


def rope_tables(positions: torch.Tensor, dim: int, theta: float, max_pos) -> Tuple[torch.Tensor, torch.Tensor]:
    pos = _c(positions[0].float())
    n_dims, N = pos.shape[0], pos.shape[1]
    if n_dims != len(max_pos):
        raise ValueError(f"Number of position dimensions ({n_dims}) must match max_pos length ({len(max_pos)})")
    n_freq = dim // (2 * n_dims)
    grid = (torch.tensor(float(theta)) ** torch.linspace(0.0, 1.0, n_freq, dtype=torch.float32) * (math.pi / 2)).float().to(pos.device)
    mp = torch.tensor([float(m) for m in max_pos], device=pos.device)
    cos = torch.empty(N, dim // 2, device=pos.device, dtype=torch.float32)
    sin = torch.empty_like(cos)
    nv.check(nv.lib().ltx2_rope_tables(nv.ptr(pos), nv.ptr(grid), nv.ptr(mp), N, n_dims, n_freq, dim // 2, nv.ptr(cos), nv.ptr(sin),
                                       nv.stream()))
    return cos, sin


def timestep_sinusoid(t: torch.Tensor, mult: float, dim: int = 256) -> torch.Tensor:
    t = _c(t.float())
    out = torch.empty(t.numel(), dim, device=t.device, dtype=torch.float32)
    nv.check(nv.lib().ltx2_timestep_sinusoid(nv.ptr(t), 1, mult, t.numel(), dim, nv.ptr(out), None, nv.stream()))
    return out


def dequant_fp8(w: torch.Tensor, scale: float, dtype: torch.dtype = BF16) -> torch.Tensor:
    raw = w.view(torch.uint8) if w.dtype != torch.uint8 else w
    raw = _c(raw)
    out = torch.empty(raw.shape, device=raw.device, dtype=dtype)
    nv.check(nv.lib(dtype).ltx2_dequant_fp8_e4m3fn(nv.ptr(raw), float(scale), nv.ptr(out), raw.numel(), nv.stream()))
    return out


def cast_bf16(x: torch.Tensor, dtype: torch.dtype = BF16) -> torch.Tensor:
    x = _c(x.float())
    out = torch.empty(x.shape, device=x.device, dtype=dtype)
    nv.check(nv.lib(dtype).ltx2_cast_f32_bf16(nv.ptr(x), nv.ptr(out), x.numel(), nv.stream()))
    return out


def x0_from_velocity(latent: torch.Tensor, velocity: torch.Tensor, timesteps: torch.Tensor) -> torch.Tensor:
    latent, velocity, timesteps = _c(latent), _c(velocity), _c(timesteps.float())
    n, c = latent.shape
    out = torch.empty_like(latent)
    stride = 0 if timesteps.numel() == 1 else 1
    nv.check(nv.lib().ltx2_x0_from_velocity(nv.ptr(latent), nv.ptr(velocity), nv.ptr(timesteps), stride, 0.0, nv.ptr(out),
                                            n, c, nv.stream()))
    return out


def euler_step(x: torch.Tensor, x0: torch.Tensor, sigma: float, sigma_next: float,
               mask: Optional[torch.Tensor] = None, clean: Optional[torch.Tensor] = None) -> torch.Tensor:
    x, x0 = _c(x), _c(x0)
    n, c = x.shape
    out = torch.empty_like(x)
    nv.check(nv.lib().ltx2_euler_step(nv.ptr(x), nv.ptr(x0), nv.ptr(mask), nv.ptr(clean), float(sigma), float(sigma_next),
                                      nv.ptr(out), n, c, nv.stream()))
    return out


def pixnorm_mod_silu(x: torch.Tensor, table: torch.Tensor, te: Optional[torch.Tensor], shift_row: int, scale_row: int,
                     eps: float = 1e-6) -> torch.Tensor:
    assert x.dtype in ACT16
    x = _c(x)
    C_ = x.shape[-1]
    P = x.numel() // C_
    y = torch.empty_like(x)
    nv.check(_L(x).ltx2_pixnorm_mod_silu(nv.ptr(x), nv.ptr(y), P, C_, eps, nv.ptr(table), nv.ptr(te), shift_row,
                                            scale_row, nv.stream()))
    return y


def video_chunk_to_uint8(cur: torch.Tensor, frames: torch.Tensor, t_dst0: int, prev: Optional[torch.Tensor] = None,
                         ramp: Optional[torch.Tensor] = None) -> None:
    cur = _c(cur.float())
    _, Tc, H, W = cur.shape
    ov = 0 if prev is None else int(ramp.numel())
    if prev is not None:
        prev, ramp = _c(prev.float()), _c(ramp.float())
    nv.check(nv.lib().ltx2_video_chunk_to_uint8(nv.ptr(cur), nv.ptr(prev), nv.ptr(ramp), nv.ptr(frames), Tc, 0 if prev is None else prev.shape[1], ov,
                                                H, W, int(t_dst0), frames.shape[0], nv.stream()))


def tile_blend_accumulate(tile: torch.Tensor, nt: int, nh: int, nw: int, mt: torch.Tensor, mh: torch.Tensor, mw: torch.Tensor,
                          out: torch.Tensor, wsum: torch.Tensor, t0: int, h0: int, w0: int) -> None:
    tile = _c(tile.float())
    _, dt, dh, dw = tile.shape
    _, OT, OH, OW = out.shape
    nv.check(nv.lib().ltx2_tile_blend_accumulate(nv.ptr(tile), dt, dh, dw, nt, nh, nw, nv.ptr(_c(mt.float())), nv.ptr(_c(mh.float())),
                                                 nv.ptr(_c(mw.float())), nv.ptr(out), nv.ptr(wsum), OT, OH, OW, t0, h0, w0, nv.stream()))


def tile_blend_finish(out: torch.Tensor, wsum: torch.Tensor) -> None:
    nv.check(nv.lib().ltx2_tile_blend_finish(nv.ptr(out), nv.ptr(wsum), wsum.numel(), nv.stream()))


def video_to_uint8(video: torch.Tensor) -> torch.Tensor:
    video = _c(video.float())
    _, T, H, W = video.shape
    out = torch.empty(T, H, W, 3, device=video.device, dtype=torch.uint8)
    nv.check(nv.lib().ltx2_video_to_uint8(nv.ptr(video), nv.ptr(out), T, H, W, nv.stream()))
    return out



def gemma_attn(q: torch.Tensor, k: torch.Tensor, v: torch.Tensor, heads: int, kv_heads: int, causal: bool = True, window: int = 0,
               scale: Optional[float] = None, out: Optional[torch.Tensor] = None) -> torch.Tensor:
    assert q.dtype == BF16 and k.dtype == BF16 and v.dtype == BF16 and q.stride(1) == 1 and k.stride(1) == 1 and v.stride(1) == 1
    tq, tkv = q.shape[0], k.shape[0]
    if out is None:
        out = torch.empty(tq, heads * 256, device=q.device, dtype=BF16)
    if scale is None:
        scale = 256 ** -0.5
    nv.check(nv.lib().ltx2_gemma_attn(nv.ptr(q), q.stride(0), nv.ptr(k), k.stride(0), nv.ptr(v), v.stride(0), nv.ptr(out), out.stride(0),
                                      tq, tkv, heads, kv_heads, int(bool(causal)), int(window), float(scale), nv.stream()))
    return out


def gemma_qknorm_rope_(qkv: torch.Tensor, q_heads: int, kv_heads: int, q_w: torch.Tensor, k_w: torch.Tensor, cos: torch.Tensor,
                       sin: torch.Tensor, eps: float = 1e-6) -> torch.Tensor:
    assert qkv.dtype == BF16 and qkv.stride(1) == 1 and cos.dtype == torch.float32 and sin.dtype == torch.float32
    assert cos.shape == (qkv.shape[0], 128) and sin.shape == cos.shape and cos.is_contiguous() and sin.is_contiguous()
    nv.check(nv.lib().ltx2_gemma_qknorm_rope(nv.ptr(qkv), qkv.stride(0), qkv.shape[0], q_heads, kv_heads, nv.ptr(_c(q_w.float())),
                                             nv.ptr(_c(k_w.float())), float(eps), nv.ptr(cos), nv.ptr(sin), nv.stream()))
    return qkv


def gemma_resid_norm(x_in: torch.Tensor, y: Optional[torch.Tensor], w_post: Optional[torch.Tensor], w_next: Optional[torch.Tensor],
                     x_out: Optional[torch.Tensor] = None, h_out: Optional[torch.Tensor] = None, hf_out: Optional[torch.Tensor] = None,
                     eps: float = 1e-6) -> None:
    assert x_in.dtype == torch.float32 and x_in.stride(1) == 1
    rows, d = x_in.shape
    for t in (x_out, hf_out):
        assert t is None or (t.dtype == torch.float32 and t.shape == (rows, d) and t.stride(1) == 1)
    assert h_out is None or (h_out.dtype == BF16 and h_out.shape == (rows, d) and h_out.stride(1) == 1)
    assert y is None or (y.dtype == BF16 and y.shape == (rows, d) and y.stride(1) == 1)
    nv.check(nv.lib().ltx2_gemma_resid_norm(nv.ptr(x_in), x_in.stride(0), nv.ptr(y), y.stride(0) if y is not None else 0, nv.ptr(w_post),
                                            nv.ptr(w_next), nv.ptr(x_out), x_out.stride(0) if x_out is not None else 0, nv.ptr(h_out),
                                            h_out.stride(0) if h_out is not None else 0, nv.ptr(hf_out),
                                            hf_out.stride(0) if hf_out is not None else 0, rows, d, float(eps), nv.stream()))


def gemma_gated_act(gu: torch.Tensor, inter: int, act: int = nv.GEMMA_ACT_SILU, out: Optional[torch.Tensor] = None) -> torch.Tensor:
    assert gu.dtype == BF16 and gu.stride(1) == 1
    if out is None:
        out = torch.empty(gu.shape[0], inter, device=gu.device, dtype=BF16)
    nv.check(nv.lib().ltx2_gemma_gated_act(nv.ptr(gu), gu.stride(0), nv.ptr(out), out.stride(0), gu.shape[0], inter, int(act), nv.stream()))
    return out


def gemma_embed(ids: torch.Tensor, table: torch.Tensor, scale: float, out: Optional[torch.Tensor] = None) -> torch.Tensor:
    assert table.dtype == BF16 and table.is_contiguous() and ids.dtype == torch.int32 and ids.is_contiguous()
    vocab, d = table.shape
    if out is None:
        out = torch.empty(ids.shape[0], d, device=table.device, dtype=torch.float32)
    nv.check(nv.lib().ltx2_gemma_embed(nv.ptr(ids), ids.shape[0], nv.ptr(table), vocab, d, float(scale), nv.ptr(out), out.stride(0), nv.stream()))
    return out


def _layer_strides(states) -> Optional[Tuple[int, int]]:
    s0 = states[0]
    if any(s.shape != s0.shape or s.dtype != torch.float32 or s.device != s0.device or s.stride() != s0.stride() for s in states):
        return None
    if s0.stride(1) != 1 or s0.stride(0) % 4 or s0.stride(0) < s0.shape[1]:
        return None
    if len(states) == 1:
        return 0, s0.stride(0)
    step = states[1].data_ptr() - s0.data_ptr()
    if step <= 0 or step % 16 or any(states[i + 1].data_ptr() - states[i].data_ptr() != step for i in range(len(states) - 1)):
        return None
    same = s0.untyped_storage().data_ptr()
    if any(s.untyped_storage().data_ptr() != same for s in states):
        return None
    return step // 4, s0.stride(0)


def gemma_features_rms(hidden_states, valid: Optional[torch.Tensor] = None, eps: float = 1e-6, dtype: torch.dtype = BF16,
                       out: Optional[torch.Tensor] = None) -> torch.Tensor:
    states = list(hidden_states.unbind(0)) if isinstance(hidden_states, torch.Tensor) else list(hidden_states)
    assert states and all(s.dim() == 2 and s.is_cuda for s in states)
    strides = _layer_strides(states)
    if strides is None:
        stacked = torch.stack([s.float() for s in states])
        states, strides = list(stacked.unbind(0)), (stacked.stride(0), stacked.stride(1))
    nl, (t, d) = len(states), states[0].shape
    if out is None:
        out = torch.empty(t, nl * d, device=states[0].device, dtype=dtype)
    assert out.dtype == dtype and dtype in ACT16 and out.shape == (t, nl * d) and out.stride(1) == 1
    if valid is not None:
        valid = _c(valid.to(states[0].device, torch.int32).reshape(-1))
        assert valid.shape[0] == t
    nv.check(nv.lib(dtype).ltx2_gemma_features_rms(nv.ptr(states[0]), strides[0], strides[1], nv.ptr(valid), nv.ptr(out), out.stride(0), t, nl, d,
                                                   float(eps), nv.stream()))
    return out



def _f32(*ts):
    for t in ts:
        assert t is None or (t.dtype == torch.float32 and t.is_cuda and t.stride(-1) == 1), "audio kernels take CUDA fp32 tensors with unit channel stride"


def pack_conv_weight(w: torch.Tensor) -> torch.Tensor:
    w = w.float()
    if w.dim() == 3:
        w = w[:, :, None, :]
    cout, cin, kh, kw = w.shape
    packed = torch.zeros(kh * kw * cin, (cout + 3) // 4 * 4, device=w.device, dtype=torch.float32)
    packed[:, :cout] = w.permute(2, 3, 1, 0).reshape(kh * kw * cin, cout)
    return packed


def pack_conv_transpose_weight(w: torch.Tensor, rate: int) -> torch.Tensor:
    w = w.float()
    cin, cout, k = w.shape
    ntaps = (k + rate - 1) // rate
    packed = torch.zeros(rate, ntaps, cin, (cout + 3) // 4 * 4, device=w.device, dtype=torch.float32)
    for ph in range(rate):
        for t in range(ntaps):
            j = ph + rate * (ntaps - 1 - t)
            if j < k:
                packed[ph, t, :, :cout] = w[:, :, j]
    return packed


def audio_conv1d(x: torch.Tensor, w: torch.Tensor, bias: Optional[torch.Tensor], c_out: int, k: int, *, stride: int = 1, dilation: int = 1,
                 padding: int = 0, t_out: Optional[int] = None, out: Optional[torch.Tensor] = None, prologue: int = nv.AUDIO_PRO_NONE,
                 slope: float = 0.0, res: Optional[torch.Tensor] = None, alpha: float = 1.0, beta: float = 0.0, act: int = nv.AUDIO_ACT_NONE,
                 c_in: Optional[int] = None) -> torch.Tensor:
    c_in = x.shape[1] if c_in is None else c_in
    T = x.shape[0]
    if t_out is None:
        t_out = (T + 2 * padding - dilation * (k - 1) - 1) // stride + 1
    if out is None:
        out = torch.empty(t_out, c_out, device=x.device, dtype=torch.float32)
    _f32(x, w, bias, out, res)
    assert w.shape[0] == k * c_in and out.shape[0] >= t_out
    nv.check(nv.lib().ltx2_audio_conv(nv.ptr(x), x.stride(0), 1, T, c_in, nv.ptr(w), w.stride(0), nv.ptr(bias), nv.ptr(out), out.stride(0), 1, t_out,
                                      c_out, 1, k, stride, dilation, 0, padding, 0, int(prologue), float(slope), nv.ptr(res),
                                      res.stride(0) if res is not None else 0, float(alpha), float(beta), int(act), nv.stream()))
    return out


def audio_conv2d(x: torch.Tensor, w: torch.Tensor, bias: Optional[torch.Tensor], c_out: int, kh: int, kw: int, pad_h: int, pad_w: int, *,
                 upsample: bool = False, out: Optional[torch.Tensor] = None, res: Optional[torch.Tensor] = None) -> torch.Tensor:
    H, W, c_in = x.shape
    if upsample:
        h_out, w_out = 2 * H + pad_h - kh, 2 * W + 2 * pad_w - kw + 1
    else:
        h_out, w_out = H + pad_h - kh + 1, W + 2 * pad_w - kw + 1
    if out is None:
        out = torch.empty(h_out, w_out, c_out, device=x.device, dtype=torch.float32)
    assert x.is_contiguous() and out.is_contiguous() and (res is None or res.is_contiguous())
    _f32(x, w, bias, out, res)
    nv.check(nv.lib().ltx2_audio_conv(nv.ptr(x), c_in, H, W, c_in, nv.ptr(w), w.stride(0), nv.ptr(bias), nv.ptr(out), c_out, h_out, w_out, c_out,
                                      kh, kw, 1, 1, pad_h, pad_w, 1 if upsample else 0, nv.AUDIO_PRO_NONE, 0.0, nv.ptr(res),
                                      c_out if res is not None else 0, 1.0, 0.0, nv.AUDIO_ACT_NONE, nv.stream()))
    return out


def audio_conv_transpose1d(x: torch.Tensor, w_phase: torch.Tensor, bias: Optional[torch.Tensor], c_out: int, k: int, rate: int, padding: int,
                           prologue: int = nv.AUDIO_PRO_NONE, slope: float = 0.0) -> torch.Tensor:
    T, c_in = x.shape
    t_out = (T - 1) * rate + k - 2 * padding
    out = torch.empty(t_out, c_out, device=x.device, dtype=torch.float32)
    _f32(x, w_phase, bias, out)
    assert w_phase.is_contiguous() and tuple(w_phase.shape[:3]) == (rate, (k + rate - 1) // rate, c_in)
    nv.check(nv.lib().ltx2_audio_conv_transpose1d(nv.ptr(x), x.stride(0), T, c_in, nv.ptr(w_phase), nv.ptr(bias), nv.ptr(out), out.stride(0), t_out,
                                                  c_out, k, rate, padding, int(prologue), float(slope), nv.stream()))
    return out


def audio_pixnorm_silu(x: torch.Tensor, eps: float = 1e-6, out: Optional[torch.Tensor] = None) -> torch.Tensor:
    assert x.is_contiguous()
    _f32(x)
    c = x.shape[-1]
    if out is None:
        out = torch.empty_like(x)
    nv.check(nv.lib().ltx2_audio_pixnorm_silu(nv.ptr(x), c, nv.ptr(out), c, x.numel() // c, c, float(eps), nv.stream()))
    return out


def audio_snake_aa(x: torch.Tensor, alpha: torch.Tensor, beta: torch.Tensor, up_filter: torch.Tensor, down_filter: torch.Tensor,
                   out: Optional[torch.Tensor] = None) -> torch.Tensor:
    T, c = x.shape
    if out is None:
        out = torch.empty(T, c, device=x.device, dtype=torch.float32)
    _f32(x, alpha, beta, up_filter, down_filter, out)
    nv.check(nv.lib().ltx2_audio_snake_aa(nv.ptr(x), x.stride(0), T, c, nv.ptr(alpha), nv.ptr(beta), nv.ptr(up_filter), up_filter.numel(),
                                          nv.ptr(down_filter), down_filter.numel(), nv.ptr(out), out.stride(0), nv.stream()))
    return out


def audio_upsample(x: torch.Tensor, filt: torch.Tensor, ratio: int, pad: int, pad_left: int, t_out: int) -> torch.Tensor:
    T, c = x.shape
    out = torch.empty(t_out, c, device=x.device, dtype=torch.float32)
    _f32(x, filt, out)
    nv.check(nv.lib().ltx2_audio_upsample(nv.ptr(x), x.stride(0), T, c, nv.ptr(filt), filt.numel(), ratio, pad, pad_left, nv.ptr(out), out.stride(0),
                                          t_out, nv.stream()))
    return out
```

Baseline: 13.60 steps/s.

## Add paired attention form processing two head/q-tile units per workgroup

Adds a PAIR variant of the flash attention kernel in which each workgroup processes two (head, q-tile) units back to back. The K/V prefetch for the second unit is issued during the last tile of the first, and its Q is loaded before the first unit's epilogue. Auto mode selects this when qtiles*H exceeds twice the CU count, aiming to cut tail and launch-wave overhead and hide the prologue latency. Costs are added register pressure, since qraw is live, and more complex indexing.

```diff
diff --git a/include/ltx2hip.h b/include/ltx2hip.h
--- a/include/ltx2hip.h
+++ b/include/ltx2hip.h
@@ -103,6 +103,8 @@
 
 int ltx2_vt_transpose(const void* V, int64_t ld, void* VT, int Nkv, int Npad, int H, int head_dim, void* stream);
 
+#define LTX2_ATTN_FORM_ONE_UNIT 0x100
+#define LTX2_ATTN_FORM_PAIRED 0x200
 int ltx2_flash_attn(const void* Q, int64_t ldq, const void* K, int64_t ldk, const void* VT, int Npad, void* out,
                     int64_t ldo, int Nq, int Nkv, int H, int head_dim, float scale, void* stream);
 
diff --git a/ltx-2-mlx_amd/csrc/attention.h b/ltx-2-mlx_amd/csrc/attention.h
--- a/ltx-2-mlx_amd/csrc/attention.h
+++ b/ltx-2-mlx_amd/csrc/attention.h
@@ -1,5 +1,11 @@
 #pragma once
 #include "common.h"
+
+enum {
+    ATTN_FORM_AUTO = 0,
+    ATTN_FORM_ONE_UNIT = 1,
+    ATTN_FORM_PAIRED = 2,
+};
 
 struct AttnParams {
     const bf16* Q;
@@ -18,6 +24,7 @@
     int gate_ld;
     int gate_parts;
     const float* gate_bias;
+    int form;
 };
 
 int attn_launch(const AttnParams& p, hipStream_t stream);
diff --git a/ltx-2-mlx_amd/csrc/attention.hip b/ltx-2-mlx_amd/csrc/attention.hip
--- a/ltx-2-mlx_amd/csrc/attention.hip
+++ b/ltx-2-mlx_amd/csrc/attention.hip
@@ -81,11 +81,12 @@
 __device__ unsigned long long ltx2_at_counts[2];
 #endif
 
-template <int HD, bool QS = false, bool KM = false, int NW = 4>
+template <int HD, bool QS = false, bool KM = false, int NW = 4, bool PAIR = false>
 __global__ __launch_bounds__(NW * 64, NW == 4 ? 2 : 1) void attn_fwd_kernel(const AttnParams p) {
     using G = Geo<HD>;
     constexpr int K_TILE = G::K_TILE, STAGE = G::STAGE, NJ = G::NJ * 4 / NW, QB = NW * 32;
     static_assert(NW == 4 || (NW == 8 && HD == 128), "waves per workgroup");
+    static_assert(!PAIR || (HD == 128 && NW == 4), "the paired form exists for head_dim 128, 4 waves");
     constexpr int NKS = HD / 32, NDB = HD / 16;
     constexpr int NK = 4 * NKS, NV = 2 * NDB;
     constexpr int DK = AT_DK < NK ? AT_DK : NK, DV = AT_DV < NV ? AT_DV : NV;
@@ -117,25 +118,58 @@
     for (int kk = 0; kk < 2; ++kk) v_lane[kk] = lds0 + K_TILE + l15 * 128 + (((4 * kk + g) ^ v_xor) << 4);
 
     int head = blockIdx.y, qt = blockIdx.x;
+    [[maybe_unused]] int head_n = 0, qt_n = 0, nu = 1;
+    if constexpr (PAIR) {
+        const int b = blockIdx.x, T = (p.Nq + QB - 1) / QB;
 #if AT_XCD
-    if ((gridDim.y & 7) == 0) {
-        const int b = blockIdx.y * gridDim.x + blockIdx.x, xcd = b & 7, idx = b >> 3;
-        head = xcd + 8 * (idx / (int)gridDim.x);
-        qt = idx % (int)gridDim.x;
-    }
-#endif
+        if ((p.H & 7) == 0) {
+            const int xcd = b & 7, pi = b >> 3, hj = p.H >> 3, np = (hj >> 1) * T;
+            if (pi < np) {
+                const int m = pi / T;
+                head = xcd + 16 * m;
+                qt = pi - m * T;
+                head_n = head + 8;
+                qt_n = qt;
+                nu = 2;
+            } else {
+                head = head_n = xcd + 8 * (hj - 1);
+                qt = 2 * (pi - np);
+                qt_n = qt + 1;
+                nu = qt_n < T ? 2 : 1;
+            }
+        } else
+#endif
+        {
+            const int u = 2 * b;
+            head = u / T;
+            qt = u - head * T;
+            head_n = (u + 1) / T;
+            qt_n = (u + 1) - head_n * T;
+            nu = u + 1 < p.H * T ? 2 : 1;
+        }
+    } else {
+#if AT_XCD
+        if ((gridDim.y & 7) == 0) {
+            const int b = blockIdx.y * gridDim.x + blockIdx.x, xcd = b & 7, idx = b >> 3;
+            head = xcd + 8 * (idx / (int)gridDim.x);
+            qt = idx % (int)gridDim.x;
+        }
+#endif
+    }
     const int tb = nt;
-    const int q0 = qt * QB + wv * 32;
-
-    const __amdgpu_buffer_rsrc_t rk = __builtin_amdgcn_make_buffer_rsrc((void*)(p.K + head * HD), 0, (int)k_bytes, 0x00020000);
-    const __amdgpu_buffer_rsrc_t rv = __builtin_amdgcn_make_buffer_rsrc((void*)(p.VT + (long)head * p.vt_head_stride), 0, (int)v_bytes, 0x00020000);
+    int q0 = qt * QB + wv * 32;
+
+    auto k_rsrc = [&](int h) { return __builtin_amdgcn_make_buffer_rsrc((void*)(p.K + h * HD), 0, (int)k_bytes, 0x00020000); };
+    auto v_rsrc = [&](int h) { return __builtin_amdgcn_make_buffer_rsrc((void*)(p.VT + (long)h * p.vt_head_stride), 0, (int)v_bytes, 0x00020000); };
+    __amdgpu_buffer_rsrc_t rk_pre = k_rsrc(head), rv_pre = v_rsrc(head);
+    int tn_max = tb - 1;
     auto stage_piece = [&](int t, int buf, int i) {
         char* dst = smem + buf * STAGE + wv * (NJ * 1024);
 #if defined(__HIP_DEVICE_COMPILE__)
         if (i < NJ)
-            __builtin_amdgcn_raw_ptr_buffer_load_lds(rk, (lds_ptr_t)(dst + i * 1024), 16, k_vo[i], t * k_tile_bytes, 0, 0);
+            __builtin_amdgcn_raw_ptr_buffer_load_lds(rk_pre, (lds_ptr_t)(dst + i * 1024), 16, k_vo[i], t * k_tile_bytes, 0, 0);
         else
-            __builtin_amdgcn_raw_ptr_buffer_load_lds(rv, (lds_ptr_t)(dst + K_TILE + (i - NJ) * 1024), 16, v_vo[i - NJ], t * (KVB * 2), 0, 0);
+            __builtin_amdgcn_raw_ptr_buffer_load_lds(rv_pre, (lds_ptr_t)(dst + K_TILE + (i - NJ) * 1024), 16, v_vo[i - NJ], t * (KVB * 2), 0, 0);
 #else
         (void)dst; (void)t; (void)i;
 #endif
@@ -144,22 +178,26 @@
     for (int i = 0; i < 2 * NJ; ++i) stage_piece(0, 0, i);
 
     float c[2] = {p.scale_log2e, p.scale_log2e};
-    if constexpr (QS) {
-        const int quarter = p.q_ss_ld >> 2;
-        float ss[2] = {0.f, 0.f};
-#pragma unroll
-        for (int qb = 0; qb < 2; ++qb) {
-            const float* sp = p.q_ss + (long)min(q0 + 16 * qb + l15, p.Nq - 1) * p.q_ss_ld + g * quarter;
+    auto row_scale = [&](int q0u) __attribute__((always_inline)) {
+        c[0] = c[1] = p.scale_log2e;
+        if constexpr (QS) {
+            const int quarter = p.q_ss_ld >> 2;
+            float ss[2] = {0.f, 0.f};
+#pragma unroll
+            for (int qb = 0; qb < 2; ++qb) {
+                const float* sp = p.q_ss + (long)min(q0u + 16 * qb + l15, p.Nq - 1) * p.q_ss_ld + g * quarter;
 #pragma unroll 4
-            for (int jj = 0; jj < quarter; jj += 4) {
-                const f32x4 t = *(const f32x4*)(sp + jj);
-                ss[qb] += (t[0] + t[1]) + (t[2] + t[3]);
-            }
-        }
-        quad_fold_sum(ss[0], ss[1]);
-        c[0] *= rsqrtf(ss[0] / (float)p.q_norm_dim + p.q_eps);
-        c[1] *= rsqrtf(ss[1] / (float)p.q_norm_dim + p.q_eps);
-    }
+                for (int jj = 0; jj < quarter; jj += 4) {
+                    const f32x4 t = *(const f32x4*)(sp + jj);
+                    ss[qb] += (t[0] + t[1]) + (t[2] + t[3]);
+                }
+            }
+            quad_fold_sum(ss[0], ss[1]);
+            c[0] *= rsqrtf(ss[0] / (float)p.q_norm_dim + p.q_eps);
+            c[1] *= rsqrtf(ss[1] / (float)p.q_norm_dim + p.q_eps);
+        }
+    };
+    row_scale(q0);
     bf16x8 qf[2][NKS];
 #pragma unroll
     for (int qb = 0; qb < 2; ++qb) {
@@ -172,6 +210,7 @@
             for (int e = 0; e < 8; ++e) qf[qb][ks][e] = f2bf(bf2f(raw[e]) * c[qb]);
         }
     }
+    [[maybe_unused]] bf16x8 qraw[2][NKS];
 
     f32x4 o[NDB][2];
 #pragma unroll
@@ -185,7 +224,7 @@
         static_assert(!(FAST && (MASKED || KM)), "the stale-maximum path takes whole, unmasked tiles");
         asm volatile("s_waitcnt vmcnt(0)" ::: "memory");
         __syncthreads();
-        const int tn = min(t + 1, tb - 1);
+        const int tn = min(t + 1, tn_max);
         constexpr int nbuf = 1 - PAR;
 #if AT_PRIO
         __builtin_amdgcn_s_setprio(AT_PQK);
@@ -350,60 +389,121 @@
     using F_ = std::false_type;
     using P0 = std::integral_constant<int, 0>;
     using P1 = std::integral_constant<int, 1>;
-    if constexpr (KM) {
-        for (int t = 0; t < tb; ++t) {
-            if (t & 1) tile(t, F_{}, T_{}, P1{}, false);
-            else tile(t, F_{}, T_{}, P0{}, t == 0);
-        }
-    } else {
-        const int t_fast_end = min(tb, nfull);
-        int t = 0;
-        if (nfull > 0) {
-            tile(0, F_{}, F_{}, P0{}, true);
-            t = 1;
-            for (; t + 1 < t_fast_end; t += 2) {
-                tile(t, T_{}, F_{}, P1{}, false);
-                tile(t + 1, T_{}, F_{}, P0{}, false);
-            }
-            if (t < t_fast_end) {
-                tile(t, T_{}, F_{}, P1{}, false);
-                ++t;
-            }
-        }
-        if (nfull < tb) {
-            if (nfull & 1) tile(nfull, F_{}, T_{}, P1{}, false);
-            else tile(nfull, F_{}, T_{}, P0{}, nfull == 0);
-        }
-    }
-    asm volatile("s_waitcnt vmcnt(0)" ::: "memory");
-
-    float lt[2] = {l_run[0], l_run[1]};
-    quad_fold_sum(lt[0], lt[1]);
-#pragma unroll
-    for (int qb = 0; qb < 2; ++qb) {
-        const int qrow = q0 + 16 * qb + l15;
-        float inv = 1.0f / lt[qb];
-        if (p.gate && qrow < p.Nq) {
-            float gl = p.gate[(long)qrow * p.gate_ld + head];
-            if (p.gate_parts > 1) {
-                for (int pt = 1; pt < p.gate_parts; ++pt) gl += p.gate[((long)pt * p.Nq + qrow) * p.gate_ld + head];
-                gl += p.gate_bias[head];
-            }
-            inv *= 2.f / (1.f + __expf(-gl));
-        }
-        bf16* op = p.O + (long)min(qrow, p.Nq - 1) * p.ldo + head * HD + 16 * (g & 1) + 8 * (g >> 1);
-#pragma unroll
-        for (int i = 0; i < NDB / 2; ++i) {
-            bf16x4 a, b;
-#pragma unroll
-            for (int e = 0; e < 4; ++e) {
-                a[e] = f2bf(o[2 * i][qb][e] * inv);
-                b[e] = f2bf(o[2 * i + 1][qb][e] * inv);
-            }
-            u32x2 ua = __builtin_bit_cast(u32x2, a), ub = __builtin_bit_cast(u32x2, b);
-            asm volatile("s_nop 1\n\tv_permlane16_swap_b32 %0, %2\n\tv_permlane16_swap_b32 %1, %3\n\ts_nop 1" : "+v"(ua[0]), "+v"(ua[1]), "+v"(ub[0]), "+v"(ub[1]));
-            const u32x4 w = {ua[0], ua[1], ub[0], ub[1]};
-            if (qrow < p.Nq) *(u32x4*)(op + 32 * i) = w;
+    [[maybe_unused]] int ui = 0;
+#pragma nounroll
+    for (;;) {
+        [[maybe_unused]] const bool has_next = PAIR && ui + 1 < nu;
+        auto to_next = [&]() __attribute__((always_inline)) {
+            if constexpr (PAIR) {
+                if (has_next && !(tb & 1)) {
+                    rk_pre = k_rsrc(head_n);
+                    rv_pre = v_rsrc(head_n);
+                    tn_max = 0;
+                }
+            }
+        };
+        if constexpr (KM) {
+            for (int t = 0; t < tb; ++t) {
+                if (t == tb - 1) to_next();
+                if (t & 1) tile(t, F_{}, T_{}, P1{}, false);
+                else tile(t, F_{}, T_{}, P0{}, t == 0);
+            }
+        } else {
+            const int t_fast_end = min(tb, nfull);
+            int t = 0;
+            if (nfull > 0) {
+                tile(0, F_{}, F_{}, P0{}, true);
+                t = 1;
+                for (; t + 1 < t_fast_end; t += 2) {
+                    tile(t, T_{}, F_{}, P1{}, false);
+                    tile(t + 1, T_{}, F_{}, P0{}, false);
+                }
+                if (t < t_fast_end) {
+                    if (nfull == tb) to_next();
+                    tile(t, T_{}, F_{}, P1{}, false);
+                    ++t;
+                }
+            }
+            if (nfull < tb) {
+                to_next();
+                if (nfull & 1) tile(nfull, F_{}, T_{}, P1{}, false);
+                else tile(nfull, F_{}, T_{}, P0{}, nfull == 0);
+            }
+        }
+        [[maybe_unused]] int q0_n = 0;
+        if (has_next) {
+            if constexpr (PAIR) {
+                q0_n = qt_n * QB + wv * 32;
+                if (tb & 1) {
+                    __syncthreads();
+                    rk_pre = k_rsrc(head_n);
+                    rv_pre = v_rsrc(head_n);
+#pragma unroll
+                    for (int i = 0; i < 2 * NJ; ++i) stage_piece(0, 0, i);
+                }
+#pragma unroll
+                for (int qb = 0; qb < 2; ++qb) {
+                    const int qrow = min(q0_n + 16 * qb + l15, p.Nq - 1);
+                    const bf16* qp = p.Q + (long)qrow * p.ldq + head_n * HD + 8 * g;
+#pragma unroll
+                    for (int ks = 0; ks < NKS; ++ks) qraw[qb][ks] = *(const bf16x8*)(qp + 32 * ks);
+                }
+            }
+        } else {
+            asm volatile("s_waitcnt vmcnt(0)" ::: "memory");
+        }
+
+        float lt[2] = {l_run[0], l_run[1]};
+        quad_fold_sum(lt[0], lt[1]);
+#pragma unroll
+        for (int qb = 0; qb < 2; ++qb) {
+            const int qrow = q0 + 16 * qb + l15;
+            float inv = 1.0f / lt[qb];
+            if (p.gate && qrow < p.Nq) {
+                float gl = p.gate[(long)qrow * p.gate_ld + head];
+                if (p.gate_parts > 1) {
+                    for (int pt = 1; pt < p.gate_parts; ++pt) gl += p.gate[((long)pt * p.Nq + qrow) * p.gate_ld + head];
+                    gl += p.gate_bias[head];
+                }
+                inv *= 2.f / (1.f + __expf(-gl));
+            }
+            bf16* op = p.O + (long)min(qrow, p.Nq - 1) * p.ldo + head * HD + 16 * (g & 1) + 8 * (g >> 1);
+#pragma unroll
+            for (int i = 0; i < NDB / 2; ++i) {
+                bf16x4 a, b;
+#pragma unroll
+                for (int e = 0; e < 4; ++e) {
+                    a[e] = f2bf(o[2 * i][qb][e] * inv);
+                    b[e] = f2bf(o[2 * i + 1][qb][e] * inv);
+                }
+                u32x2 ua = __builtin_bit_cast(u32x2, a), ub = __builtin_bit_cast(u32x2, b);
+                asm volatile("s_nop 1\n\tv_permlane16_swap_b32 %0, %2\n\tv_permlane16_swap_b32 %1, %3\n\ts_nop 1" : "+v"(ua[0]), "+v"(ua[1]), "+v"(ub[0]), "+v"(ub[1]));
+                const u32x4 w = {ua[0], ua[1], ub[0], ub[1]};
+                if (qrow < p.Nq) *(u32x4*)(op + 32 * i) = w;
+            }
+        }
+        if (!has_next) break;
+        if constexpr (PAIR) {
+            if (QS && qt_n != qt) row_scale(q0_n);
+            head = head_n;
+            qt = qt_n;
+            q0 = q0_n;
+            rk_pre = k_rsrc(head);
+            rv_pre = v_rsrc(head);
+            tn_max = tb - 1;
+            ++ui;
+#pragma unroll
+            for (int qb = 0; qb < 2; ++qb)
+#pragma unroll
+                for (int ks = 0; ks < NKS; ++ks)
+#pragma unroll
+                    for (int e = 0; e < 8; ++e) qf[qb][ks][e] = f2bf(bf2f(qraw[qb][ks][e]) * c[qb]);
+#pragma unroll
+            for (int d = 0; d < NDB; ++d)
+#pragma unroll
+                for (int qb = 0; qb < 2; ++qb) o[d][qb] = f32x4{0.f, 0.f, 0.f, 0.f};
+            M[0] = M[1] = 0.f;
+            l_run[0] = l_run[1] = 0.f;
         }
     }
 }
@@ -448,6 +548,29 @@
     }
 }
 
+int pair_grid(int qtiles, int H) {
+#if AT_XCD
+    if ((H & 7) == 0) {
+        const int hj = H >> 3;
+        return 8 * ((hj >> 1) * qtiles + (hj & 1) * ((qtiles + 1) / 2));
+    }
+#endif
+    return (qtiles * H + 1) / 2;
+}
+
+int device_cus() {
+    static int cus[64] = {};
+    int dev = 0;
+    (void)hipGetDevice(&dev);
+    if (dev < 0 || dev >= 64) dev = 0;
+    if (!cus[dev]) {
+        int n = 0;
+        if (hipDeviceGetAttribute(&n, hipDeviceAttributeMultiprocessorCount, dev) != hipSuccess || n <= 0) n = 256;
+        cus[dev] = n;
+    }
+    return cus[dev];
+}
+
 }
 
 int attn_launch(const AttnParams& p, hipStream_t stream) {
@@ -462,27 +585,40 @@
 #ifndef AT_NW
 #define AT_NW 4
 #endif
+    LTX2_CHECK_ARG(p.form >= ATTN_FORM_AUTO && p.form <= ATTN_FORM_PAIRED, "attention: launch form %d is not one of 0 (default), 1 (one unit), 2 (paired)", p.form);
     const int nw = (p.head_dim != 64 && !p.kmask) ? AT_NW : 4;
-    dim3 grid((p.Nq + nw * 32 - 1) / (nw * 32), p.H);
-#define AT_LAUNCH_NW(HDV, QSV, KMV, NWV)                                                                                                        \
+    const int qtiles = (p.Nq + nw * 32 - 1) / (nw * 32);
+    bool paired = false;
+    if (p.head_dim != 64 && nw == 4 && p.form != ATTN_FORM_ONE_UNIT)
+        paired = p.form == ATTN_FORM_PAIRED || (long)qtiles * p.H > 2L * device_cus();
+    dim3 grid(qtiles, p.H);
+    if (paired) grid = dim3(pair_grid(qtiles, p.H));
+#define AT_LAUNCH_NW(HDV, QSV, KMV, NWV, PRV)                                                                                                   \
     do {                                                                                                                                        \
         static PerDeviceOnce once_;                                                                                                             \
         if (once_.first())                                                                                                                      \
-            (void)hipFuncSetAttribute((const void*)attn_fwd_kernel<HDV, QSV, KMV, NWV>, hipFuncAttributeMaxDynamicSharedMemorySize, Geo<HDV>::LDS_BYTES); \
-        hipLaunchKernelGGL((attn_fwd_kernel<HDV, QSV, KMV, NWV>), grid, dim3(NWV * 64), Geo<HDV>::LDS_BYTES, stream, p);                         \
+            (void)hipFuncSetAttribute((const void*)attn_fwd_kernel<HDV, QSV, KMV, NWV, PRV>, hipFuncAttributeMaxDynamicSharedMemorySize, Geo<HDV>::LDS_BYTES); \
+        hipLaunchKernelGGL((attn_fwd_kernel<HDV, QSV, KMV, NWV, PRV>), grid, dim3(NWV * 64), Geo<HDV>::LDS_BYTES, stream, p);                    \
     } while (0)
-#define AT_LAUNCH(HDV, QSV, KMV) AT_LAUNCH_NW(HDV, QSV, KMV, 4)
+#define AT_LAUNCH(HDV, QSV, KMV)                                   \
+    do {                                                           \
+        if (paired) AT_LAUNCH_NW(HDV, QSV, KMV, 4, true);          \
+        else AT_LAUNCH_NW(HDV, QSV, KMV, 4, false);                \
+    } while (0)
     if (p.head_dim == 64) {
-        if (p.kmask) AT_LAUNCH(64, false, true);
-        else AT_LAUNCH(64, false, false);
+        if (p.kmask) AT_LAUNCH_NW(64, false, true, 4, false);
+        else AT_LAUNCH_NW(64, false, false, 4, false);
     } else if (p.kmask) {
         if (p.q_ss) AT_LAUNCH(128, true, true);
         else AT_LAUNCH(128, false, true);
-    } else if (p.q_ss) {
-        if (nw == 8) AT_LAUNCH_NW(128, true, false, 8);
-        else AT_LAUNCH(128, true, false);
-    } else if (nw == 8) AT_LAUNCH_NW(128, false, false, 8);
+    }
+#if AT_NW == 8
+    else if (p.q_ss) AT_LAUNCH_NW(128, true, false, 8, false);
+    else AT_LAUNCH_NW(128, false, false, 8, false);
+#else
+    else if (p.q_ss) AT_LAUNCH(128, true, false);
     else AT_LAUNCH(128, false, false);
+#endif
 #undef AT_LAUNCH
 #undef AT_LAUNCH_NW
     LTX2_CHECK_LAUNCH("attn_fwd_kernel");
diff --git a/ltx-2-mlx_amd/csrc/capi.hip b/ltx-2-mlx_amd/csrc/capi.hip
--- a/ltx-2-mlx_amd/csrc/capi.hip
+++ b/ltx-2-mlx_amd/csrc/capi.hip
@@ -103,11 +103,19 @@
     return gemm_launch(p, epilogue, false, (hipStream_t)stream);
 }
 
+static int split_attn_form(int& head_dim) {
+    const int form = (head_dim >> 8) & 3;
+    head_dim &= 0xff;
+    return form;
+}
+
 int ltx2_flash_attn_rowscale(const void* Q, int64_t ldq, const void* K, int64_t ldk, const void* VT, int Npad, void* out, int64_t ldo, int Nq, int Nkv,
                              int H, int head_dim, float scale, const float* q_ss, int q_ss_ld, int q_norm_dim, float q_eps, void* stream) {
     LTX2_CHECK_ARG(Q && K && VT && out && q_ss, "flash_attn_rowscale: null operand");
+    const int form = split_attn_form(head_dim);
     LTX2_CHECK_ARG(head_dim == 128, "flash_attn_rowscale: head_dim=%d, only 128 is implemented", head_dim);
     AttnParams a{};
+    a.form = form;
     a.Q = (const bf16*)Q;
     a.ldq = ldq;
     a.K = (const bf16*)K;
@@ -132,8 +140,10 @@
 int ltx2_flash_attn_keymask(const void* Q, int64_t ldq, const void* K, int64_t ldk, const void* VT, int Npad, void* out, int64_t ldo, int Nq, int Nkv,
                             int H, int head_dim, float scale, const float* mask, void* words, void* stream) {
     LTX2_CHECK_ARG(Q && K && VT && out && mask && words, "flash_attn_keymask: null operand");
+    const int form = split_attn_form(head_dim);
     if (const int rc = keymask_words_launch(mask, Nkv, (unsigned long long*)words, Npad / 64, (hipStream_t)stream)) return rc;
     AttnParams a{};
+    a.form = form;
     a.Q = (const bf16*)Q;
     a.ldq = ldq;
     a.K = (const bf16*)K;
@@ -334,8 +344,10 @@
 int ltx2_flash_attn_gated(const void* Q, int64_t ldq, const void* K, int64_t ldk, const void* VT, int Npad, void* out, int64_t ldo, int Nq, int Nkv,
                           int H, int head_dim, float scale, const float* gate_logits, int gate_ld, void* stream) {
     LTX2_CHECK_ARG(Q && K && VT && out && gate_logits && gate_ld >= H, "flash_attn_gated: null operand / gate_ld < H");
+    const int form = split_attn_form(head_dim);
     LTX2_CHECK_ARG(head_dim == 128 || head_dim == 64, "flash_attn_gated: head_dim=%d, only 128 and 64 are implemented", head_dim);
     AttnParams a{};
+    a.form = form;
     a.Q = (const bf16*)Q;
     a.ldq = ldq;
     a.K = (const bf16*)K;
@@ -359,9 +371,11 @@
                                 int H, int head_dim, float scale, const void* x, int64_t ldx, const void* gate_w, const float* gate_b, int Dq, float* parts,
                                 void* stream) {
     LTX2_CHECK_ARG(Q && K && VT && out && x && gate_w && gate_b && parts, "flash_attn_gated_parts: null operand");
+    const int form = split_attn_form(head_dim);
     LTX2_CHECK_ARG(head_dim == 128 || head_dim == 64, "flash_attn_gated_parts: head_dim=%d, only 128 and 64 are implemented", head_dim);
     if (const int rc = gate_logits_parts_launch((const bf16*)x, ldx, (const bf16*)gate_w, parts, Nq, Dq, H, (hipStream_t)stream)) return rc;
     AttnParams a{};
+    a.form = form;
     a.Q = (const bf16*)Q;
     a.ldq = ldq;
     a.K = (const bf16*)K;
@@ -386,8 +400,10 @@
 int ltx2_flash_attn(const void* Q, int64_t ldq, const void* K, int64_t ldk, const void* VT, int Npad, void* out,
                     int64_t ldo, int Nq, int Nkv, int H, int head_dim, float scale, void* stream) {
     LTX2_CHECK_ARG(Q && K && VT && out, "flash_attn: null operand");
+    const int form = split_attn_form(head_dim);
     LTX2_CHECK_ARG(head_dim == 128 || head_dim == 64, "flash_attn: head_dim=%d, only 128 and 64 are implemented", head_dim);
     AttnParams a{};
+    a.form = form;
     a.Q = (const bf16*)Q;
     a.ldq = ldq;
     a.K = (const bf16*)K;
diff --git a/ltx-2-mlx_amd/csrc/dit_engine.hip b/ltx-2-mlx_amd/csrc/dit_engine.hip
--- a/ltx-2-mlx_amd/csrc/dit_engine.hip
+++ b/ltx-2-mlx_amd/csrc/dit_engine.hip
@@ -98,6 +98,7 @@
     bool adaln_combine = true;
     bool text_kv_ahead = true;
     hipEvent_t text_kv_ev = nullptr;
+    int attn_form = ATTN_FORM_AUTO;
     int fold_norms = 1;
     bool fp8_compute = false;
     bool prepared = false;
@@ -533,8 +534,9 @@
 };
 int attend(const bf16* q, long ldq, const bf16* k, long ldk, const bf16* vt, int npad, bf16* out, long ldo, int nq,
            int nkv, int H, int hd, hipStream_t st, const float* q_ss = nullptr, float q_eps = 0.f,
-           const unsigned long long* kmask = nullptr, GateRef gate = GateRef{}) {
+           const unsigned long long* kmask = nullptr, GateRef gate = GateRef{}, int form = ATTN_FORM_AUTO) {
     AttnParams a{};
+    a.form = form;
     a.kmask = kmask;
     a.gate = gate.p;
     a.gate_ld = H;
@@ -667,7 +669,7 @@
         TRY(qknorm_rope_launch(m.qkv, 3 * D, N, D, hd, 2, offs, wts, eps, m.cosb, m.sinb, st));
     }
     if (!vt_done) TRY(vt_transpose_launch(m.qkv + 2 * D, 3 * D, m.vt, N, m.Npad, H, st, hd));
-    TRY(attend(m.qkv, 3 * D, m.qkv + D, 3 * D, m.vt, m.Npad, m.att, D, N, N, H, hd, st, nullptr, 0.f, nullptr, glog(c, m)));
+    TRY(attend(m.qkv, 3 * D, m.qkv + D, 3 * D, m.vt, m.Npad, m.att, D, N, N, H, hd, st, nullptr, 0.f, nullptr, glog(c, m), c->attn_form));
     Fold fo{};
     if (fl >= 1) fold_produce(fo, m, nullptr);
     TRY(dense(c, m.att, D, w.self.o_w, w.self.o_b, m.x, D, N, D, D, EPI_RESID_GATE_F32, st, E(2), es, tab + 2 * D, nullptr, nullptr, false, nullptr, fl >= 1 ? &fo : nullptr));
@@ -703,7 +705,7 @@
         TRY(qknorm_rope_launch(m.qkv, D, N, D, hd, 1, offs, wts, eps, nullptr, nullptr, st));
     }
     TRY(attend(m.qkv, D, kk, 2 * D, vt, m.Spad, m.att, D, N, m.S, H, hd, st, m.qfold ? m.qss : nullptr, eps,
-               m.has_kmask ? m.kmask : nullptr, glog(c, m)));
+               m.has_kmask ? m.kmask : nullptr, glog(c, m), c->attn_form));
     if (c->v2)
         TRY(dense(c, m.att, D, w.text.o_w, w.text.o_b, m.x, D, N, D, D, EPI_RESID_GATE_F32, st, E(8), es, tab + 8 * D));
     else
@@ -772,7 +774,7 @@
         TRY(qknorm_rope_launch(a_q, Da, a.N, Da, hd, 1, offs, wts, eps, a.ccos, a.csin, sa));
     }
     TRY(event_wait(audio_kv, st));
-    TRY(attend(v_q, Da, a_kv, 2 * Da, a.vt, a.Npad, v.att, Da, v.N, a.N, H, hd, st, nullptr, 0.f, nullptr, glog(c, v)));
+    TRY(attend(v_q, Da, a_kv, 2 * Da, a.vt, a.Npad, v.att, Da, v.N, a.N, H, hd, st, nullptr, 0.f, nullptr, glog(c, v), c->attn_form));
     TRY(dense(c, v.att, Da, w.a2v.o_w, w.a2v.o_b, v.x, Dv, v.N, Dv, Da, EPI_RESID_GATE_F32, st, comb ? nullptr : v.cross_gate, 0, tv + 4 * Dv));
     TRY(event_wait(video_norm, sa));
     TRY(dense(c, v.h2, Dv, w.v2a.kv_w, w.v2a.kv_b, v_kv, 2 * Da, v.N, 2 * Da, Dv, EPI_BF16, sa, nullptr, 0, nullptr, &vo, &vt_done));
@@ -781,7 +783,7 @@
         TRY(qknorm_rope_launch(v_kv, 2 * Da, v.N, Da, hd, 1, offs, wts, eps, v.ccos, v.csin, sa));
     }
     if (!vt_done) TRY(vt_transpose_launch(v_kv + Da, 2 * Da, v.vt, v.N, v.Npad, H, sa, hd));
-    TRY(attend(a_q, Da, v_kv, 2 * Da, v.vt, v.Npad, a.att, Da, a.N, v.N, H, hd, sa, nullptr, 0.f, nullptr, glog(c, a)));
+    TRY(attend(a_q, Da, v_kv, 2 * Da, v.vt, v.Npad, a.att, Da, a.N, v.N, H, hd, sa, nullptr, 0.f, nullptr, glog(c, a), c->attn_form));
     TRY(dense(c, a.att, Da, w.v2a.o_w, w.v2a.o_b, a.x, Da, a.N, Da, Da, EPI_RESID_GATE_F32, sa, comb ? nullptr : a.cross_gate, 0, ta + 4 * Da));
     return LTX2_OK;
 }
@@ -1323,6 +1325,11 @@
         c->fold_norms = value;
         return LTX2_OK;
     }
+    if (!strcmp(name, "attn_form")) {
+        LTX2_CHECK_ARG(value >= ATTN_FORM_AUTO && value <= ATTN_FORM_PAIRED, "dit_set_option: attn_form is 0, 1 or 2");
+        c->attn_form = value;
+        return LTX2_OK;
+    }
     if (!strcmp(name, "adaln_combine")) {
         c->adaln_combine = value != 0;
         return LTX2_OK;
diff --git a/ltx-2-mlx_amd/kernels.py b/ltx-2-mlx_amd/kernels.py
--- a/ltx-2-mlx_amd/kernels.py
+++ b/ltx-2-mlx_amd/kernels.py
@@ -107,15 +107,19 @@
     return (out, ss) if prod else out
 
 
+ATTN_FORM_ONE_UNIT = 0x100
+ATTN_FORM_PAIRED = 0x200
+
+
 def flash_attn_rowscale(q: torch.Tensor, k: torch.Tensor, vt: torch.Tensor, heads: int, nkv: int, q_ss: torch.Tensor, eps: float = 1e-6,
-                        scale: Optional[float] = None) -> torch.Tensor:
+                        scale: Optional[float] = None, form: int = 0) -> torch.Tensor:
     assert q.dtype in ACT16 and q_ss.dtype == torch.float32 and q_ss.is_contiguous()
     nq, hd = q.shape[0], vt.shape[1]
     out = torch.empty(nq, heads * hd, device=q.device, dtype=q.dtype)
     if scale is None:
         scale = 1.0 / math.sqrt(float(hd))
     nv.check(_L(q).ltx2_flash_attn_rowscale(nv.ptr(q), q.stride(0), nv.ptr(k), k.stride(0), nv.ptr(vt), vt.shape[2], nv.ptr(out), out.stride(0), nq, nkv,
-                                            heads, hd, scale, nv.ptr(q_ss), q_ss.shape[1], heads * hd, eps, nv.stream()))
+                                            heads, hd | form, scale, nv.ptr(q_ss), q_ss.shape[1], heads * hd, eps, nv.stream()))
     return out
 
 
@@ -146,7 +150,7 @@
 
 
 def flash_attn_keymask(q: torch.Tensor, k: torch.Tensor, vt: torch.Tensor, heads: int, nkv: int, mask: torch.Tensor,
-                       scale: Optional[float] = None) -> torch.Tensor:
+                       scale: Optional[float] = None, form: int = 0) -> torch.Tensor:
     assert q.dtype in ACT16 and mask.numel() == nkv
     nq, hd = q.shape[0], vt.shape[1]
     out = torch.empty(nq, heads * hd, device=q.device, dtype=q.dtype)
@@ -155,7 +159,7 @@
     if scale is None:
         scale = 1.0 / math.sqrt(float(hd))
     nv.check(_L(q).ltx2_flash_attn_keymask(nv.ptr(q), q.stride(0), nv.ptr(k), k.stride(0), nv.ptr(vt), vt.shape[2], nv.ptr(out), out.stride(0), nq, nkv,
-                                           heads, hd, scale, nv.ptr(f), nv.ptr(words), nv.stream()))
+                                           heads, hd | form, scale, nv.ptr(f), nv.ptr(words), nv.stream()))
     return out
 
 
@@ -365,14 +369,14 @@
 
 
 def flash_attn(q: torch.Tensor, k: torch.Tensor, vt: torch.Tensor, heads: int, nkv: int,
-               scale: Optional[float] = None) -> torch.Tensor:
+               scale: Optional[float] = None, form: int = 0) -> torch.Tensor:
     assert q.dtype in ACT16 and k.dtype == q.dtype and vt.dtype == q.dtype and q.stride(1) == 1 and k.stride(1) == 1
     nq, hd = q.shape[0], vt.shape[1]
     out = torch.empty(nq, heads * hd, device=q.device, dtype=q.dtype)
     if scale is None:
         scale = 1.0 / math.sqrt(float(hd))
     nv.check(_L(q).ltx2_flash_attn(nv.ptr(q), q.stride(0), nv.ptr(k), k.stride(0), nv.ptr(vt), vt.shape[2], nv.ptr(out),
-                                      out.stride(0), nq, nkv, heads, hd, scale, nv.stream()))
+                                      out.stride(0), nq, nkv, heads, hd | form, scale, nv.stream()))
     return out
 
 
```

New measurement: 13.52 steps/s. Within noise of the previous version (-0.6%).
